# wwang2/CoarseGrainingVAE

Measured on AMD Instinct MI355X. Metric: train_step_frames_per_sec, higher is better.
Workload: dtype f32

## Files before the change

coarsegrainingvae_amd/_lib.py:

```python
from __future__ import annotations

import ctypes as C
import os
import re
import threading

import torch

from . import ktimer

_PKG = os.path.dirname(os.path.abspath(__file__))
LIB_PATH = os.environ.get("CGV_LIB") or os.path.join(_PKG, "libcgvae_hip.so")
HEADER_PATH = os.path.join(os.path.dirname(_PKG), "include", "cgvae_hip.h")

_lock = threading.Lock()
_lib = None

_p, _i, _f, _sz = C.c_void_p, C.c_int, C.c_float, C.c_size_t

PROTOTYPES = {
    "cgv_version": (_i, []),
    "cgv_last_error_string": (C.c_char_p, []),
    "cgv_timestamp": (_i, [_p, _p]),
    "cgv_timestamp_hz": (_i, []),
    "cgv_sustained_clock_probe": (_i, [_p, _p, _i, _i, _p]),
    "cgv_set_option": (_i, [_i, _i]),
    "cgv_get_option": (_i, [_i]),
    "cgv_reset_options": (_i, []),
    "cgv_rbf_supported": (_i, [_i]),
    "cgv_geom_stride": (_i, [_i]),
    "cgv_geom_unit_offset": (_i, [_i]),
    "cgv_radius_graph_count": (_i, [_p, _p, _i, _i, _f, _i, _p, _p, _p]),
    "cgv_radius_graph_emit": (_i, [_p, _p, _i, _i, _f, _i, _p, _p, _p]),
    "cgv_csr_workspace_bytes": (_sz, [_i]),
    "cgv_csr_build": (_i, [_p, _p, _i, _i, _i, _i, _p, _p, _p, _p, _p, _p, _p, _p, _p, _sz, _p]),
    "cgv_group_plan_workspace_bytes": (_sz, [_i]),
    "cgv_group_plan_build": (_i, [_p, _p, _p, _i, _i, _i, _i, _p, _p, _p, _p, _p, _sz, _p]),
    "cgv_group_plan_radix_workspace_bytes": (_sz, [_i]),
    "cgv_group_plan_build_radix": (_i, [_p, _p, _i, _i, _i, _i, _p, _p, _p, _p, _p, _sz, _p]),
    "cgv_geom_group_stride": (_i, [_i]),
    "cgv_geom_group_unit_offset": (_i, [_i]),
    "cgv_edge_geometry_grouped": (_i, [_p, _p, _p, _p, _p, _i, _i, _f, _p, _p, _p]),
    "cgv_edge_geometry": (_i, [_p, _p, _p, _p, _p, _p, _i, _i, _f, _p, _p, _p]),
    "cgv_plan_jobs_max": (_i, []),
    "cgv_plan_job_bytes": (_i, []),
    "cgv_plan_jobs_build": (_i, [_p, _i, _p]),
    "cgv_geom_jobs_max": (_i, []),
    "cgv_geom_job_bytes": (_i, []),
    "cgv_geom_jobs_build": (_i, [_p, _i, _p]),
    "cgv_segment_reduce": (_i, [_p, _p, _p, _i, _i, _i, _p, _p]),
    "cgv_embedding_rows": (_i, [_p, _p, _i, _i, _i, _i, _p, _p]),
    "cgv_embedding_rows2": (_i, [_p, _p, _i, _i, _i, _p, _p, _p, _i, _i, _i, _p, _i, _p]),
    "cgv_segment_reduce_pair": (_i, [_p, _p, _p, _i, _p, _p, _p, _p, _i, _p, _i, _p]),
    "cgv_segment_broadcast": (_i, [_p, _p, _p, _i, _i, _i, _p, _p]),
    "cgv_equi_msg_fwd": (_i, [_p, _p, _p, _p, _p, _p, _p, _p, _p, _i, _i, _i, _i, C.c_int64, C.c_int64, _p, _p, _p]),
    "cgv_equi_msg_grouped_supported": (_i, [_i, _i, _i]),
    "cgv_equi_msg_fwd_grouped": (_i, [_p] * 9 + [_i, _i, _i, _i, C.c_int64, C.c_int64, _p, _p, _p]),
    "cgv_equi_msg_bwd_workspace_bytes": (_sz, [_i, _i, _i]),
    "cgv_equi_msg_bwd": (_i, [_p] * 13 + [_i, _i, _i, C.c_int64, C.c_int64, _p, _sz, _p]),
    "cgv_pseudo_msg_fwd": (_i, [_p] * 14 + [_i, _i, _i, _i, _p]),
    "cgv_pseudo_msg_fwd_rows": (_i, [_p] * 15 + [_i, _i, _i, _i, C.c_int64, _p]),
    "cgv_pseudo_msg_bwd_workspace_bytes": (_sz, [_i, _i, _i]),
    "cgv_pseudo_msg_bwd": (_i, [_p] * 24 + [_i, _i, _i, _i, C.c_int64, _p, _sz, _p]),
    "cgv_pseudo_msg_bwd_deferred": (_i, [_p] * 22 + [_i, _i, _i, _i, C.c_int64, _p, _sz, _p, _p]),
    "cgv_update_rows_from_vec": (_i, [_p, _p, _i, _i, _p]),
    "cgv_tile_bwd_input_plan": (_i, [_i, _i, _i, _i, _p, _p]),
    "cgv_tile_linear_bwd_input_norm_stack": (_i, [_p, _p, _p, _i, _i, _i, _i, _p, _p, _p, _p, _p, _i, _i, _p]),
    "cgv_update_vec_from_rows": (_i, [_p, _p, _p, _i, _i, _p]),
    "cgv_update_norm_stack_fwd": (_i, [_p, _p, _p, _i, _i, _i, _p]),
    "cgv_update_norm_stack_bwd": (_i, [_p, _p, _p, _p, _p, _p, _i, _i, _i, _i, _p]),
    "cgv_update_gate_fwd": (_i, [_p, _p, _p, _p, _p, _p, _p, _i, _i, _i, _p]),
    "cgv_update_gate_bwd": (_i, [_p, _p, _p, _p, _p, _p, _p, _p, _i, _i, _i, _p]),
    "cgv_skinny_max_rows": (_i, []),
    "cgv_skinny_supported": (_i, [_i, _i, _i]),
    "cgv_skinny_fwd_supported": (_i, [_i, _i, _i]),
    "cgv_skinny_linear_fwd": (_i, [_p, _p, _p, _p, _p, _i, _i, _i, _i, _p]),
    "cgv_skinny_bwd_input_supported": (_i, [_i, _i, _i]),
    "cgv_skinny_bwd_input_workspace_bytes": (_sz, [_i, _i, _i]),
    "cgv_skinny_linear_bwd_input": (_i, [_p, _p, _p, _p, _i, _i, _i, _i, _p, _sz, _p]),
    "cgv_decoder_layer_supported": (_i, [_i, _i, _i]),
    "cgv_decoder_slice_floats": (C.c_int64, [_i, _i]),
    "cgv_batch_load_rows": (_i, [_p, _p, _p, _i, _p, _p, _p, _i, _p]),
    "cgv_reparam_sample": (_i, [_p, _p, _p, _p, C.c_int64, _p, _p]),
    "cgv_reparam_bwd": (_i, [_p, _p, _p, _p, _p, _p, C.c_int64, _p]),
    "cgv_pair_linear_fwd": (_i, [_p] * 10 + [_i] * 5 + [_p]),
    "cgv_equi_msg_bwd_deferred": (_i, [_p] * 11 + [_i, _i, _i, C.c_int64, C.c_int64, _p, C.c_size_t, _p, _p, _p]),
    "cgv_filter_reduce_jobs_max": (_i, []),
    "cgv_filter_reduce_job_bytes": (_i, []),
    "cgv_filter_reduce_jobs": (_i, [_p, _i, _p]),
    "cgv_pair_linear_bwd_input": (_i, [_p] * 6 + [_i, _i, _p, _p, _i, _i, _i, _p, C.c_size_t, _p]),
    "cgv_loss_tail_supported": (_i, [_i, _i, _i, _i]),
    "cgv_loss_tail_workspace_bytes": (_sz, [_i]),
    "cgv_loss_tail": (_i, [_p] * 12 + [_i, _i, _i, _i, _i, _f, _f] + [_p] * 9 + [_p, _sz, _p]),
    "cgv_multi_linear_max": (_i, []),
    "cgv_multi_linear_fwd": (_i, [_i] + [_p] * 6 + [_i, _i, _i, _p]),
    "cgv_multi_linear_bwd_input": (_i, [_i, _i] + [_p] * 5 + [_i, _i, _i, _p, C.c_size_t, _p]),
    "cgv_decoder_max_edges": (_i, []),
    "cgv_decoder_block_channels": (_i, [_i]),
    "cgv_decoder_debug_clock": (_i, [_p]),
    "cgv_decoder_msg_fwd": (_i, [_p] * 18 + [_i, _i, _i, _i, _p]),
    "cgv_decoder_dense_fwd": (_i, [_p, _p, _p, _p, _p, _i, _i, _i, _i, _p]),
    "cgv_prior_msg_fwd": (_i, [_p] * 13 + [_i, _i, _i, _i, _i, _p]),
    "cgv_prior_msg_bwd": (_i, [_p] * 8 + [_i, C.c_int64] + [_p] * 6 + [C.c_int64, _i, _i, _i, _i, _p]),
    "cgv_decoder_uv_fwd": (_i, [_p, _p, _p, _p, _i, _i, _p]),
    "cgv_decoder_gate_fwd": (_i, [_p] * 9 + [_i, _i, _p]),
    "cgv_decoder_gate_bwd": (_i, [_p, _p, _p, _p, _i, C.c_int64, _p, _p, _p, _p, _p, _p, C.c_int64, _i, _i, _p]),
    "cgv_decoder_dense_bwd": (_i, [_p, _i, C.c_int64, _p, _i, _p, _p, _p, C.c_int64, _i, _i, _i, _p]),
    "cgv_decoder_uv_bwd": (_i, [_p, _i, C.c_int64, _p, _p, _p, _p, _p, _p, _p, _p, C.c_int64, _i, _i, _p]),
    "cgv_decoder_msg_bwd": (_i, [_p] * 15 + [_p, _i, C.c_int64, _p, _p, _p] + [_p] * 8 + [C.c_int64, _i, _i, _i, _i, _p]),
    "cgv_decoder_slices_to_dense": (_i, [_p, _p, _i, C.c_int64, _p, _i, _i, _p]),
    "cgv_dense_grad_prepare": (_i, [_p, _p, _p, _p, _i, _i, _i, _i, _p]),
    "cgv_tile_supported": (_i, [_i, _i, _i]),
    "cgv_tile_linear_fwd": (_i, [_p, _p, _p, _p, _p, _i, _i, _i, _i, _p]),
    "cgv_tile_linear_bwd_input": (_i, [_p, _p, _p, _i, _i, _i, _p]),
    "cgv_tile_linear_bwd_input_act": (_i, [_p, _p, _p, _p, _i, _i, _i, _i, _p]),
    "cgv_tile_linear_bwd_input_act_add": (_i, [_p, _p, _p, _p, _p, _i, _i, _i, _i, _p]),
    "cgv_tile_linear_bwd_input_act_add_bcast": (_i, [_p] * 7 + [_i, _p, _i, _i, _i, _i, _p]),
    "cgv_tile_pair_supported": (_i, [_i, _i, _i]),
    "cgv_tile_pair_linear_fwd": (_i, [_p] * 10 + [_i, _i, _i, _i, _i, _p]),
    "cgv_tile_pair_linear_bwd_input": (_i, [_p] * 10 + [_i, _i, _i, _i, _i, _p]),
    "cgv_tile_linear_bwd_input_out": (_i, [_p] * 5 + [_i, _i, _i, _i, _p, _i, _p]),
    "cgv_tile_bwd_input_split": (_i, [_p, _sz, _p]),
    "cgv_tile_pair_linear_bwd_input_out": (_i, [_p] * 10 + [_i, _i, _i, _i, _i, _p, _i, _p, _i, _p]),
    "cgv_tile_linear_bwd_input_sum2": (_i, [_p] * 10 + [_i, _p, _i, _i, _i, _i, _i, _p]),
    "cgv_segment_reduce2": (_i, [_p, _i, _p, _p, _i, _p, _p, _p, _i, _i, _p]),
    "cgv_skinny_linear_bwd_input_add": (_i, [_p, _p, _p, _p, _p, _i, _i, _i, _i, _p, _sz, _p]),
    "cgv_skinny_linear_bwd_input_out": (_i, [_p] * 5 + [_i, _i, _i, _i, _p, _i, _p, _sz, _p]),
    "cgv_tile_linear_wgrad": (_i, [_p, _p, _p, _i, _i, _i, _i, _p]),
    "cgv_wgrad_record_bytes": (_i, []),
    "cgv_wgrad_plan": (_i, [_i, _i, _i, _p, _p, _p]),
    "cgv_wgrad_lds_floats": (_i, [_i, _i]),
    "cgv_grouped_wgrad": (_i, [_p, _i, _i, _i, _p]),
    "cgv_wgrad_gathered_plan": (_i, [_i, _i, _i, _i, _p, _p]),
    "cgv_grouped_wgrad_gathered": (_i, [_p, _i, _i, _p]),
    "cgv_wgrad_gathered_plan_tile": (_i, [_i, _i, _i, _i, _i, _p, _p]),
    "cgv_grouped_wgrad_gathered_tile": (_i, [_p, _i, _i, _i, _p]),
    "cgv_grouped_wgrad_split": (_i, [_p, _i, _i, _p]),
    "cgv_grouped_wgrad_gathered_sumsq": (_i, [_p, _i, _i, _p, _p, _p]),
    "cgv_grouped_wgrad_gathered_adam": (_i, [_p, _i, _i, _p, _p, _p, _p, _f, _f, _f, _f, _p, _p]),
    "cgv_wgrad_strip_max_rows": (_i, []),
    "cgv_wgrad_strip_plan": (_i, [_i, _i, _i, _i, _p]),
    "cgv_wgrad_strip_split_max_rows": (_i, []),
    "cgv_wgrad_strip_split_plane_bytes": (_sz, [_i, _i]),
    "cgv_grouped_wgrad_strip_split": (_i, [_p, _i, _i, _i, _i, _p, _sz, _p]),
    "cgv_grouped_wgrad_strip": (_i, [_p, _i, _i, _i, _p]),
    "cgv_grouped_wgrad_strip_sumsq": (_i, [_p, _i, _i, _i, _p, _p, _p]),
    "cgv_grouped_wgrad_strip_adam": (_i, [_p, _i, _i, _i, _p, _p, _p, _p, _f, _f, _f, _f, _p, _p]),
    "cgv_pack_record_bytes": (_i, []),
    "cgv_pack_plan": (_i, [_i, _i, _i, _p]),
    "cgv_pack_operands": (_i, [_p, _i, _i, _p]),
    "cgv_reconstruct_fwd": (_i, [_p, _p, _p, _p, _p, _i, _i, _i, _p, _p]),
    "cgv_reconstruct_bwd": (_i, [_p, _p, _p, _p, _i, _i, _i, _p, _p, _p]),
    "cgv_elbo_workspace_bytes": (_sz, [_i, _i]),
    "cgv_elbo_fwd": (_i, [_p] * 7 + [_i, _i, _i, _i, _f, _f] + [_p] * 7 + [_p, _sz, _p]),
    "cgv_elbo_scale": (_i, [_p, _p, _p, _p, _p, _i, _p, _i, _p]),
    "cgv_optim_state_floats": (_i, []),
    "cgv_optim_partial_floats": (_i, []),
    "cgv_adam_clip_step": (_i, [_p, _p, _p, _p, C.c_int64, _f, _f, _f, _f, _f, _f, _p, _f, _p, _p, _p]),
    "cgv_optim_prepare": (_i, [_p, C.c_int64, _f, _f, _f, _f, _p, _f, _p, _p, _p]),
    "cgv_adam_apply": (_i, [_p, _p, _p, _p, C.c_int64, _f, _f, _f, _f, _p, _p]),
    "cgv_sgd_apply": (_i, [_p, _p, C.c_int64, _f, _p, _p]),
    "cgv_wgrad_gram": (_i, [_p, _i, _i, _p, _p, C.c_size_t, _p]),
    "cgv_wgrad_gram_workspace_bytes": (C.c_size_t, [_i]),
    "cgv_wgrad_gram_mfma": (_i, [_p, _i, _i, _p, _p, C.c_size_t, _p]),
    "cgv_wgrad_gram_mfma_workspace_bytes": (C.c_size_t, [_i, _i]),
    "cgv_wgrad_gram_mfma_max_rows": (_i, []),
    "cgv_rank_update_supported": (_i, [_i, _i, _i]),
    "cgv_optim_prepare_extra": (_i, [_p, C.c_int64, _p, _i, _f, _f, _f, _f, _p, _f, _p, _p, _p]),
    "cgv_grouped_wgrad_adam": (_i, [_p, _i, _i, _i, _p, _p, _p, _p, _f, _f, _f, _f, _p, _p]),
    "cgv_rank_flat_quantum": (_i, []),
    "cgv_rank_flat_plan": (_i, [_i, _i, _i, _i, _p, _p]),
    "cgv_grouped_wgrad_adam_flat": (_i, [_p, _i, _i, _i, _i, _p, _p, _p, _p, _f, _f, _f, _f, _p, _p]),
    "cgv_grouped_wgrad_adam_mixed": (_i, [_p, _i, _i, _i, _i, _i, _i, _p, _p, _p, _p, _f, _f, _f, _f, _p, _p]),
    "cgv_sample_quality_max_classes": (_i, []),
    "cgv_sample_quality": (_i, [_p] * 6 + [_i] * 5 + [_p, _p, _p]),
    "cgv_ensemble_check_max_classes": (_i, []),
    "cgv_ensemble_check_max_samples": (_i, []),
    "cgv_ensemble_check": (_i, [_p] * 7 + [_i] * 6 + [_p, _p, _p]),
    "cgv_internal_hist_max_features": (_i, []),
    "cgv_internal_hist_max_pairs": (_i, []),
    "cgv_internal_hist_max_bins": (_i, []),
    "cgv_internal_hist_max_bins2": (_i, []),
    "cgv_internal_hist_max_atoms": (_i, []),
    "cgv_internal_hist_max_staged_atoms": (_i, []),
    "cgv_internal_hist_feature_tile": (_i, [_i]),
    "cgv_internal_hist_pair_tile": (_i, [_i]),
    "cgv_internal_hist": (_i, [_p] * 4 + [_i] * 6 + [C.c_double] * 2 + [_p] * 3),
    "cgv_internal_values": (_i, [_p] * 3 + [_i] * 3 + [_p] * 3),
    "cgv_kde_max_planes": (_i, []),
    "cgv_kde_max_samples": (_i, []),
    "cgv_kde_max_points": (_i, []),
    "cgv_kde_max_splits": (_i, []),
# ... 21 lines not shown
    "cgv_sasa_max_points": (_i, []),
    "cgv_sasa_max_classes": (_i, []),
    "cgv_sasa_max_structures": (_i, []),
    "cgv_sasa_workspace_bytes": (_sz, [_i, _i, _i]),
    "cgv_sasa_counts": (_i, [_p] * 5 + [_i] * 5 + [_p] * 5 + [_p, _sz, _p]),
    "cgv_cluster_max_structures": (_i, []),
    "cgv_cluster_workspace_bytes": (_sz, [_i, _i]),
    "cgv_cluster_pack": (_i, [_p, _i, _i, _i, _i, _i, C.c_double, _p, _p]),
    "cgv_cluster_gromos": (_i, [_p, _p, _i, _p, _p, _p, _p, _p]),
    "cgv_hbond_max_structures": (_i, []),
    "cgv_hbond_max_hydrogens": (_i, []),
    "cgv_hbond_max_acceptors": (_i, []),
    "cgv_hbond_row_tile": (_i, []),
    "cgv_hbond_chunk": (_i, []),
    "cgv_hbond_workspace_bytes": (_sz, [_i, _i, _i]),
    "cgv_hbond_counts": (_i, [_p] * 6 + [_i, _i, _i, _i, _f, _f] + [_p] * 5 + [_p, _sz, _p]),
    "cgv_lddt_max_atoms": (_i, []),
    "cgv_lddt_max_structures": (_i, []),
    "cgv_lddt_max_references": (_i, []),
    "cgv_lddt_row_tile": (_i, []),
    "cgv_lddt_col_tile": (_i, []),
    "cgv_lddt_chunk": (_i, []),
    "cgv_lddt_workspace_bytes": (_sz, [_i, _i, _i]),
    "cgv_lddt_counts": (_i, [_p] * 7 + [_i] * 4 + [_f] * 6 + [_p] * 3 + [_p, _sz, _p]),
    "cgv_dssp_max_residues": (_i, []),
    "cgv_dssp_max_structures": (_i, []),
    "cgv_dssp_wave_path_max": (_i, []),
    "cgv_dssp_bend_c2": (_f, []),
    "cgv_dssp_assign": (_i, [_p] * 4 + [_i, _i, _i] + [_p] * 5 + [_p]),
    "cgv_pca_max_features": (_i, []),
    "cgv_pca_max_atoms": (_i, []),
    "cgv_pca_max_structures": (_i, []),
    "cgv_pca_max_components": (_i, []),
    "cgv_pca_max_bins2": (_i, []),
    "cgv_pca_moments_splits": (_i, [_i, _i]),
    "cgv_pca_moments_workspace_bytes": (_sz, [_i, _i]),
    "cgv_pca_moments": (_i, [_p] * 4 + [_i] * 3 + [_p] * 3 + [_p, _sz, _p]),
    "cgv_pca_project": (_i, [_p] * 6 + [_i] * 4 + [_p, _i, _i, _i] + [C.c_double] * 4 + [_p] * 3),
    "cgv_pairdist_max_atoms": (_i, []),
    "cgv_pairdist_max_structures": (_i, []),
    "cgv_pairdist_max_classes": (_i, []),
    "cgv_pairdist_max_bins": (_i, []),
    "cgv_pairdist_row_tile": (_i, []),
    "cgv_pairdist_col_tile": (_i, []),
    "cgv_pairdist_chunk": (_i, []),
    "cgv_pairdist_workspace_bytes": (_sz, [_i, _i]),
    "cgv_pairdist_counts": (_i, [_p] * 4 + [_i] * 5 + [_f] * 2 + [_p] * 3 + [_p, _sz, _p]),
    "cgv_dist_moments_max_atoms": (_i, []),
    "cgv_dist_moments_max_structures": (_i, []),
    "cgv_dist_moments_max_total": (_i, []),
    "cgv_dist_moments_row_tile": (_i, []),
    "cgv_dist_moments_col_tile": (_i, []),
    "cgv_dist_moments_chunk": (_i, []),
    "cgv_dist_moments_workspace_bytes": (_sz, [_i, _i]),
    "cgv_dist_moments": (_i, [_p] * 4 + [_i] * 3 + [_p] * 4 + [_p, _sz, _p]),
    "cgv_align_max_atoms": (_i, []),
    "cgv_align_max_structures": (_i, []),
    "cgv_align_wave_fits": (_i, [_i]),
    "cgv_align_workspace_bytes": (_sz, [_i, _i, _i]),
    "cgv_align_accumulate": (_i, [_p] * 3 + [_i] * 4 + [_p] * 6 + [_p, _sz, _p]),
    "cgv_cgae_resident_fits": (_i, [_i, _i, _i]),
    "cgv_cgae_workspace_bytes": (_sz, [_i, _i, _i, _i]),
    "cgv_cgae_steps": (_i, [_i] + [_p] * 7 + [_i, _p, C.c_int64, _i, _i, _i, _i, C.c_int64, _i, _f] + [C.c_double] * 4 +
                       [C.c_uint64, _p, _p, _p, _p, _sz, _p]),
    "cgv_cgae_noise": (_i, [C.c_uint64, C.c_int64, _i, _i, _i, _p, _p]),
    "cgv_newman_resident_fits": (_i, [_i, _i]),
    "cgv_newman_groups": (_i, [_i, _i]),
    "cgv_newman_workspace_bytes": (_sz, [_i, _i, _i, _i]),
    "cgv_newman_betweenness": (_i, [_p] * 4 + [_i] * 4 + [_p, _p, _sz, _p]),
    "cgv_newman_components": (_i, [_p] * 5 + [_i] * 4 + [_p, _p, _p, _sz, _p]),
    "cgv_newman_partition": (_i, [_p] * 8 + [_i] * 6 + [_p, _sz, _p]),
    "cgv_baseline_resident_fits": (_i, [_i, _i, _i, _i]),
    "cgv_baseline_workspace_bytes": (_sz, [_i] * 7),
    "cgv_baseline_steps": (_i, [_i, _i, _i] + [_p] * 4 + [_i, _p, C.c_int64] + [_i] * 5 + [_p, _p, _p, _i, C.c_int64, _i, _f] +
                           [C.c_double] * 4 + [_p, _p, _p, _sz, _p]),
    "cgv_baseline_loss_workspace_bytes": (_sz, [_i, _i, _i]),
    "cgv_baseline_loss": (_i, [_p, _p, _p, _i, _i, _i, _f, _p, _p, _p, _sz, _p]),
}


OPTIONS = {"msg_fwd_split": 0, "msg_bwd_split": 1, "csr_build": 2, "pseudo_chunks": 3, "wgrad_tiling": 4, "tile_fwd_lds_min": 5,
           "bwd_input_waves": 6, "pseudo_fwd": 7, "decoder_fat": 8, "decoder_wlds": 9, "skinny_rows": 10, "tile_fwd_bal": 11,
           "optim_one_launch": 12, "decoder_colsplit": 13, "decoder_nodesplit": 14, "bwd_input_split": 15, "msg_bwd_mfma": 16,
           "streamk": 17}


def set_option(name: str, value: int) -> None:
    call("cgv_set_option", OPTIONS[name], int(value))


def get_option(name: str) -> int:
    return int(load().cgv_get_option(OPTIONS[name]))


def reset_options() -> None:
    call("cgv_reset_options")


def header_symbols():
    text = open(HEADER_PATH).read()
    text = re.sub(r"/\*.*?\*/", "", text, flags=re.S)
    return sorted(set(re.findall(r"\b(cgv_[a-z0-9_]+)\s*\(", text)))


def load():
    global _lib
    if _lib is not None:
        return _lib
    with _lock:
        if _lib is not None:
            return _lib
        if not os.path.exists(LIB_PATH):
            raise RuntimeError(
                f"{LIB_PATH} is missing: build it with `python -m coarsegrainingvae_amd.build` "
                "(hipcc --offload-arch=gfx950).  There is no fallback path.")
        lib = C.CDLL(LIB_PATH)
        for name, (res, args) in PROTOTYPES.items():
            fn = getattr(lib, name)
            fn.restype = res
            fn.argtypes = args
        if lib.cgv_version() < 101:
            raise RuntimeError("libcgvae_hip.so is older than this package")
        _lib = lib
    return _lib


def stream_ptr() -> int:
    return torch.cuda.current_stream().cuda_stream


def ptr(t):
    if t is None:
        return None
    if not t.is_cuda:
        raise RuntimeError("coarsegrainingvae_amd kernels need device (hip) tensors; there is no CPU path")
    if not t.is_contiguous():
        raise RuntimeError("tensor handed to the C ABI must be contiguous")
    return t.data_ptr()


_SPLIT_WS = {}
_SPLIT_TLS = threading.local()
_SPLIT_BYTES = 64 * 1024 + 64 * 1024 * 1024


def prepare_split_workspace(stream=None):
    st = torch.cuda.current_stream() if stream is None else stream
    key = (st.device.index if st.device.index is not None else torch.cuda.current_device(), int(st.cuda_stream))
    if key not in _SPLIT_WS:
        if torch.cuda.is_current_stream_capturing():
            return None
        _SPLIT_WS[key] = torch.zeros(_SPLIT_BYTES, dtype=torch.uint8, device=f"cuda:{key[0]}")
    return _SPLIT_WS[key]


def split_workspace_ready() -> bool:
    if load().cgv_get_option(OPTIONS["bwd_input_split"]) == 1:
        return False
    key = (torch.cuda.current_device(), int(torch.cuda.current_stream().cuda_stream))
    return key in _SPLIT_WS or not torch.cuda.is_current_stream_capturing()


def _register_split_workspace(lib):
    key = (torch.cuda.current_device(), int(torch.cuda.current_stream().cuda_stream))
    if getattr(_SPLIT_TLS, "cur", None) == key:
        return
    ws = prepare_split_workspace()
# ... 20 lines not shown
```

coarsegrainingvae_amd/csrc/api.cpp:

```cpp
#include <stdarg.h>
#include <string.h>
#include <atomic>
#include "cgv_common.h"

namespace cgv {
static thread_local char g_err[512] = "";
void set_error(const char* fmt, ...) {
  va_list ap;
  va_start(ap, fmt);
  vsnprintf(g_err, sizeof(g_err), fmt, ap);
  va_end(ap);
}

static const int g_opt_default[] = {
     -1,    -1,     0,
     0,     0,       448,
     0,   0,         1,
     1,      0,        1,
     0,  2,   1,
     -1,  -1,      0};
static_assert(sizeof(g_opt_default) == CGV_OPT_COUNT * sizeof(int), "one default per CGV_OPT_*");
static std::atomic<int> g_opt[CGV_OPT_COUNT];
static void reset_options() {
  for (int i = 0; i < CGV_OPT_COUNT; ++i) g_opt[i].store(g_opt_default[i], std::memory_order_relaxed);
}
static const bool g_opt_ready = (reset_options(), true);
int option(int id) { return g_opt[id].load(std::memory_order_relaxed); }
}

extern "C" {
int cgv_version(void) { return CGV_VERSION; }
int cgv_set_option(int option, int value) {
  CGV_REQUIRE(option >= 0 && option < CGV_OPT_COUNT, "unknown option");
  cgv::g_opt[option].store(value, std::memory_order_relaxed);
  return 0;
}
int cgv_get_option(int option) {
  if (option < 0 || option >= CGV_OPT_COUNT) return INT32_MIN;
  return cgv::g_opt[option].load(std::memory_order_relaxed);
}
int cgv_reset_options(void) {
  cgv::reset_options();
  return 0;
}
const char* cgv_last_error_string(void) { return cgv::g_err; }
int cgv_rbf_supported(int R) {
  switch (R) {
#define X(n) case n:
    CGV_RBF_LIST(X)
#undef X
    return 1;
    default:
      return 0;
  }
}
int cgv_geom_stride(int R) { return cgv::geom_stride(R); }
int cgv_geom_unit_offset(int R) { return cgv::geom_unit_offset(R); }
}
```

coarsegrainingvae_amd/csrc/decoder_layer.hip:

```cpp
#include "cgv_common.h"

namespace cgv {

typedef float f32x4 __attribute__((ext_vector_type(4)));

__constant__ unsigned long long* g_dl_clock = nullptr;
#ifndef CGV_DL_CLOCK
#define CGV_DL_CLOCK 0
#endif
#if CGV_DL_CLOCK
#define DL_SPAN(id, end)                                                                                    \
  do {                                                                                                      \
    if (g_dl_clock && threadIdx.x == 0) {                                                                   \
      if (blockIdx.x == 0) g_dl_clock[32 + 4 * (id) + (end)] = wall_clock64();                              \
      if (blockIdx.x == gridDim.x - 1) g_dl_clock[32 + 4 * (id) + 2 + (end)] = wall_clock64();              \
    }                                                                                                       \
  } while (0)

#define DL_PH(id, i) do { if (g_dl_clock && blockIdx.x == 0 && threadIdx.x == 0) g_dl_clock[80 + 10 * (id) + (i)] = wall_clock64(); } while (0)
#else
#define DL_SPAN(id, end) do { } while (0)
#define DL_PH(id, i) do { } while (0)
#endif

#if CGV_DL_CLOCK
#define DL_WV(i) do { if (g_dl_clock && blockIdx.x == 0 && (threadIdx.x & 63) == 0) g_dl_clock[192 + 8 * (threadIdx.x >> 6) + (i)] = wall_clock64(); } while (0)
#else
#define DL_WV(i) do { } while (0)
#endif
#ifndef CGV_DL_FILTER_PERM
#define CGV_DL_FILTER_PERM 1
#endif
constexpr int DL_CB = 4;
constexpr int DL_WAVES = 9;
constexpr int DL_THREADS = 64 * DL_WAVES;
constexpr int DL_MAX_NODES = 16;

struct dv3 { float x, y, z; };
__device__ __forceinline__ dv3 dldv(const float* p) { f3 t = ld3(p); return dv3{t.x, t.y, t.z}; }
__device__ __forceinline__ dv3 dcross(const dv3& a, const dv3& b) {
  return dv3{a.y * b.z - a.z * b.y, a.z * b.x - a.x * b.z, a.x * b.y - a.y * b.x};
}
__device__ __forceinline__ float ddot(const dv3& a, const dv3& b) { return a.x * b.x + a.y * b.y + a.z * b.z; }
__device__ __forceinline__ void daxpy(dv3& acc, float a, const dv3& x) {
  acc.x = fmaf(a, x.x, acc.x); acc.y = fmaf(a, x.y, acc.y); acc.z = fmaf(a, x.z, acc.z);
}
__device__ __forceinline__ float add_xor32(float x) {
  const auto r = __builtin_amdgcn_permlane32_swap(__float_as_uint(x), __float_as_uint(x), false, false);
  return __uint_as_float(r[0]) + __uint_as_float(r[1]);
}
__device__ __forceinline__ float add_xor16(float x) {
  const auto r = __builtin_amdgcn_permlane16_swap(__float_as_uint(x), __float_as_uint(x), false, false);
  return __uint_as_float(r[0]) + __uint_as_float(r[1]);
}
__device__ __forceinline__ float add_row_stride4(float x) {
  x += __uint_as_float(__builtin_amdgcn_update_dpp(0, __float_as_uint(x), 0x128 , 0xf, 0xf, false));
  x += __uint_as_float(__builtin_amdgcn_update_dpp(0, __float_as_uint(x), 0x124 , 0xf, 0xf, false));
  return x;
}
template <int R>
__device__ __forceinline__ float dfilt(const float (&W)[R + 1], const float* __restrict__ g) {
  float w = W[R] * g[R];
#pragma unroll
  for (int n = 0; n < R; ++n) w = fmaf(W[n], g[n], w);
  return w;
}

extern __shared__ __attribute__((aligned(16))) unsigned char dl_smem[];
struct Carve {
  size_t off = 0;
  __device__ __forceinline__ float* take(size_t floats) {
    float* p = reinterpret_cast<float*>(dl_smem + off);
    off += ((floats * 4 + 15) / 16) * 16;
    return p;
  }
};

#define CGV_GLOBAL_AS __attribute__((address_space(1)))
typedef const CGV_GLOBAL_AS float* gcf;
typedef const CGV_GLOBAL_AS int* gci;
__device__ __forceinline__ gcf launder(const float* p) {
  unsigned long long a = reinterpret_cast<unsigned long long>(p);
  asm volatile("" : "+s"(a));
  return reinterpret_cast<gcf>(a);
}
__device__ __forceinline__ gci launder(const int* p) {
  unsigned long long a = reinterpret_cast<unsigned long long>(p);
  asm volatile("" : "+s"(a));
  return reinterpret_cast<gci>(a);
}
__device__ __forceinline__ const float* generic(gcf p) { return (const float*)p; }
__device__ __forceinline__ void pin_loads() { asm volatile("" ::: "memory"); }
__device__ __forceinline__ float4 ldg4_pinned(gcf p) {
  const f32x4 t = *reinterpret_cast<const CGV_GLOBAL_AS f32x4*>(p);
  return make_float4(t.x, t.y, t.z, t.w);
}
#ifndef CGV_DL_NT_WEIGHTS
#define CGV_DL_NT_WEIGHTS 0
#endif
__device__ __forceinline__ float4 ldg4_stream(gcf p) {
#if CGV_DL_NT_WEIGHTS
  const f32x4 t = __builtin_nontemporal_load(reinterpret_cast<const CGV_GLOBAL_AS f32x4*>(p));
#else
  const f32x4 t = *reinterpret_cast<const CGV_GLOBAL_AS f32x4*>(p);
#endif
  return make_float4(t.x, t.y, t.z, t.w);
}
__device__ __forceinline__ float ldg_pinned(gcf p) { return *p; }
__device__ __forceinline__ int ldgi_pinned(gci p) { return *p; }
__device__ __forceinline__ f3 ld3_pinned(gcf p) { return f3{p[0], p[1], p[2]}; }

constexpr int DL_QS = 6;
template <int MB, int NQ, int QS = DL_QS>
struct QuadRegs { float4 v[QS][NQ][MB]; };

template <int MB, int NQ, int QS>
__device__ __forceinline__ void quad_issue(QuadRegs<MB, NQ, QS>& r, gcf slices, int n_slices, long long stride,
                                           int rows, const int (&kq)[NQ]) {
  const int lane = threadIdx.x & 63, wave = __builtin_amdgcn_readfirstlane(threadIdx.x >> 6);
  const int m = lane & 15, cls = wave * 4 + (lane >> 4);
#pragma unroll
  for (int u = 0; u < QS; ++u) {
    const int s = min(cls + 36 * u, n_slices - 1);
#pragma unroll
    for (int q = 0; q < NQ; ++q)
#pragma unroll
      for (int mb = 0; mb < MB; ++mb)
        r.v[u][q][mb] = ldg4_pinned(slices + (size_t)s * stride + ((size_t)kq[q] * rows + min(mb * 16 + m, rows - 1)) * 4);
  }
}

template <int MB, int NQ, int QS>
__device__ __forceinline__ void quad_finish(const QuadRegs<MB, NQ, QS>& r, float4* __restrict__ tile ,
                                            float4* __restrict__ scratch , int n_slices, int rows, int ph = -1) {
  constexpr int MP = 16 * MB;
  const int lane = threadIdx.x & 63, wave = __builtin_amdgcn_readfirstlane(threadIdx.x >> 6);
  const int m = lane & 15, cls = wave * 4 + (lane >> 4);
#pragma unroll
  for (int q = 0; q < NQ; ++q)
#pragma unroll
    for (int mb = 0; mb < MB; ++mb) {
      float4 acc = make_float4(0.f, 0.f, 0.f, 0.f);
#pragma unroll
      for (int u = 0; u < QS; ++u)
        if (cls + 36 * u < n_slices) { acc.x += r.v[u][q][mb].x; acc.y += r.v[u][q][mb].y; acc.z += r.v[u][q][mb].z; acc.w += r.v[u][q][mb].w; }
      acc.x = add_xor16(acc.x); acc.y = add_xor16(acc.y); acc.z = add_xor16(acc.z); acc.w = add_xor16(acc.w);
      acc.x = add_xor32(acc.x); acc.y = add_xor32(acc.y); acc.z = add_xor32(acc.z); acc.w = add_xor32(acc.w);
      if (lane < 16) scratch[((q * DL_WAVES + wave) * MB + mb) * 16 + m] = acc;
    }
  if (ph >= 0) DL_PH(ph, 2);
  if (ph == 8) DL_WV(3);
  __syncthreads();
  if (ph >= 0) DL_PH(ph, 3);
  if (threadIdx.x < NQ * MP) {
    const int q = threadIdx.x / MP, mm = threadIdx.x - q * MP;
    float4 t = make_float4(0.f, 0.f, 0.f, 0.f);
#pragma unroll
    for (int c = 0; c < DL_WAVES; ++c) {
      const float4 v = scratch[((q * DL_WAVES + c) * MB + mm / 16) * 16 + (mm & 15)];
      t.x += v.x; t.y += v.y; t.z += v.z; t.w += v.w;
    }
    if (mm >= rows) t = make_float4(0.f, 0.f, 0.f, 0.f);
    tile[q * MP + mm] = t;
  }
  __syncthreads();
}

template <int G, int NT>
struct BiRegs { float4 w[NT][G]; };

struct TileRange { int beg, end; };
__device__ __forceinline__ TileRange dl_tile_range(int K) {
  const int tiles = (K + 63) / 64, per = (tiles + (int)gridDim.y - 1) / (int)gridDim.y;
  const int beg = (int)blockIdx.y * per;
  return TileRange{beg, min(beg + per, tiles)};
}
__device__ __forceinline__ int dl_tile_of(const TileRange& tr, int wave, int t) {
  const int pos = t == 0 ? wave : (int)((0x854372106ull >> (4 * wave)) & 15);
  return tr.beg + DL_WAVES * t + pos;
}

template <int G, int NT>
__device__ __forceinline__ void bi_prefetch(BiRegs<G, NT>& r, gcf W, int K, const int (&row0)[G], const TileRange& tr) {
  const int lane = threadIdx.x & 63, wave = __builtin_amdgcn_readfirstlane(threadIdx.x >> 6);
  const int j = lane & 15, q = lane >> 4;
#pragma unroll
  for (int t = 0; t < NT; ++t) {
    const int tile = dl_tile_of(tr, wave, t);
    if (tile < tr.end) {
      const int col = tile * 64 + 4 * j;
      const int cc = col < K ? col : 0;
#pragma unroll
      for (int g = 0; g < G; ++g) r.w[t][g] = ldg4_stream(W + (size_t)(row0[g] + q) * K + cc);
    } else {
#pragma unroll
      for (int g = 0; g < G; ++g) r.w[t][g] = make_float4(0.f, 0.f, 0.f, 0.f);
    }
  }
}

template <int SLOT, int G, int NT>
__device__ __forceinline__ void bi_prefetch_slot(BiRegs<G, NT>& r, gcf W, int K, const int (&row0)[G], int tile) {
  const int lane = threadIdx.x & 63;
  const int j = lane & 15, q = lane >> 4;
  const int col = tile * 64 + 4 * j;
  const int cc = col < K ? col : 0;
#pragma unroll
  for (int g = 0; g < G; ++g) r.w[SLOT][g] = ldg4_stream(W + (size_t)(row0[g] + q) * K + cc);
}

#ifndef CGV_DL_SLICE_STORE
#define CGV_DL_SLICE_STORE 1
#endif
__device__ __forceinline__ void st4_slice(float4* p, const float4& v) {
#if CGV_DL_SLICE_STORE == 1
  const f32x4 t = {v.x, v.y, v.z, v.w};
  asm volatile("global_store_dwordx4 %0, %1, off sc1" : : "v"(p), "v"(t) : "memory");
#else
  *p = v;
#endif
}

template <int MB>
__host__ __device__ constexpr size_t bi_stage_floats() { return (size_t)DL_WAVES * 16 * 16 * MB * 4; }

template <int MB, int G, int NT, int NPRE = NT>
__device__ __forceinline__ void bi_core(const BiRegs<G, NPRE>& r, const float* __restrict__ g_tile ,
                                        float* __restrict__ stage ,
                                        float* __restrict__ slice , int K, int rows, const TileRange& tr,
                                        const float* __restrict__ W = nullptr, const int* row0 = nullptr, int ph = -1) {
  constexpr int MP = 16 * MB;
  const int lane = threadIdx.x & 63, wave = __builtin_amdgcn_readfirstlane(threadIdx.x >> 6);
  const int j = lane & 15, q = lane >> 4;
  float4* st = reinterpret_cast<float4*>(stage) + (size_t)wave * 16 * MP;
#pragma unroll
  for (int t = 0; t < NT; ++t) {
    const int tile = dl_tile_of(tr, wave, t);
    if (tile >= tr.end) continue;
    f32x4 acc[MB][4];
#pragma unroll
    for (int mb = 0; mb < MB; ++mb)
#pragma unroll
      for (int c = 0; c < 4; ++c) acc[mb][c] = f32x4{0.f, 0.f, 0.f, 0.f};
    float4 late[G];
    if (t >= NPRE) {
      const int col = tile * 64 + 4 * j;
      const int cc = col < K ? col : 0;
#pragma unroll
      for (int g = 0; g < G; ++g) late[g] = *reinterpret_cast<const float4*>(W + (size_t)(row0[g] + q) * K + cc);
    }
#pragma unroll
    for (int g = 0; g < G; ++g) {
      const float4 w = t < NPRE ? r.w[t < NPRE ? t : 0][g] : late[g];
#pragma unroll
      for (int mb = 0; mb < MB; ++mb) {
        const float a = g_tile[(mb * 16 + j) * (G * 4) + g * 4 + q];
        acc[mb][0] = __builtin_amdgcn_mfma_f32_16x16x4f32(a, w.x, acc[mb][0], 0, 0, 0);
        acc[mb][1] = __builtin_amdgcn_mfma_f32_16x16x4f32(a, w.y, acc[mb][1], 0, 0, 0);
        acc[mb][2] = __builtin_amdgcn_mfma_f32_16x16x4f32(a, w.z, acc[mb][2], 0, 0, 0);
        acc[mb][3] = __builtin_amdgcn_mfma_f32_16x16x4f32(a, w.w, acc[mb][3], 0, 0, 0);
      }
    }
#pragma unroll
    for (int mb = 0; mb < MB; ++mb)
#pragma unroll
      for (int rr = 0; rr < 4; ++rr)
        st[j * MP + mb * 16 + 4 * q + rr] = make_float4(acc[mb][0][rr], acc[mb][1][rr], acc[mb][2][rr], acc[mb][3][rr]);
    if (ph >= 0 && t == 0) DL_PH(ph, 7);
    const int quads = min(16, (K - tile * 64) / 4);
    float4* out = reinterpret_cast<float4*>(slice) + (size_t)tile * 16 * rows;
    for (int idx = lane; idx < quads * rows; idx += 64) {
      const int jj = idx / rows, m = idx - jj * rows;
      st4_slice(out + idx, st[jj * MP + m]);
    }
  }
}

template <int MB, int G>
__host__ __device__ constexpr size_t fwd_red_floats() { return (size_t)DL_WAVES * ((G + 3) / 4) * MB * 256; }

struct NoHook { __device__ __forceinline__ void operator()() const {} };
template <int MB, int G, int SB = (((G + 3) / 4) * MB >= 3 ? 5 : 9), typename Hook = NoHook>
__device__ __forceinline__ void fwd_core(float* __restrict__ out, float* __restrict__ red, const float* __restrict__ x,
                                         int M, int K, const float* __restrict__ W, const int (&row0)[G],
                                         Hook after_issue = Hook(), int ph = -1) {
  constexpr int T = (G + 3) / 4;
  const int lane = threadIdx.x & 63, wave = __builtin_amdgcn_readfirstlane(threadIdx.x >> 6);
  const int i = lane & 15, q = lane >> 4;
  const int steps = (K + 15) / 16, per = (steps + DL_WAVES - 1) / DL_WAVES;
  const int s_beg = wave * per, s_end = min(s_beg + per, steps);
  const float* wrow[T];
#pragma unroll
  for (int t = 0; t < T; ++t) {
    const int g = min(t * 4 + (i >> 2), G - 1);
    wrow[t] = W + (size_t)(row0[g] + (i & 3)) * K;
  }
  const float* xrow[MB];
#pragma unroll
  for (int mb = 0; mb < MB; ++mb) xrow[mb] = x + (size_t)min(mb * 16 + i, M - 1) * K;
  f32x4 acc[T][MB];
#pragma unroll
  for (int t = 0; t < T; ++t)
#pragma unroll
    for (int mb = 0; mb < MB; ++mb) acc[t][mb] = f32x4{0.f, 0.f, 0.f, 0.f};
  bool first = true;
  for (int s0 = s_beg; first || s0 < s_end; s0 += SB) {
    float4 a[SB][T], b[SB][MB];
#pragma unroll
    for (int u = 0; u < SB; ++u) {
      const int k = (s0 + u) * 16 + 4 * q;
      const int kc = (s0 + u < s_end && k < K) ? k : 0;
#pragma unroll
      for (int t = 0; t < T; ++t) a[u][t] = *reinterpret_cast<const float4*>(wrow[t] + kc);
#pragma unroll
      for (int mb = 0; mb < MB; ++mb) b[u][mb] = *reinterpret_cast<const float4*>(xrow[mb] + kc);
    }
    if (first) { after_issue(); first = false; if (ph >= 0) DL_PH(ph, 1); }
#pragma unroll
    for (int u = 0; u < SB; ++u) {
      if (s0 + u < s_end) {
        const bool kok = (s0 + u) * 16 + 4 * q < K;
#pragma unroll
        for (int t = 0; t < T; ++t) {
          const float4 w = make_float4(kok ? a[u][t].x : 0.f, kok ? a[u][t].y : 0.f, kok ? a[u][t].z : 0.f, kok ? a[u][t].w : 0.f);
#pragma unroll
          for (int mb = 0; mb < MB; ++mb) {
            acc[t][mb] = __builtin_amdgcn_mfma_f32_16x16x4f32(w.x, b[u][mb].x, acc[t][mb], 0, 0, 0);
            acc[t][mb] = __builtin_amdgcn_mfma_f32_16x16x4f32(w.y, b[u][mb].y, acc[t][mb], 0, 0, 0);
            acc[t][mb] = __builtin_amdgcn_mfma_f32_16x16x4f32(w.z, b[u][mb].z, acc[t][mb], 0, 0, 0);
            acc[t][mb] = __builtin_amdgcn_mfma_f32_16x16x4f32(w.w, b[u][mb].w, acc[t][mb], 0, 0, 0);
          }
        }
      }
    }
  }
#pragma unroll
  for (int t = 0; t < T; ++t)
#pragma unroll
    for (int mb = 0; mb < MB; ++mb)
#pragma unroll
      for (int r = 0; r < 4; ++r) red[(((wave * T + t) * MB + mb) * 4 + r) * 64 + lane] = acc[t][mb][r];
  if (ph >= 0) DL_PH(ph, 2);
  __syncthreads();
  if (ph >= 0) DL_PH(ph, 3);
  for (int o = threadIdx.x; o < T * MB * 256; o += DL_THREADS) {
    const int l = o & 63, r = (o >> 6) & 3, rest = o >> 8;
    const int mb = rest % MB, t = rest / MB;
    const int g = t * 4 + (l >> 4), m = mb * 16 + (l & 15);
    float v = 0.f;
#pragma unroll
    for (int w = 0; w < DL_WAVES; ++w) v += red[(((w * T + t) * MB + mb) * 4 + r) * 64 + l];
    if (g < G) out[(m * G + g) * 4 + r] = v;
  }
  __syncthreads();
  if (ph >= 0) DL_PH(ph, 4);
}

template <int G>
__device__ __forceinline__ void wlds_issue(float* __restrict__ w_l, const float* __restrict__ W, int K, const int (&row0)[G]) {
  const int lane = threadIdx.x & 63, wave = __builtin_amdgcn_readfirstlane(threadIdx.x >> 6);
#pragma unroll
  for (int g = 0; g < G; ++g) {
    if ((g % DL_WAVES) != wave) continue;
    const float* src = W + (size_t)row0[g] * K;
    for (int u = 0; u * 64 < K; ++u) {
      const int idx = u * 64 + lane;
      if (idx < K)
        __builtin_amdgcn_global_load_lds(reinterpret_cast<const CGV_GLOBAL_AS void*>(reinterpret_cast<unsigned long long>(src + 4 * (size_t)idx)),
                                         (__attribute__((address_space(3))) void*)(w_l + (size_t)g * 4 * K + u * 256), 16, 0, 0);
    }
  }
}

constexpr int WLDS_SB = 6;
__device__ __forceinline__ void wlds_x_issue(float4 (&b)[WLDS_SB], const float* __restrict__ x, int M, int K) {
  const int lane = threadIdx.x & 63, wave = __builtin_amdgcn_readfirstlane(threadIdx.x >> 6);
  const int i = lane & 15, q = lane >> 4;
  const int steps = (K + 15) / 16, per = (steps + DL_WAVES - 1) / DL_WAVES;
  const int s_beg = wave * per, s_end = min(s_beg + per, steps);
  const float* xrow = x + (size_t)min(i, M - 1) * K;
#pragma unroll
  for (int u = 0; u < WLDS_SB; ++u) {
    const int k = (s_beg + u) * 16 + 4 * q;
    b[u] = *reinterpret_cast<const float4*>(xrow + ((s_beg + u < s_end && k < K) ? k : 0));
  }
}
template <int G>
__device__ __forceinline__ void fwd_core_wlds_finish(float* __restrict__ out, float* __restrict__ red, const float4 (&b)[WLDS_SB],
                                                     int K, const float* __restrict__ w_l, int ph = -1) {
  constexpr int T = (G + 3) / 4, SB = WLDS_SB;
  const int lane = threadIdx.x & 63, wave = __builtin_amdgcn_readfirstlane(threadIdx.x >> 6);
  const int i = lane & 15, q = lane >> 4;
  const int steps = (K + 15) / 16, per = (steps + DL_WAVES - 1) / DL_WAVES;
  const int s_beg = wave * per, s_end = min(s_beg + per, steps);
  if (ph >= 0) DL_PH(ph, 1);
  asm volatile("s_waitcnt vmcnt(0)" ::: "memory");
  __syncthreads();
  if (ph >= 0) DL_PH(ph, 2);
  f32x4 acc[T];
#pragma unroll
  for (int t = 0; t < T; ++t) acc[t] = f32x4{0.f, 0.f, 0.f, 0.f};
  int wrow[T];
#pragma unroll
  for (int t = 0; t < T; ++t) wrow[t] = (min(t * 4 + (i >> 2), G - 1) * 4 + (i & 3)) * K;
#pragma unroll
  for (int u = 0; u < SB; ++u) {
    const int k = (s_beg + u) * 16 + 4 * q;
    const bool kok = s_beg + u < s_end && k < K;
    if (s_beg + u < s_end) {
#pragma unroll
      for (int t = 0; t < T; ++t) {
        float4 w = *reinterpret_cast<const float4*>(w_l + wrow[t] + (kok ? k : 0));
        if (!kok) w = make_float4(0.f, 0.f, 0.f, 0.f);
        acc[t] = __builtin_amdgcn_mfma_f32_16x16x4f32(w.x, b[u].x, acc[t], 0, 0, 0);
        acc[t] = __builtin_amdgcn_mfma_f32_16x16x4f32(w.y, b[u].y, acc[t], 0, 0, 0);
        acc[t] = __builtin_amdgcn_mfma_f32_16x16x4f32(w.z, b[u].z, acc[t], 0, 0, 0);
        acc[t] = __builtin_amdgcn_mfma_f32_16x16x4f32(w.w, b[u].w, acc[t], 0, 0, 0);
      }
    }
  }
#pragma unroll
  for (int t = 0; t < T; ++t)
#pragma unroll
    for (int r = 0; r < 4; ++r) red[((wave * T + t) * 4 + r) * 64 + lane] = acc[t][r];
  if (ph >= 0) DL_PH(ph, 3);
  __syncthreads();
  for (int o = threadIdx.x; o < T * 256; o += DL_THREADS) {
    const int l = o & 63, r = (o >> 6) & 3, t = o >> 8;
    const int g = t * 4 + (l >> 4), m = l & 15;
    float v = 0.f;
#pragma unroll
    for (int w = 0; w < DL_WAVES; ++w) v += red[((w * T + t) * 4 + r) * 64 + l];
    if (g < G) out[(m * G + g) * 4 + r] = v;
  }
  __syncthreads();
  if (ph >= 0) DL_PH(ph, 4);
}

constexpr int DL_MAX_EDGES = 240;
template <int SLOTS> struct Slots4 { float4 v[SLOTS]; };
template <int SLOTS>
__device__ __forceinline__ void copy4_issue(Slots4<SLOTS>& r, gcf src, int n4) {
#pragma unroll
  for (int u = 0; u < SLOTS; ++u) r.v[u] = ldg4_pinned(src + 4 * (size_t)min((int)threadIdx.x + u * DL_THREADS, n4 - 1));
}
template <int SLOTS>
__device__ __forceinline__ void copy4_commit(const Slots4<SLOTS>& r, float* __restrict__ dst, int n4) {
#pragma unroll
  for (int u = 0; u < SLOTS; ++u)
    if ((int)threadIdx.x + u * DL_THREADS < n4) reinterpret_cast<float4*>(dst)[threadIdx.x + u * DL_THREADS] = r.v[u];
}
__device__ __forceinline__ int int_issue(gci src, int n) { return ldgi_pinned(src + min((int)threadIdx.x, n - 1)); }
__device__ __forceinline__ void int_commit(int v, int* __restrict__ dst, int n) { if ((int)threadIdx.x < n) dst[threadIdx.x] = v; }
__device__ __forceinline__ float4 scalar_issue(gcf src, gcf valid, int n, int F, int f0) {
  return ldg4_pinned((src ? src : valid) + (size_t)min((int)threadIdx.x, n - 1) * F + f0);
}
__device__ __forceinline__ void scalar_commit(float4 v, bool have, float* __restrict__ dst, int n) {
  if ((int)threadIdx.x < n) reinterpret_cast<float4*>(dst)[threadIdx.x] = have ? v : make_float4(0.f, 0.f, 0.f, 0.f);
}
__device__ __forceinline__ float4 vector_issue(gcf src, gcf valid, int n, int F, int f0) {
  const int t = min((int)threadIdx.x, 3 * n - 1), m = t / 3, part = t - 3 * m;
  return ldg4_pinned((src ? src : valid) + ((size_t)m * F + f0) * 3 + 4 * part);
}
__device__ __forceinline__ void vector_commit(float4 v, bool have, float* __restrict__ dst, int n) {
  if ((int)threadIdx.x < 3 * n) reinterpret_cast<float4*>(dst)[threadIdx.x] = have ? v : make_float4(0.f, 0.f, 0.f, 0.f);
}
constexpr int geom_slots(int R) { return (DL_MAX_EDGES * geom_stride(R) / 4 + DL_THREADS - 1) / DL_THREADS; }
__device__ __forceinline__ void stage_copy4(float* __restrict__ dst, const float* __restrict__ src, int n4) {
  for (int i = threadIdx.x; i < n4; i += DL_THREADS) reinterpret_cast<float4*>(dst)[i] = reinterpret_cast<const float4*>(src)[i];
}
__device__ __forceinline__ void stage_ints(int* __restrict__ dst, const int* __restrict__ src, int n) {
  for (int i = threadIdx.x; i < n; i += DL_THREADS) dst[i] = src[i];
}
__device__ __forceinline__ void stage_scalar(float* __restrict__ dst, const float* __restrict__ src, int n, int F, int f0) {
  if (threadIdx.x < n)
    reinterpret_cast<float4*>(dst)[threadIdx.x] = src ? *reinterpret_cast<const float4*>(src + (size_t)threadIdx.x * F + f0)
                                                      : make_float4(0.f, 0.f, 0.f, 0.f);
}
__device__ __forceinline__ void stage_vector(float* __restrict__ dst, const float* __restrict__ src, int n, int F, int f0) {
  if (threadIdx.x < 3 * n) {
    const int m = threadIdx.x / 3, part = threadIdx.x - 3 * m;
    reinterpret_cast<float4*>(dst)[threadIdx.x] =
        src ? *reinterpret_cast<const float4*>(src + ((size_t)m * F + f0) * 3 + 4 * part) : make_float4(0.f, 0.f, 0.f, 0.f);
  }
}
__device__ __forceinline__ dv3 lds_v3(const float* p) { return dv3{p[0], p[1], p[2]}; }

template <int R, bool WLDS>
__global__ __launch_bounds__(DL_THREADS) void dec_msg_fwd_k(
    const float* __restrict__ a1, const float* __restrict__ W2, const float* __restrict__ b2, const float* __restrict__ s_,
    const float* __restrict__ sbar_, const float* __restrict__ v_, const float* __restrict__ vbar_,
    const float* __restrict__ geom_, const int* __restrict__ rowptr_, const int* __restrict__ src_,
    const float* __restrict__ Wd_, const float* __restrict__ bd_, float* __restrict__ phi_out, float* __restrict__ stack,
    float* __restrict__ sbar_out, float* __restrict__ v_out, float* __restrict__ vbar_out, float* __restrict__ rows_out,
    int n, int F, int E) {
  constexpr int GS = geom_stride(R), U = geom_unit_offset(R);
  Carve cv;
  float* red = cv.take(fwd_red_floats<1, 9>());
  float* phi_l = cv.take(16 * 9 * 4);
  float* red2 = cv.take(8 * 3 * 64);
  float* geom_l = cv.take((size_t)DL_MAX_EDGES * GS);
  int* rp_l = reinterpret_cast<int*>(cv.take(20));
  int* src_l = reinterpret_cast<int*>(cv.take(DL_MAX_EDGES));
  float* s_l = cv.take(64); float* sb_l = cv.take(64);
  float* v_l = cv.take(192); float* vb_l = cv.take(192);
  float* w_l = cv.take(WLDS ? (size_t)36 * F : 0);
  const int f0 = blockIdx.x * DL_CB;
  const int lane = threadIdx.x & 63;
  const int k = __builtin_amdgcn_readfirstlane(threadIdx.x >> 6);
  const int i = lane >> 2, c = lane & 3;
  const bool live = i < n;
  const int f = f0 + c;
  int row0[9];
#pragma unroll
  for (int g = 0; g < 9; ++g) row0[g] = g * F + f0;
  if (WLDS) wlds_issue<9>(w_l, W2, F, row0);
  DL_PH(1, 0);
  DL_SPAN(1, 0);
  const gcf geom = launder(geom_); const gci rowptr = launder(rowptr_); const gci src = launder(src_);
  const gcf s = launder(s_); const gcf sbar = launder(sbar_); const gcf v = launder(v_);
  const gcf vbar = launder(vbar_); const gcf Wd = launder(Wd_); const gcf bd = launder(bd_);
  const int n4 = E * GS / 4;
  Slots4<geom_slots(R)> r_geom;
  copy4_issue(r_geom, geom, n4);
  const int half = k == 0 ? lane >> 5 : 0;
  const gcf cand = k == 0 ? (half == 0 ? s : sbar) : k == 1 ? v : vbar;
  const int sm_D = k == 0 ? 1 : 3, sm_cnt = k == 0 ? n : 3 * n, sm_A = k == 0 ? F : 3 * F, sm_B = k == 0 ? 0 : 4;
  const int sm_C = k == 0 ? f0 : 3 * f0, sm_item = k == 0 ? (lane & 31) : lane;
  float4 r_small;
  {
    const int it = min(sm_item, sm_cnt - 1);
    const int m = (it * (sm_D == 1 ? 65536 : 21846)) >> 16, part = it - m * sm_D;
    r_small = ldg4_pinned(cand + ((size_t)m * sm_A + part * sm_B + sm_C));
  }
  const int id_item = k < 4 ? k * 64 + lane : lane, id_cnt = k < 4 ? E : n + 1;
  const int r_ids = ldgi_pinned((k < 4 ? src : rowptr) + min(id_item, id_cnt - 1));
  float W[R + 1];
#pragma unroll
  for (int nn = 0; nn < R; ++nn) W[nn] = ldg_pinned(Wd + ((size_t)k * F + f) * R + nn);
  W[R] = ldg_pinned(bd + (size_t)k * F + f);
  pin_loads();
  float4 xb[WLDS_SB];
  if (WLDS) wlds_x_issue(xb, a1, n, F);
  else fwd_core<1, 9, 5>(phi_l, red, a1, n, F, W2, row0, NoHook(), 1);
  {
    copy4_commit(r_geom, geom_l, n4);
    float* dst = k == 0 ? (half == 0 ? s_l : sb_l) : k == 1 ? v_l : vb_l;
    if (k <= 2 && sm_item < sm_cnt) reinterpret_cast<float4*>(dst)[sm_item] = r_small;
    if (k <= 4 && id_item < id_cnt) (k < 4 ? src_l : rp_l)[id_item] = r_ids;
  }
  if (WLDS) fwd_core_wlds_finish<9>(phi_l, red, xb, F, w_l, 1);
  for (int o = threadIdx.x; o < 16 * 9; o += DL_THREADS) {
    const int m = o / 9, g = o - m * 9;
    float4 p = *reinterpret_cast<float4*>(phi_l + (m * 9 + g) * 4);
    const float4 b = *reinterpret_cast<const float4*>(b2 + (size_t)g * F + f0);
    p.x += b.x; p.y += b.y; p.z += b.z; p.w += b.w;
    *reinterpret_cast<float4*>(phi_l + (m * 9 + g) * 4) = p;
    if (m < n) *reinterpret_cast<float4*>(phi_out + (size_t)m * 9 * F + (size_t)g * F + f0) = p;
  }
  __syncthreads();
  DL_PH(1, 5);
  const int ic = live ? i : 0;
  const float s_i = s_l[ic * 4 + c], sb_i = sb_l[ic * 4 + c];
  const dv3 v_i = lds_v3(v_l + (ic * 4 + c) * 3), vb_i = lds_v3(vb_l + (ic * 4 + c) * 3);
  float ah = 0.f, ahb = 0.f;
  dv3 acc{0.f, 0.f, 0.f};
  const float* __restrict__ vsrc = (k == 2 || k == 6 || k == 7) ? v_l : vb_l;
  const int e_beg = live ? rp_l[i] : 0, e_end = live ? min(rp_l[i + 1], E) : 0;
  int j_nx = e_beg < e_end ? src_l[e_beg] : 0;
  for (int e = e_beg; e < e_end; ++e) {
    const int j = j_nx;
    j_nx = src_l[min(e + 1, e_end - 1)];
    const float* __restrict__ g = geom_l + (size_t)e * GS;
    const dv3 vj = lds_v3(vsrc + (j * 4 + c) * 3);
    const float q = phi_l[(j * 9 + k) * 4 + c] * dfilt<R>(W, g);
    switch (k) {
      case 0: ah = fmaf(q, s_i, ah); ahb += ddot(v_i, vj); break;
      case 1: daxpy(acc, q, dv3{g[U], g[U + 1], g[U + 2]}); break;
      case 2: daxpy(acc, q, vj); break;
      case 3: daxpy(acc, q, dcross(v_i, vj)); break;
      case 4: daxpy(acc, q * sb_i, vj); break;
      case 5: daxpy(acc, q, vj); break;
      case 6: daxpy(acc, q * sb_i, vj); break;
      case 7: daxpy(acc, q, dcross(v_i, vj)); break;
      default: daxpy(acc, q, dcross(vb_i, vj)); break;
    }
  }
  DL_PH(1, 6);
  if (k > 0) { red2[((k - 1) * 3 + 0) * 64 + lane] = acc.x; red2[((k - 1) * 3 + 1) * 64 + lane] = acc.y; red2[((k - 1) * 3 + 2) * 64 + lane] = acc.z; }
  __syncthreads();
  if (k != 0 || !live) { DL_SPAN(1, 1); return; }
  dv3 av{0.f, 0.f, 0.f}, avb{0.f, 0.f, 0.f};
#pragma unroll
  for (int w = 0; w < 4; ++w) { av.x += red2[(w * 3 + 0) * 64 + lane]; av.y += red2[(w * 3 + 1) * 64 + lane]; av.z += red2[(w * 3 + 2) * 64 + lane]; }
#pragma unroll
  for (int w = 4; w < 8; ++w) { avb.x += red2[(w * 3 + 0) * 64 + lane]; avb.y += red2[(w * 3 + 1) * 64 + lane]; avb.z += red2[(w * 3 + 2) * 64 + lane]; }
  ah += s_i; ahb += sb_i;
  av.x += v_i.x; av.y += v_i.y; av.z += v_i.z;
  avb.x += vb_i.x; avb.y += vb_i.y; avb.z += vb_i.z;
  const size_t nf = (size_t)i * F + f;
  stack[(size_t)i * 2 * F + f] = ah;
  sbar_out[nf] = ahb;
  st3(v_out + nf * 3, av.x, av.y, av.z);
  st3(vbar_out + nf * 3, avb.x, avb.y, avb.z);
  rows_out[((size_t)3 * i + 0) * F + f] = av.x;
  rows_out[((size_t)3 * i + 1) * F + f] = av.y;
  rows_out[((size_t)3 * i + 2) * F + f] = av.z;
  DL_PH(1, 7);
  DL_SPAN(1, 1);
}

__global__ __launch_bounds__(DL_THREADS) void dec_dense_fwd_k(const float* __restrict__ x, const float* __restrict__ W,
                                                              const float* __restrict__ bias_, float* __restrict__ y,
                                                              float* __restrict__ zout, int n, int N, int K, int act) {
  Carve cv;
  float* red = cv.take(fwd_red_floats<1, 1>());
  float* o_l = cv.take(16 * 4);
  const int n0 = blockIdx.x * DL_CB;
  const int row0[1] = {n0};
  const bool mine = threadIdx.x < n * 4;
  const int i = threadIdx.x >> 2, c = threadIdx.x & 3;
  const gcf bias = launder(bias_);
  const float b = (mine && bias) ? ldg_pinned(bias + n0 + c) : 0.f;
  pin_loads();
  const int ph = K > N ? 3 : 0;
  DL_SPAN(ph, 0);
  DL_PH(ph, 0);
  if (K <= 16 * DL_WAVES * 5) fwd_core<1, 1, 5>(o_l, red, x, n, K, W, row0, NoHook(), ph);
  else fwd_core<1, 1, 9>(o_l, red, x, n, K, W, row0, NoHook(), ph);
  if (mine) {
    const float zv = o_l[i * 4 + c] + b;
    const size_t at = (size_t)i * N + n0 + c;
    if (act) { if (zout) zout[at] = zv; y[at] = act_fwd(zv, act); } else y[at] = zv;
  }
  DL_PH(ph, 5);
  DL_SPAN(ph, 1);
}

constexpr int DL_MULTI_MAX = 4;
struct DensePair {
  const float* x[DL_MULTI_MAX]; const float* W[DL_MULTI_MAX]; const float* bias[DL_MULTI_MAX];
  float* y[DL_MULTI_MAX]; float* z[DL_MULTI_MAX];
  int act[DL_MULTI_MAX];
};
template <int CQ>
__global__ __launch_bounds__(DL_THREADS) void dec_dense_fwd_pair_k(DensePair p, int n, int N, int K) {
  Carve cv;
  float* red = cv.take(fwd_red_floats<1, CQ>());
  float* o_l = cv.take(16 * CQ * 4);
  const int j = blockIdx.y;
  const float* __restrict__ x = p.x[j];
  const float* __restrict__ W = p.W[j];
  float* __restrict__ y = p.y[j];
  float* __restrict__ zout = p.z[j];
  const int act = p.act[j];
  const int n0 = blockIdx.x * DL_CB * CQ;
  int row0[CQ];
#pragma unroll
  for (int g = 0; g < CQ; ++g) row0[g] = n0 + 4 * g;
  const bool mine = threadIdx.x < n * 4 * CQ;
  const int i = threadIdx.x / (4 * CQ), c = threadIdx.x - i * 4 * CQ;
  const gcf bias = launder(p.bias[j]);
  const float b = (mine && bias) ? ldg_pinned(bias + n0 + c) : 0.f;
  pin_loads();
  if (K <= 16 * DL_WAVES * 5) fwd_core<1, CQ, 5>(o_l, red, x, n, K, W, row0);
  else fwd_core<1, CQ, 9>(o_l, red, x, n, K, W, row0);
  if (mine) {
    const float zv = o_l[(i * CQ + (c >> 2)) * 4 + (c & 3)] + b;
    const size_t at = (size_t)i * N + n0 + c;
    if (act) { if (zout) zout[at] = zv; y[at] = act_fwd(zv, act); } else y[at] = zv;
  }
}

__global__ __launch_bounds__(DL_THREADS) void dec_uv_fwd_k(const float* __restrict__ rows, const float* __restrict__ Wuv,
                                                           float* __restrict__ UV, float* __restrict__ stack, int n, int F) {
  Carve cv;
  float* red = cv.take(fwd_red_floats<3, 2>());
  float* uv_l = cv.take(48 * 2 * 4);
  const int f0 = blockIdx.x * DL_CB;
  const int row0[2] = {f0, F + f0};
  DL_SPAN(2, 0);
  DL_PH(2, 0);
  fwd_core<3, 2>(uv_l, red, rows, 3 * n, F, Wuv, row0, NoHook(), 2);
  for (int o = threadIdx.x; o < 3 * n * 2; o += DL_THREADS) {
    const int m = o >> 1, g = o & 1;
    *reinterpret_cast<float4*>(UV + (size_t)m * 2 * F + (size_t)g * F + f0) = *reinterpret_cast<const float4*>(uv_l + (m * 2 + g) * 4);
  }
// ... 184 lines not shown
      g = reinterpret_cast<const float*>(sum_l + q * 16)[i * 4 + c4];
      if (blockIdx.y == 0) g_dense[at] = g;
      if (act) g *= act_bwd(zz, act);
    }
    g_l[(i * CBQ + q) * 4 + c4] = g;
  }
  __syncthreads();
  DL_PH(ph, 6);
  bi_core<1, CBQ, NT>(wr, g_l, stage, slices_out + (size_t)blockIdx.x * out_stride, K, n, tr, nullptr, nullptr, ph);
  DL_PH(ph, 8);
  DL_SPAN(ph, 1);
}

template <int CBQ, int QS, int NT>
__global__ __launch_bounds__(DL_THREADS) void dec_uv_bwd_k(const float* __restrict__ gstack_slices_, int gs_n, long long gs_stride,
                                                           const float* __restrict__ UV_, const float* __restrict__ stack_,
                                                           const float* __restrict__ gs_res_, const float* __restrict__ Wuv_,
                                                           const float* gUV_in_, float* gUV_out, float* __restrict__ g_s2,
                                                           float* __restrict__ slices_out, long long out_stride, int n, int F) {
  constexpr int C = 4 * CBQ, G = 2 * CBQ;
  Carve cv;
  float* stage = cv.take(bi_stage_floats<3>());
  float4* scratch = reinterpret_cast<float4*>(cv.take(G * 36 * 16 * 4));
  float4* gsum_l = reinterpret_cast<float4*>(cv.take(G * 16 * 4));
  float* g_l = cv.take(48 * G * 4);
  const int f0 = blockIdx.x * C;
  DL_SPAN(7, 0);
  DL_PH(7, 0);
  const gcf gstack_slices = launder(gstack_slices_); const gcf UV = launder(UV_); const gcf stack = launder(stack_);
  const gcf gs_res = launder(gs_res_); const gcf Wuv = launder(Wuv_);
  const gcf gUV_in = launder(gUV_in_);
  int row0[G], kq[G];
#pragma unroll
  for (int q = 0; q < CBQ; ++q) {
    row0[q] = f0 + 4 * q; row0[CBQ + q] = F + f0 + 4 * q;
    kq[q] = (int)blockIdx.x * CBQ + q; kq[CBQ + q] = F / 4 + (int)blockIdx.x * CBQ + q;
  }
  QuadRegs<1, G, QS> qr;
  quad_issue<1, G>(qr, gstack_slices, gs_n, gs_stride, n, kq);
  const bool mine = threadIdx.x < n * C;
  const int i = threadIdx.x / C, c = threadIdx.x - i * C, f = f0 + c;
  const size_t nf = (size_t)i * F + f;
  const size_t b = (size_t)i * 3 * 2 * F + f;
  float gu[3] = {0.f, 0.f, 0.f}, gvv[3] = {0.f, 0.f, 0.f}, vv[3] = {0.f, 0.f, 0.f}, res = 0.f, nrm = 1.f;
  if (mine) {
#pragma unroll
    for (int xyz = 0; xyz < 3; ++xyz) {
      const size_t at = b + (size_t)xyz * 2 * F;
      gu[xyz] = ldg_pinned(gUV_in + at); gvv[xyz] = ldg_pinned(gUV_in + at + F); vv[xyz] = ldg_pinned(UV + at + F);
    }
    res = ldg_pinned(gs_res + nf);
    nrm = ldg_pinned(stack + (size_t)i * 2 * F + F + f);
  }
  const TileRange tr = dl_tile_range(F);
  BiRegs<G, NT> wr;
  bi_prefetch<G, NT>(wr, Wuv, F, row0, tr);
  pin_loads();
  DL_PH(7, 1);
  for (int o = threadIdx.x; o < 48 * G * 4; o += DL_THREADS) g_l[o] = 0.f;
  quad_finish<1, G>(qr, gsum_l, scratch, gs_n, n, 7);
  DL_PH(7, 4);
  if (mine) {
    const int q = c >> 2, c4 = c & 3;
    if (blockIdx.y == 0) g_s2[nf] = reinterpret_cast<const float*>(gsum_l + q * 16)[i * 4 + c4] + res;
    const float t = reinterpret_cast<const float*>(gsum_l + (CBQ + q) * 16)[i * 4 + c4] / nrm;
#pragma unroll
    for (int xyz = 0; xyz < 3; ++xyz) {
      const float tot = gvv[xyz] + t * vv[xyz];
      if (blockIdx.y == 0) {
        if (gUV_out != gUV_in_) gUV_out[b + (size_t)xyz * 2 * F] = gu[xyz];
        gUV_out[b + (size_t)xyz * 2 * F + F] = tot;
      }
      g_l[((3 * i + xyz) * G + q) * 4 + c4] = gu[xyz];
      g_l[((3 * i + xyz) * G + CBQ + q) * 4 + c4] = tot;
    }
  }
  __syncthreads();
  DL_PH(7, 6);
  bi_core<3, G, NT>(wr, g_l, stage, slices_out + (size_t)blockIdx.x * out_stride, F, 3 * n, tr, nullptr, nullptr, 7);
  DL_PH(7, 8);
  DL_SPAN(7, 1);
}

template <int R, int QS>
__global__ __launch_bounds__(DL_THREADS) void dec_msg_bwd_k(
    const float* __restrict__ phi_, const float* __restrict__ s_, const float* __restrict__ sbar_, const float* __restrict__ v_,
    const float* __restrict__ vbar_, const float* __restrict__ geom_d_, const int* __restrict__ rowptr_d_,
    const int* __restrict__ src_d_, const float* __restrict__ geom_s_, const int* __restrict__ rowptr_s_,
    const int* __restrict__ dst_s_, const float* __restrict__ Wd_, const float* __restrict__ bd_,
    const float* __restrict__ gh_, const float* __restrict__ ghb_, const float* __restrict__ gvrows_slices_, int gvr_n,
    long long gvr_stride, const float* __restrict__ gv_res_, const float* __restrict__ gvb_, const float* __restrict__ W2_,
    float* __restrict__ g_phi, float* __restrict__ g_s, float* __restrict__ g_sbar, float* __restrict__ g_v,
    float* __restrict__ g_vbar, float* __restrict__ gWd, float* __restrict__ gbd, float* __restrict__ slices_out,
    long long out_stride, int n, int F, int E) {
  constexpr int GS = geom_stride(R), U = geom_unit_offset(R);
  Carve cv;
  float* stage = cv.take(bi_stage_floats<1>());
  float4* scratch = reinterpret_cast<float4*>(stage);
  static_assert(bi_stage_floats<1>() >= 36 * 16 * 3 * 4, "scratch aliases the stage");
  float4* gvr_l = reinterpret_cast<float4*>(cv.take(48 * 4));
  float* gphi_l = cv.take(16 * 9 * 4);
  float* phi_l = cv.take(16 * 9 * 4);
  float* red_src = cv.take(9 * 6 * 64);
  float* red_rcv = cv.take(9 * 8 * 64);
  float* geomd_l = cv.take((size_t)DL_MAX_EDGES * GS);
  float* geoms_l = cv.take((size_t)DL_MAX_EDGES * GS);
  int* rpd_l = reinterpret_cast<int*>(cv.take(20)); int* rps_l = reinterpret_cast<int*>(cv.take(20));
  int* srcd_l = reinterpret_cast<int*>(cv.take(DL_MAX_EDGES)); int* dsts_l = reinterpret_cast<int*>(cv.take(DL_MAX_EDGES));
  float* s_l = cv.take(64); float* sb_l = cv.take(64); float* gh_l = cv.take(64); float* ghb_l = cv.take(64);
  float* v_l = cv.take(192); float* vb_l = cv.take(192); float* gv_l = cv.take(192); float* gvb_l = cv.take(192);
  float* gvres_l = cv.take(192);
  const int f0 = blockIdx.x * DL_CB;
  int row0[9];
#pragma unroll
  for (int g = 0; g < 9; ++g) row0[g] = g * F + f0;
  DL_PH(8, 0);
  DL_WV(0);
  DL_SPAN(8, 0);
  const gcf geom_d = launder(geom_d_); const gcf geom_s = launder(geom_s_); const gci rowptr_d = launder(rowptr_d_);
  const gci rowptr_s = launder(rowptr_s_); const gci src_d = launder(src_d_); const gci dst_s = launder(dst_s_);
  const gcf s = launder(s_); const gcf sbar = launder(sbar_); const gcf v = launder(v_);
  const gcf vbar = launder(vbar_); const gcf gh = launder(gh_); const gcf ghb = launder(ghb_);
  const gcf gvb = launder(gvb_); const gcf gv_res = launder(gv_res_); const gcf phi = launder(phi_);
  const gcf Wd = launder(Wd_); const gcf bd = launder(bd_); const gcf gvrows_slices = launder(gvrows_slices_);
  const gcf W2 = launder(W2_);
  const int lane = threadIdx.x & 63;
  const int wave = __builtin_amdgcn_readfirstlane(threadIdx.x >> 6);
#if CGV_DL_FILTER_PERM
  const int k = (int)((0x164058732ull >> (4 * wave)) & 15);
#else
  const int k = wave;
#endif
  const int node = lane >> 2, c = lane & 3, f = f0 + c;
  const bool live = node < n;
  const int nc = live ? node : 0;
  const int n4 = E * GS / 4;
  Slots4<geom_slots(R)> r_gd, r_gs;
#pragma unroll
  for (int u = 0; u < geom_slots(R); ++u) {
    if (wave * 64 + u * DL_THREADS < n4) {
      const int at = min((int)threadIdx.x + u * DL_THREADS, n4 - 1);
      r_gd.v[u] = ldg4_pinned(geom_d + 4 * (size_t)at);
      r_gs.v[u] = ldg4_pinned(geom_s + 4 * (size_t)at);
    }
  }
  const int quarter = wave == 0 ? lane >> 4 : 0;
  const gcf cand = wave == 0 ? (quarter == 0 ? s : quarter == 1 ? sbar : quarter == 2 ? gh : ghb)
                 : wave == 1 ? v : wave == 2 ? vbar : wave == 3 ? gvb : wave == 4 ? gv_res : phi;
  const bool small_have = cand != nullptr;
  const int sm_D = wave == 0 ? 1 : wave <= 4 ? 3 : 9;
  const int sm_cnt = wave == 0 ? n : wave <= 4 ? 3 * n : n * 9;
  const int sm_A = wave == 0 ? F : wave <= 4 ? 3 * F : 9 * F, sm_B = wave == 0 ? 0 : wave <= 4 ? 4 : F;
  const int sm_C = wave <= 4 && wave >= 1 ? 3 * f0 : f0;
  const int sm_item = wave == 0 ? (lane & 15) : wave <= 4 ? lane : (wave - 5) * 64 + lane;
  float4 r_small;
  {
    const int it = min(sm_item, sm_cnt - 1);
    const int m = (it * (sm_D == 1 ? 65536 : sm_D == 3 ? 21846 : 7282)) >> 16, part = it - m * sm_D;
    r_small = ldg4_pinned((small_have ? cand : (wave >= 1 && wave <= 4 ? v : s)) + ((size_t)m * sm_A + part * sm_B + sm_C));
  }
  const int id_item = wave < 8 ? (wave & 3) * 64 + lane : (lane & 31), id_cnt = wave < 8 ? E : n + 1;
  const gci id_src = wave < 4 ? src_d : wave < 8 ? dst_s : (lane < 32 ? rowptr_d : rowptr_s);
  const int r_ids = ldgi_pinned(id_src + min(id_item, id_cnt - 1));
  float W[R + 1], G[R + 1];
#pragma unroll
  for (int nn = 0; nn < R; ++nn) W[nn] = ldg_pinned(Wd + ((size_t)k * F + f) * R + nn);
  W[R] = ldg_pinned(bd + (size_t)k * F + f);
#pragma unroll
  for (int nn = 0; nn <= R; ++nn) G[nn] = 0.f;
  QuadRegs<3, 1, QS> qr;
  { const int kq[1] = {(int)blockIdx.x}; quad_issue<3, 1>(qr, gvrows_slices, gvr_n, gvr_stride, 3 * n, kq); }
  pin_loads();
  DL_WV(1);
#pragma unroll
  for (int u = 0; u < geom_slots(R); ++u)
    if ((int)threadIdx.x + u * DL_THREADS < n4) {
      reinterpret_cast<float4*>(geomd_l)[threadIdx.x + u * DL_THREADS] = r_gd.v[u];
      reinterpret_cast<float4*>(geoms_l)[threadIdx.x + u * DL_THREADS] = r_gs.v[u];
    }
  {
    float* dst = wave == 0 ? (quarter == 0 ? s_l : quarter == 1 ? sb_l : quarter == 2 ? gh_l : ghb_l)
               : wave == 1 ? v_l : wave == 2 ? vb_l : wave == 3 ? gvb_l : wave == 4 ? gvres_l : phi_l;
    if (sm_item < sm_cnt && wave <= 7) reinterpret_cast<float4*>(dst)[sm_item] = small_have ? r_small : make_float4(0.f, 0.f, 0.f, 0.f);
    int* idst = wave < 4 ? srcd_l : wave < 8 ? dsts_l : (lane < 32 ? rpd_l : rps_l);
    if (id_item < id_cnt) idst[id_item] = r_ids;
  }
  DL_PH(8, 1);
  DL_WV(2);
  BiRegs<9, 2> wr;
  const TileRange tr{0, (F + 63) / 64};
  bi_prefetch_slot<0>(wr, W2, F, row0, dl_tile_of(tr, wave, 0));
  pin_loads();
  quad_finish<3, 1>(qr, gvr_l, scratch, gvr_n, 3 * n, 8);
  if (threadIdx.x < 64) {
    const float* gr = reinterpret_cast<const float*>(gvr_l);
#pragma unroll
    for (int xyz = 0; xyz < 3; ++xyz)
      gv_l[(node * 4 + c) * 3 + xyz] = live ? gr[(3 * node + xyz) * 4 + c] + gvres_l[(node * 4 + c) * 3 + xyz] : 0.f;
  }
  __syncthreads();
  DL_PH(8, 4);
  if (dl_tile_of(tr, wave, 1) < tr.end) {
    bi_prefetch_slot<1>(wr, W2, F, row0, dl_tile_of(tr, wave, 1));
  } else {
#pragma unroll
    for (int g = 0; g < 9; ++g) wr.w[1][g] = make_float4(0.f, 0.f, 0.f, 0.f);
  }
  pin_loads();
  const float p_j = phi_l[(nc * 9 + k) * 4 + c];
  const float s_n = s_l[nc * 4 + c], sb_n = sb_l[nc * 4 + c];
  const dv3 v_n = lds_v3(v_l + (nc * 4 + c) * 3), vb_n = lds_v3(vb_l + (nc * 4 + c) * 3);
  const float gh_n = gh_l[nc * 4 + c], ghb_n = ghb_l[nc * 4 + c];
  const dv3 gvb_n = lds_v3(gvb_l + (nc * 4 + c) * 3), gv_n = lds_v3(gv_l + (nc * 4 + c) * 3);
  (void)s_n;
  float a = 0.f;
  dv3 av{0.f, 0.f, 0.f}, avb{0.f, 0.f, 0.f};
  {
    DL_WV(4);
    const float* __restrict__ pA = k >= 5 ? gvb_l : gv_l;
    const float* __restrict__ pB = k == 8 ? vb_l : v_l;
    const float* __restrict__ pS = k == 0 ? gh_l : sb_l;
    const int e_beg = live ? rps_l[node] : 0, e_end = live ? min(rps_l[node + 1], E) : 0;
    int i_nx = e_beg < e_end ? dsts_l[e_beg] : 0;
    for (int e = e_beg; e < e_end; ++e) {
      const float* __restrict__ g = geoms_l + (size_t)e * GS;
      const int ic = i_nx * 4 + c;
      i_nx = dsts_l[min(e + 1, e_end - 1)];
      const dv3 gA = lds_v3(pA + ic * 3), sB = lds_v3(pB + ic * 3);
      const float sc = pS[ic], s_i = s_l[ic], ghb_i = ghb_l[ic];
      float gr[R + 1];
#pragma unroll
      for (int nn = 0; nn <= R; ++nn) gr[nn] = g[nn];
      const dv3 unit{g[U], g[U + 1], g[U + 2]};
      const dv3 zero{0.f, 0.f, 0.f};
      float gq = 0.f;
      dv3 cav = zero, cavb = zero;
      switch (k) {
        case 0: gq = sc * s_i; break;
        case 1: gq = ddot(gA, unit); break;
        case 2: gq = ddot(gA, v_n); cav = gA; break;
        case 3: gq = ddot(gA, dcross(sB, vb_n)); cavb = dcross(gA, sB); break;
        case 4: gq = sc * ddot(gA, vb_n); cavb = dv3{sc * gA.x, sc * gA.y, sc * gA.z}; break;
        case 5: gq = ddot(gA, vb_n); cavb = gA; break;
        case 6: gq = sc * ddot(gA, v_n); cav = dv3{sc * gA.x, sc * gA.y, sc * gA.z}; break;
        case 7: gq = ddot(gA, dcross(sB, v_n)); cav = dcross(gA, sB); break;
        default: gq = ddot(gA, dcross(sB, vb_n)); cavb = dcross(gA, sB); break;
      }
      const float w = dfilt<R>(W, gr);
      a = fmaf(gq, w, a);
      const float t = gq * p_j;
#pragma unroll
      for (int nn = 0; nn <= R; ++nn) G[nn] = fmaf(t, gr[nn], G[nn]);
      const float q = p_j * w;
      daxpy(av, q, cav);
      daxpy(avb, q, cavb);
      if (k == 0) daxpy(avb, ghb_i, sB);
    }
  }
  DL_PH(8, 5);
  DL_WV(5);
  gphi_l[(node * 9 + k) * 4 + c] = live ? a : 0.f;
  {
    float* r = red_src + (size_t)k * 6 * 64 + lane;
    r[0] = av.x; r[64] = av.y; r[128] = av.z; r[192] = avb.x; r[256] = avb.y; r[320] = avb.z;
  }
#pragma unroll
  for (int nn = 0; nn <= R; ++nn) {
    float x = G[nn];
    x = add_xor32(add_xor16(add_row_stride4(x)));
    G[nn] = x;
  }
  if (lane < 4) {
#pragma unroll
    for (int nn = 0; nn < R; ++nn) gWd[((size_t)k * F + f) * R + nn] = G[nn];
    gbd[(size_t)k * F + f] = G[R];
  }
  float as = 0.f, asb = 0.f;
  dv3 rv{0.f, 0.f, 0.f}, rvb{0.f, 0.f, 0.f};
  if (k == 0 || k == 1 || k == 3 || k == 4 || k == 6 || k == 7 || k == 8) {
    const float* __restrict__ pV = (k == 6 || k == 7) ? v_l : vb_l;
    const int e_beg = live ? rpd_l[node] : 0, e_end = live ? min(rpd_l[node + 1], E) : 0;
    int j_nx = e_beg < e_end ? srcd_l[e_beg] : 0;
    for (int e = e_beg; e < e_end; ++e) {
      const int j = j_nx;
      j_nx = srcd_l[min(e + 1, e_end - 1)];
      const dv3 vj = lds_v3(pV + (j * 4 + c) * 3);
      if (k == 1) { daxpy(rv, ghb_n, vj); continue; }
      const float* __restrict__ g = geomd_l + (size_t)e * GS;
      const float q = phi_l[(j * 9 + k) * 4 + c] * dfilt<R>(W, g);
      switch (k) {
        case 0: as = fmaf(gh_n, q, as); break;
        case 3: daxpy(rv, q, dcross(vj, gv_n)); break;
        case 4: asb = fmaf(q, ddot(gv_n, vj), asb); break;
        case 6: asb = fmaf(q, ddot(gvb_n, vj), asb); break;
        case 7: daxpy(rv, q, dcross(vj, gvb_n)); break;
        default: daxpy(rvb, q, dcross(vj, gvb_n)); break;
      }
    }
  }
  {
    float* r = red_rcv + (size_t)k * 8 * 64 + lane;
    r[0] = as; r[64] = asb; r[128] = rv.x; r[192] = rv.y; r[256] = rv.z; r[320] = rvb.x; r[384] = rvb.y; r[448] = rvb.z;
  }
  DL_PH(8, 6);
  DL_WV(6);
  __syncthreads();
  DL_PH(8, 9);
  for (int o = threadIdx.x; o < n * 9; o += DL_THREADS) {
    const int m = o / 9, g = o - m * 9;
    *reinterpret_cast<float4*>(g_phi + (size_t)m * 9 * F + (size_t)g * F + f0) = *reinterpret_cast<const float4*>(gphi_l + (m * 9 + g) * 4);
  }
  if (k < 8 && live) {
    float t = k == 0 ? gh_n : k == 1 ? ghb_n : k == 2 ? gv_n.x : k == 3 ? gv_n.y : k == 4 ? gv_n.z
            : k == 5 ? gvb_n.x : k == 6 ? gvb_n.y : gvb_n.z;
#pragma unroll
    for (int w = 0; w < 9; ++w) t += red_rcv[((size_t)w * 8 + k) * 64 + lane];
    if (k >= 2) {
#pragma unroll
      for (int w = 0; w < 9; ++w) t += red_src[((size_t)w * 6 + (k - 2)) * 64 + lane];
    }
    const size_t jf = (size_t)node * F + f;
    if (k == 0) g_s[jf] = t;
    else if (k == 1) g_sbar[jf] = t;
    else if (k < 5) g_v[jf * 3 + (k - 2)] = t;
    else g_vbar[jf * 3 + (k - 5)] = t;
  }
  bi_core<1, 9, 2>(wr, gphi_l, stage, slices_out + (size_t)blockIdx.x * out_stride, F, n, tr, nullptr, nullptr, 8);
  DL_WV(7);
  DL_PH(8, 8);
  DL_SPAN(8, 1);
}

template <int QS>
__global__ __launch_bounds__(DL_THREADS) void dec_quad_to_dense_k(const float* __restrict__ base, const float* __restrict__ slices,
                                                                  int n_slices, long long stride, float* __restrict__ out, int n,
                                                                  int F) {
  Carve cv;
  float4* scratch = reinterpret_cast<float4*>(cv.take(36 * 16 * 4));
  float4* sum_l = reinterpret_cast<float4*>(cv.take(16 * 4));
  const int kq[1] = {(int)blockIdx.x};
  QuadRegs<1, 1, QS> qr;
  quad_issue<1, 1>(qr, launder(slices), n_slices, stride, n, kq);
  quad_finish<1, 1>(qr, sum_l, scratch, n_slices, n);
  if (threadIdx.x < n) {
    float4 t = sum_l[threadIdx.x];
    if (base) {
      const float4 b = *reinterpret_cast<const float4*>(base + (size_t)threadIdx.x * F + 4 * blockIdx.x);
      t.x += b.x; t.y += b.y; t.z += b.z; t.w += b.w;
    }
    *reinterpret_cast<float4*>(out + (size_t)threadIdx.x * F + 4 * blockIdx.x) = t;
  }
}

template <int R>
__global__ __launch_bounds__(DL_THREADS) void prior_msg_fwd_k(
    const float* __restrict__ a1, const float* __restrict__ W2, const float* __restrict__ b2, const float* __restrict__ s_,
    const float* __restrict__ v_, const float* __restrict__ geom_, const int* __restrict__ rowptr_, const int* __restrict__ src_,
    const float* __restrict__ Wd_, const float* __restrict__ bd_, float* __restrict__ phi_out, float* __restrict__ s_out,
    float* __restrict__ v_out, int n, int F, int E, int with_dv) {
  constexpr int GS = geom_stride(R), U = geom_unit_offset(R);
  Carve cv;
  float* red = cv.take(fwd_red_floats<1, 3>());
  float* phi_l = cv.take(16 * 3 * 4);
  float* red2 = cv.take(2 * 3 * 64);
  float* geom_l = cv.take((size_t)DL_MAX_EDGES * GS);
  int* rp_l = reinterpret_cast<int*>(cv.take(20));
  int* src_l = reinterpret_cast<int*>(cv.take(DL_MAX_EDGES));
  float* s_l = cv.take(64);
  float* v_l = cv.take(192);
  const int f0 = blockIdx.x * DL_CB;
  const int lane = threadIdx.x & 63;
  const int k = __builtin_amdgcn_readfirstlane(threadIdx.x >> 6);
  const int kf = k < 3 ? k : 0;
  const int i = lane >> 2, c = lane & 3;
  const bool live = i < n;
  const int f = f0 + c;
  const int row0[3] = {f0, F + f0, 2 * F + f0};
  const gcf geom = launder(geom_); const gci rowptr = launder(rowptr_); const gci src = launder(src_);
  const gcf s = launder(s_); const gcf v = launder(v_); const gcf Wd = launder(Wd_); const gcf bd = launder(bd_);
  Slots4<geom_slots(R)> r_geom;
  copy4_issue(r_geom, geom, E * GS / 4);
  const int r_rp = int_issue(rowptr, n + 1), r_src = int_issue(src, E);
  const float4 r_s = scalar_issue(s, s, n, F, f0);
  const float4 r_v = vector_issue(v, v, n, F, f0);
  float W[R + 1];
#pragma unroll
  for (int nn = 0; nn < R; ++nn) W[nn] = ldg_pinned(Wd + ((size_t)kf * F + f) * R + nn);
  W[R] = ldg_pinned(bd + (size_t)kf * F + f);
  pin_loads();
  auto commit = [&]() {
    copy4_commit(r_geom, geom_l, E * GS / 4);
    int_commit(r_rp, rp_l, n + 1); int_commit(r_src, src_l, E);
    scalar_commit(r_s, true, s_l, n);
    vector_commit(r_v, true, v_l, n);
  };
  fwd_core<1, 3, 5>(phi_l, red, a1, n, F, W2, row0, commit);
  for (int o = threadIdx.x; o < 16 * 3; o += DL_THREADS) {
    const int m = o / 3, g = o - m * 3;
    float4 p = *reinterpret_cast<float4*>(phi_l + (m * 3 + g) * 4);
    const float4 b = *reinterpret_cast<const float4*>(b2 + (size_t)g * F + f0);
    p.x += b.x; p.y += b.y; p.z += b.z; p.w += b.w;
    *reinterpret_cast<float4*>(phi_l + (m * 3 + g) * 4) = p;
    if (m < n) *reinterpret_cast<float4*>(phi_out + (size_t)m * 3 * F + (size_t)g * F + f0) = p;
  }
  __syncthreads();
  float as = 0.f;
  dv3 acc{0.f, 0.f, 0.f};
  if (k < 3 && (k == 1 || with_dv)) {
    const int e_beg = live ? rp_l[i] : 0, e_end = live ? min(rp_l[i + 1], E) : 0;
    for (int e = e_beg; e < e_end; ++e) {
// ... 78 lines not shown
    const float p_j = live ? p1_l[node * 4 + c] : 0.f;
    const int e_beg = live ? rps_l[node] : 0, e_end = live ? min(rps_l[node + 1], E) : 0;
    for (int e = e_beg; e < e_end; ++e) {
      const float* __restrict__ g = geoms_l + (size_t)e * GS;
      const float gq = gh_l[dsts_l[e] * 4 + c];
      a = fmaf(gq, dfilt<R>(W, g), a);
      const float t = gq * p_j;
#pragma unroll
      for (int nn = 0; nn <= R; ++nn) G[nn] = fmaf(t, g[nn], G[nn]);
    }
    gphi_l[node * 4 + c] = live ? a : 0.f;
#pragma unroll
    for (int nn = 0; nn <= R; ++nn) {
      float x = G[nn];
      x = add_xor32(add_xor16(add_row_stride4(x)));
      G[nn] = x;
    }
    if (lane < 4) {
#pragma unroll
      for (int nn = 0; nn < R; ++nn) gWd[((size_t)F + f) * R + nn] = G[nn];
      gbd[(size_t)F + f] = G[R];
    }
  } else if (k == 1 || k == 2) {
    const int kk = k == 1 ? 0 : 2;
    if (lane < 4) {
#pragma unroll
      for (int nn = 0; nn < R; ++nn) gWd[((size_t)kk * F + f) * R + nn] = 0.f;
      gbd[(size_t)kk * F + f] = 0.f;
    }
  }
  __syncthreads();
  for (int o = threadIdx.x; o < n * 3; o += DL_THREADS) {
    const int m = o / 3, g = o - m * 3;
    const float4 val = g == 1 ? *reinterpret_cast<const float4*>(gphi_l + m * 4) : make_float4(0.f, 0.f, 0.f, 0.f);
    *reinterpret_cast<float4*>(g_phi + (size_t)m * 3 * F + (size_t)g * F + f0) = val;
  }
  bi_core<1, 1, 2>(wr, gphi_l, stage, slices_out + (size_t)blockIdx.x * out_stride, F, n, tr);
}

}

namespace cgv {
static size_t lds_bytes(size_t floats) { return floats * 4 + 512; }
template <typename Kern>
static int allow_lds(Kern kern, size_t bytes) {
  if (bytes <= 64 * 1024) return 0;
  hipError_t e = hipFuncSetAttribute(reinterpret_cast<const void*>(kern), hipFuncAttributeMaxDynamicSharedMemorySize, (int)bytes);
  if (e != hipSuccess) { cgv::set_error("hipFuncSetAttribute(%zu bytes of LDS): %s", bytes, hipGetErrorString(e)); return (int)e; }
  return 0;
}
}

extern "C" {

int cgv_decoder_layer_supported(int n_nodes, int n_feat, int n_rbf) {
  return n_nodes >= 1 && n_nodes <= cgv::DL_MAX_NODES && n_feat >= 16 && (n_feat % 4) == 0 && n_feat <= 864 &&
         cgv_rbf_supported(n_rbf);
}
int cgv_decoder_max_edges(void) { return cgv::DL_MAX_EDGES; }
int cgv_decoder_block_channels(int width) { return (width % 8) == 0 && cgv::option(CGV_OPT_DECODER_FAT) != 0 ? 8 : 4; }
static int cgv_decoder_column_parts(int K, bool heavy = false) {
  const int o = cgv::option(CGV_OPT_DECODER_COLSPLIT), tiles = (K + 63) / 64;
  const int want = o <= 0 ? 1 : o == 1 ? 2 : o == 2 ? (heavy ? 3 : 2) : 3;
  return want < tiles ? want : tiles;
}
int cgv_decoder_debug_clock(uint64_t* buf) {
#if !CGV_DL_CLOCK
  if (buf) { cgv::set_error("this build has no phase clock: rebuild csrc/decoder_layer.hip with -DCGV_DL_CLOCK=1"); return CGV_E_UNSUPPORTED; }
#endif
  unsigned long long* p = reinterpret_cast<unsigned long long*>(buf);
  hipError_t e = hipMemcpyToSymbol(HIP_SYMBOL(cgv::g_dl_clock), &p, sizeof(p));
  return e == hipSuccess ? 0 : (int)e;
}

int64_t cgv_decoder_slice_floats(int K, int rows) { return (int64_t)K * rows; }


#define CGV_DL_QS(n_slices, ...)                                           \
  do {                                                                     \
    if ((n_slices) <= 108) { constexpr int QS = 3; __VA_ARGS__ }           \
    else { constexpr int QS = 6; __VA_ARGS__ }                             \
  } while (0)

#define CGV_DL_CHECK()                                                                                        \
  CGV_REQUIRE(cgv_decoder_layer_supported(n_nodes, n_feat, n_rbf), "unsupported shape (n <= 16 nodes, F % 4 == 0, 16 <= F <= 864)"); \
  hipStream_t st = (hipStream_t)stream;                                                                       \
  const int blocks = n_feat / cgv::DL_CB

int cgv_decoder_msg_fwd(const float* a1, const float* W2, const float* b2, const float* s, const float* sbar, const float* v,
                        const float* vbar, const float* geom_d, const int32_t* rowptr_d, const int32_t* src_d, const float* Wd,
                        const float* bd, float* phi, float* stack, float* sbar_out, float* v_out, float* vbar_out,
                        float* rows_out, int n_nodes, int n_feat, int n_rbf, int n_edges, void* stream) {
  CGV_REQUIRE(a1 && W2 && b2 && s && sbar && v && vbar && geom_d && rowptr_d && src_d && Wd && bd, "null input");
  CGV_REQUIRE(phi && stack && sbar_out && v_out && vbar_out && rows_out, "null output");
  CGV_REQUIRE(n_edges >= 1 && n_edges <= cgv::DL_MAX_EDGES, "the staged bead graph holds 1..cgv_decoder_max_edges() edges");
  CGV_DL_CHECK();
  const size_t base_floats = cgv::fwd_red_floats<1, 9>() + 576 + 1536 + (size_t)cgv::DL_MAX_EDGES * cgv::geom_stride(n_rbf) + 20 +
                             cgv::DL_MAX_EDGES + 128 + 384;
  const bool wlds = cgv::option(CGV_OPT_DECODER_WLDS) != 0 && cgv::lds_bytes(base_floats + (size_t)36 * n_feat) <= 160 * 1024;
  const size_t lds = cgv::lds_bytes(base_floats + (wlds ? (size_t)36 * n_feat : 0));
  CGV_DISPATCH_RBF(n_rbf, {
    if (wlds) {
      if (int rc = cgv::allow_lds(cgv::dec_msg_fwd_k<RBF, true>, lds)) return rc;
      hipLaunchKernelGGL((cgv::dec_msg_fwd_k<RBF, true>), dim3(blocks), dim3(cgv::DL_THREADS), lds, st, a1, W2, b2, s, sbar, v, vbar,
                         geom_d, rowptr_d, src_d, Wd, bd, phi, stack, sbar_out, v_out, vbar_out, rows_out, n_nodes, n_feat, n_edges);
    } else {
      if (int rc = cgv::allow_lds(cgv::dec_msg_fwd_k<RBF, false>, lds)) return rc;
      hipLaunchKernelGGL((cgv::dec_msg_fwd_k<RBF, false>), dim3(blocks), dim3(cgv::DL_THREADS), lds, st, a1, W2, b2, s, sbar, v, vbar,
                         geom_d, rowptr_d, src_d, Wd, bd, phi, stack, sbar_out, v_out, vbar_out, rows_out, n_nodes, n_feat, n_edges);
    }
  });
  return cgv::check_launch("cgv_decoder_msg_fwd");
}

int cgv_prior_msg_fwd(const float* a1, const float* W2, const float* b2, const float* s, const float* v, const float* geom_d,
                      const int32_t* rowptr_d, const int32_t* src_d, const float* Wd, const float* bd, float* phi, float* s_out,
                      float* v_out, int n_nodes, int n_feat, int n_rbf, int n_edges, int with_dv, void* stream) {
  CGV_REQUIRE(a1 && W2 && b2 && s && v && geom_d && rowptr_d && src_d && Wd && bd && phi && s_out && v_out, "null pointer");
  CGV_REQUIRE(n_edges >= 1 && n_edges <= cgv::DL_MAX_EDGES, "the staged bead graph holds 1..cgv_decoder_max_edges() edges");
  CGV_DL_CHECK();
  const size_t lds = cgv::lds_bytes(cgv::fwd_red_floats<1, 3>() + 192 + 384 + (size_t)cgv::DL_MAX_EDGES * cgv::geom_stride(n_rbf) + 20 +
                                    cgv::DL_MAX_EDGES + 64 + 192);
  CGV_DISPATCH_RBF(n_rbf, {
    if (int rc = cgv::allow_lds(cgv::prior_msg_fwd_k<RBF>, lds)) return rc;
    hipLaunchKernelGGL((cgv::prior_msg_fwd_k<RBF>), dim3(blocks), dim3(cgv::DL_THREADS), lds, st, a1, W2, b2, s, v, geom_d, rowptr_d,
                       src_d, Wd, bd, phi, s_out, v_out, n_nodes, n_feat, n_edges, with_dv);
  });
  return cgv::check_launch("cgv_prior_msg_fwd");
}

int cgv_prior_msg_bwd(const float* phi, const float* geom_s, const int32_t* rowptr_s, const int32_t* dst_s, const float* Wd,
                      const float* bd, const float* gh_base, const float* gh_slices, int gh_n_slices, int64_t gh_slice_floats,
                      const float* W2, float* g_phi, float* g_h, float* gWd, float* gbd, float* slices_out,
                      int64_t out_slice_floats, int n_nodes, int n_feat, int n_rbf, int n_edges, void* stream) {
  CGV_REQUIRE(phi && geom_s && rowptr_s && dst_s && Wd && bd && W2 && g_phi && g_h && gWd && gbd && slices_out, "null pointer");
  CGV_REQUIRE((gh_base || gh_slices) && (gh_slices ? gh_n_slices >= 1 && gh_n_slices <= 216 : true), "the upstream gradient: base and / or 1 .. 216 slices");
  CGV_REQUIRE(n_edges >= 1 && n_edges <= cgv::DL_MAX_EDGES, "the staged bead graph holds 1..cgv_decoder_max_edges() edges");
  CGV_DL_CHECK();
  const size_t lds = cgv::lds_bytes(cgv::bi_stage_floats<1>() + 64 + 64 + 64 + 64 + (size_t)cgv::DL_MAX_EDGES * cgv::geom_stride(n_rbf) +
                                    20 + cgv::DL_MAX_EDGES);
  CGV_DISPATCH_RBF(n_rbf, {
    CGV_DL_QS(gh_slices ? gh_n_slices : 1, {
      if (int rc = cgv::allow_lds(cgv::prior_msg_bwd_k<RBF, QS>, lds)) return rc;
      hipLaunchKernelGGL((cgv::prior_msg_bwd_k<RBF, QS>), dim3(blocks), dim3(cgv::DL_THREADS), lds, st, phi, geom_s, rowptr_s, dst_s,
                         Wd, bd, gh_base, gh_slices, gh_n_slices, (long long)gh_slice_floats, W2, g_phi, g_h, gWd, gbd, slices_out,
                         (long long)out_slice_floats, n_nodes, n_feat, n_edges);
    });
  });
  return cgv::check_launch("cgv_prior_msg_bwd");
}

int cgv_decoder_dense_fwd(const float* x, const float* W, const float* bias, float* y, float* z, int n_nodes, int N, int K,
                          int act, void* stream) {
  CGV_REQUIRE(x && W && y, "null pointer");
  CGV_REQUIRE(act >= 0 && act <= cgv::CGV_ACT_MAX, "unknown activation");
  CGV_REQUIRE(n_nodes >= 1 && n_nodes <= cgv::DL_MAX_NODES && (N % 4) == 0 && (K % 4) == 0 && N >= 4 && K >= 4, "unsupported shape");
  hipLaunchKernelGGL(cgv::dec_dense_fwd_k, dim3(N / cgv::DL_CB), dim3(cgv::DL_THREADS), cgv::lds_bytes(cgv::fwd_red_floats<1, 1>() + 64),
                     (hipStream_t)stream, x, W, bias, y, z, n_nodes, N, K, act);
  return cgv::check_launch("cgv_decoder_dense_fwd");
}

int cgv_pair_linear_fwd(const float* x0, const float* x1, const float* W0, const float* W1, const float* bias0,
                        const float* bias1, float* y0, float* y1, float* z0, float* z1, int act0, int act1, int n_rows, int N,
                        int K, void* stream) {
  CGV_REQUIRE(x0 && x1 && W0 && W1 && y0 && y1, "null pointer");
  CGV_REQUIRE(act0 >= 0 && act0 <= cgv::CGV_ACT_MAX && act1 >= 0 && act1 <= cgv::CGV_ACT_MAX, "unknown activation");
  CGV_REQUIRE(n_rows >= 1 && n_rows <= cgv::DL_MAX_NODES && (N % 4) == 0 && (K % 4) == 0 && N >= 4 && K >= 4, "unsupported shape");
  cgv::DensePair p{{x0, x1}, {W0, W1}, {bias0, bias1}, {y0, y1}, {z0, z1}, {act0, act1}};
  hipLaunchKernelGGL(cgv::dec_dense_fwd_pair_k<1>, dim3(N / cgv::DL_CB, 2), dim3(cgv::DL_THREADS),
                     cgv::lds_bytes(cgv::fwd_red_floats<1, 1>() + 64), (hipStream_t)stream, p, n_rows, N, K);
  return cgv::check_launch("cgv_pair_linear_fwd");
}

int cgv_multi_linear_max(void) { return cgv::DL_MULTI_MAX; }

int cgv_multi_linear_fwd(int n, const float* const* x, const float* const* W, const float* const* bias, float* const* y,
                         float* const* z, const int* act, int n_rows, int N, int K, void* stream) {
  CGV_REQUIRE(n >= 1 && n <= cgv::DL_MULTI_MAX && x && W && y && act, "1 .. 4 problems, non-null tables");
  CGV_REQUIRE(n_rows >= 1 && n_rows <= cgv::DL_MAX_NODES && (N % 4) == 0 && (K % 4) == 0 && N >= 4 && K >= 4, "unsupported shape");
  cgv::DensePair p{};
  for (int j = 0; j < n; ++j) {
    CGV_REQUIRE(x[j] && W[j] && y[j], "null pointer");
    CGV_REQUIRE(act[j] >= 0 && act[j] <= cgv::CGV_ACT_MAX && (act[j] == 0 || (z && z[j])), "activation needs its pre-activation buffer");
    p.x[j] = x[j]; p.W[j] = W[j]; p.bias[j] = bias ? bias[j] : nullptr; p.y[j] = y[j]; p.z[j] = z ? z[j] : nullptr; p.act[j] = act[j];
  }
  if ((N % 8) == 0 && (N / cgv::DL_CB) * n > 256)
    hipLaunchKernelGGL(cgv::dec_dense_fwd_pair_k<2>, dim3(N / (2 * cgv::DL_CB), n), dim3(cgv::DL_THREADS),
                       cgv::lds_bytes(cgv::fwd_red_floats<1, 2>() + 128), (hipStream_t)stream, p, n_rows, N, K);
  else
    hipLaunchKernelGGL(cgv::dec_dense_fwd_pair_k<1>, dim3(N / cgv::DL_CB, n), dim3(cgv::DL_THREADS),
                       cgv::lds_bytes(cgv::fwd_red_floats<1, 1>() + 64), (hipStream_t)stream, p, n_rows, N, K);
  return cgv::check_launch("cgv_multi_linear_fwd");
}
// ... 37 lines not shown
  CGV_DL_QS(gs_n_slices, {                                                                                                      \
    if (cgv_decoder_block_channels(n_feat) == 8)                                                                                \
      hipLaunchKernelGGL((cgv::dec_gate_bwd_k<2, QS, NTV>), dim3(n_feat / 8, parts), dim3(cgv::DL_THREADS),                     \
                         cgv::lds_bytes(cgv::bi_stage_floats<1>() + 2 * 2304 + 2 * 64 + 384), st, UV, a, gs_base, gs_slices,   \
                         gs_n_slices, (long long)gs_slice_stride, gv, W1p, ga, gUV, gs_sum, slices_out,                        \
                         (long long)out_slice_stride, n_nodes, n_feat);                                                        \
    else                                                                                                                        \
      hipLaunchKernelGGL((cgv::dec_gate_bwd_k<1, QS, NTV>), dim3(n_feat / 4, parts), dim3(cgv::DL_THREADS),                     \
                         cgv::lds_bytes(cgv::bi_stage_floats<1>() + 2304 + 64 + 192), st, UV, a, gs_base, gs_slices, gs_n_slices, \
                         (long long)gs_slice_stride, gv, W1p, ga, gUV, gs_sum, slices_out, (long long)out_slice_stride, n_nodes, \
                         n_feat);                                                                                               \
  })
  if (one_round) { CGV_DL_GATE(1); } else { CGV_DL_GATE(2); }
#undef CGV_DL_GATE
  return cgv::check_launch("cgv_decoder_gate_bwd");
}
int cgv_decoder_dense_bwd(const float* g_slices, int g_n_slices, int64_t g_slice_stride, const float* z, int act, const float* W,
                          float* g_dense, float* slices_out, int64_t out_slice_stride, int n_nodes, int N, int K, void* stream) {
  CGV_REQUIRE(g_slices && W && g_dense && slices_out && g_n_slices >= 1 && g_n_slices <= 216, "null pointer / slice count");
  CGV_REQUIRE(act == 0 || (act >= 1 && act <= cgv::CGV_ACT_MAX && z), "act != 0 needs the saved pre-activation z");
  CGV_REQUIRE(n_nodes >= 1 && n_nodes <= cgv::DL_MAX_NODES && (N % 4) == 0 && (K % 4) == 0 && K <= 64 * 27 && N >= 4, "unsupported shape");
  CGV_REQUIRE(out_slice_stride >= cgv_decoder_slice_floats(K, n_nodes), "bad slices");
  hipStream_t st = (hipStream_t)stream;
  const int parts = cgv_decoder_column_parts(K);
  const int tiles = ((K + 63) / 64 + parts - 1) / parts;
  const bool fat = cgv_decoder_block_channels(N) == 8;
  const dim3 blocks(fat ? N / 8 : N / 4, parts);
  const size_t lds = cgv::lds_bytes(cgv::bi_stage_floats<1>() + 2 * 2304 + 2 * 64 + 2 * 64);
#define CGV_DL_DENSE(NTV)                                                                                                  \
  CGV_DL_QS(g_n_slices, {                                                                                                  \
    if (fat)                                                                                                               \
      hipLaunchKernelGGL((cgv::dec_dense_bwd_k<NTV, 2, QS>), blocks, dim3(cgv::DL_THREADS), lds, st, g_slices,             \
                         g_n_slices, (long long)g_slice_stride, z, act, W, g_dense, slices_out, (long long)out_slice_stride, \
                         n_nodes, N, K);                                                                                   \
    else                                                                                                                   \
      hipLaunchKernelGGL((cgv::dec_dense_bwd_k<NTV, 1, QS>), blocks, dim3(cgv::DL_THREADS), lds, st, g_slices,             \
                         g_n_slices, (long long)g_slice_stride, z, act, W, g_dense, slices_out, (long long)out_slice_stride, \
                         n_nodes, N, K);                                                                                   \
  })
  if (tiles <= 9) { CGV_DL_DENSE(1); } else if (tiles <= 18) { CGV_DL_DENSE(2); } else { CGV_DL_DENSE(3); }
#undef CGV_DL_DENSE
  return cgv::check_launch("cgv_decoder_dense_bwd");
}

int cgv_decoder_uv_bwd(const float* gstack_slices, int n_slices, int64_t slice_stride, const float* UV, const float* stack,
                       const float* gs_res, const float* Wuv, const float* gUV, float* gUV_out, float* g_s2, float* slices_out,
                       int64_t out_slice_stride, int n_nodes, int n_feat, void* stream) {
  CGV_REQUIRE(gstack_slices && UV && stack && gs_res && Wuv && gUV && gUV_out && g_s2 && slices_out && n_slices >= 1 && n_slices <= 216,
              "null pointer / slice count");
  const int parts = cgv_decoder_column_parts(n_feat, true);
  CGV_REQUIRE(parts == 1 || gUV_out != gUV, "gUV_out may alias gUV only with one block per channel group (CGV_OPT_DECODER_COLSPLIT = 0)");
  CGV_REQUIRE(out_slice_stride >= cgv_decoder_slice_floats(n_feat, 3 * n_nodes), "bad slices");
  const int n_rbf = 8;
  CGV_DL_CHECK();
  (void)blocks;
  const bool one_round = (((n_feat + 63) / 64 + parts - 1) / parts) <= cgv::DL_WAVES;
#define CGV_DL_UV(NTV)                                                                                                          \
  CGV_DL_QS(n_slices, {                                                                                                         \
    if (cgv_decoder_block_channels(n_feat) == 8) {                                                                              \
      const size_t lds = cgv::lds_bytes(cgv::bi_stage_floats<3>() + 2 * 4608 + 2 * 128 + 2 * 384);                              \
      if (int rc = cgv::allow_lds(cgv::dec_uv_bwd_k<2, QS, NTV>, lds)) return rc;                                               \
      hipLaunchKernelGGL((cgv::dec_uv_bwd_k<2, QS, NTV>), dim3(n_feat / 8, parts), dim3(cgv::DL_THREADS), lds, st, gstack_slices, \
                         n_slices, (long long)slice_stride, UV, stack, gs_res, Wuv, gUV, gUV_out, g_s2, slices_out,             \
                         (long long)out_slice_stride, n_nodes, n_feat);                                                        \
    } else {                                                                                                                    \
      const size_t lds = cgv::lds_bytes(cgv::bi_stage_floats<3>() + 4608 + 128 + 384);                                          \
      if (int rc = cgv::allow_lds(cgv::dec_uv_bwd_k<1, QS, NTV>, lds)) return rc;                                               \
      hipLaunchKernelGGL((cgv::dec_uv_bwd_k<1, QS, NTV>), dim3(n_feat / 4, parts), dim3(cgv::DL_THREADS), lds, st, gstack_slices, \
                         n_slices, (long long)slice_stride, UV, stack, gs_res, Wuv, gUV, gUV_out, g_s2, slices_out,             \
                         (long long)out_slice_stride, n_nodes, n_feat);                                                        \
    }                                                                                                                           \
  })
  if (one_round) { CGV_DL_UV(1); } else { CGV_DL_UV(2); }
#undef CGV_DL_UV
  return cgv::check_launch("cgv_decoder_uv_bwd");
}

int cgv_decoder_msg_bwd(const float* phi, const float* s, const float* sbar, const float* v, const float* vbar,
                        const float* geom_d, const int32_t* rowptr_d, const int32_t* src_d, const float* geom_s,
                        const int32_t* rowptr_s, const int32_t* dst_s, const float* Wd, const float* bd, const float* gh,
                        const float* ghb, const float* gvrows_slices, int n_slices, int64_t slice_stride, const float* gv_res,
                        const float* gvb, const float* W2, float* g_phi, float* g_s, float* g_sbar, float* g_v, float* g_vbar,
                        float* gWd, float* gbd, float* slices_out, int64_t out_slice_stride, int n_nodes, int n_feat, int n_rbf,
                        int n_edges, void* stream) {
  CGV_REQUIRE(phi && s && sbar && v && vbar && geom_d && rowptr_d && src_d && geom_s && rowptr_s && dst_s && Wd && bd && W2,
              "null input");
  CGV_REQUIRE(gvrows_slices && n_slices >= 1 && n_slices <= 216 && g_phi && g_s && g_sbar && g_v && g_vbar && gWd && gbd && slices_out,
              "null pointer / slice count");
  CGV_REQUIRE(out_slice_stride >= cgv_decoder_slice_floats(n_feat, n_nodes), "bad slices");
  CGV_REQUIRE(n_edges >= 1 && n_edges <= cgv::DL_MAX_EDGES, "the staged bead graph holds 1..cgv_decoder_max_edges() edges");
  CGV_DL_CHECK();
  const size_t lds = cgv::lds_bytes(cgv::bi_stage_floats<1>() + 192 + 576 + 576 + 3456 + 4608 +
                               2 * (size_t)cgv::DL_MAX_EDGES * cgv::geom_stride(n_rbf) + 40 + 2 * cgv::DL_MAX_EDGES + 256 + 960);
  CGV_DISPATCH_RBF(n_rbf, {
    CGV_DL_QS(n_slices, {
      if (int rc = cgv::allow_lds(cgv::dec_msg_bwd_k<RBF, QS>, lds)) return rc;
      hipLaunchKernelGGL((cgv::dec_msg_bwd_k<RBF, QS>), dim3(blocks), dim3(cgv::DL_THREADS), lds, st, phi, s, sbar, v, vbar, geom_d,
                         rowptr_d, src_d, geom_s, rowptr_s, dst_s, Wd, bd, gh, ghb, gvrows_slices, n_slices,
                         (long long)slice_stride, gv_res, gvb, W2, g_phi, g_s, g_sbar, g_v, g_vbar, gWd, gbd, slices_out,
                         (long long)out_slice_stride, n_nodes, n_feat, n_edges);
    });
  });
  return cgv::check_launch("cgv_decoder_msg_bwd");
}

int cgv_decoder_slices_to_dense(const float* base, const float* slices, int n_slices, int64_t slice_stride, float* out,
                                int n_nodes, int n_feat, void* stream) {
  CGV_REQUIRE(slices && out && n_slices >= 1 && n_slices <= 216 && n_nodes >= 1 && n_nodes <= 16 && (n_feat % 4) == 0, "bad argument");
  CGV_DL_QS(n_slices, {
    hipLaunchKernelGGL((cgv::dec_quad_to_dense_k<QS>), dim3(n_feat / 4), dim3(cgv::DL_THREADS), cgv::lds_bytes(2304 + 64),
                       (hipStream_t)stream, base, slices, n_slices, (long long)slice_stride, out, n_nodes, n_feat);
  });
  return cgv::check_launch("cgv_decoder_slices_to_dense");
}

}
```

coarsegrainingvae_amd/decoder_fused.py:

```python
from __future__ import annotations

from typing import Optional

import torch

from . import _lib
from .ktimer import mark
from .primitives import ACT_NONE, ACT_SWISH, Swish, _grad_target, _is_direct, wgrad_queue, wgrad_sink

_F32 = torch.float32
PER_LAYER = 12
calls = 0


class Slices:
    __slots__ = ("base", "part", "n", "stride")

    def __init__(self, base: Optional[torch.Tensor] = None, part: Optional[torch.Tensor] = None, n: int = 0, stride: int = 0):
        self.base, self.part, self.n, self.stride = base, part, (n if part is not None else 0), stride


def layer_params(decoder):
    flat = []
    for mb, ub in zip(decoder.message_blocks, decoder.update_blocks):
        im = mb.inv_message
        Wd, bd = im.dist_embed.filter_params()
        d0, d1 = ub.s_dense[0], ub.s_dense[1]
        flat += [im.inv_dense[0].weight, im.inv_dense[0].bias, im.inv_dense[1].weight, im.inv_dense[1].bias, Wd, bd,
                 ub.u_mat.weight, ub.v_mat.weight, d0.weight, d0.bias, d1.weight, d1.bias]
    return flat


def staged_edges(plan) -> int:
    return max(1, min(int(plan.capacity), int(_lib.load().cgv_decoder_max_edges())))


def usable(decoder, S: torch.Tensor, plan, geom) -> bool:
    from .ops import _adjacent
    if not (S.is_cuda and S.dtype == _F32 and len(decoder.message_blocks) > 0 and geom is not None):
        return False
    n, F = S.shape
    lib = _lib.load()
    if not lib.cgv_decoder_layer_supported(n, F, geom.n_rbf):
        return False
    ok = lambda M, N, K: bool(lib.cgv_skinny_supported(M, N, K))
    if not (ok(n, F, F) and ok(n, F, 2 * F)):
        return False
    if plan.n_dst != n or plan.n_src != n or not 1 <= plan.n_edges <= lib.cgv_decoder_max_edges():
        return False
    for mb, ub in zip(decoder.message_blocks, decoder.update_blocks):
        im = mb.inv_message
        d = (im.inv_dense[0], im.inv_dense[1], ub.s_dense[0], ub.s_dense[1])
        if not (isinstance(d[0].activation, Swish) and d[1].activation is None and isinstance(d[2].activation, Swish)
                and d[3].activation is None and all(x.dropout_rate == 0.0 for x in d)):
            return False
        if im.n_rbf != geom.n_rbf or any(x.bias is None for x in d) or ub.u_mat.bias is not None or ub.v_mat.bias is not None:
            return False
    params = layer_params(decoder)
    if not all(_is_direct(p) and p.grad.is_contiguous() and p.is_contiguous() and p.data_ptr() % 16 == 0 for p in params):
        return False
    for l in range(len(decoder.message_blocks)):
        Wu, Wv = params[PER_LAYER * l + 6], params[PER_LAYER * l + 7]
        if not (_adjacent(Wu, Wv) and _adjacent(Wu.grad, Wv.grad)):
            return False
    return True


class _PseudoDecoderFn(torch.autograd.Function):

    @staticmethod
    def forward(ctx, S, Sbar0, V0, plan, geom, hooks, n_layers, *flat):
        from .ops import _dense_fwd
        S = S.contiguous()
        n, F = S.shape
        R = geom.n_rbf
        dev, st = S.device, _lib.stream_ptr()
        new = lambda *shape: torch.empty(*shape, dtype=_F32, device=dev)
        Sbar, V, Vbar = Sbar0, V0, V0
        saved = []
        n_stage = staged_edges(plan)
        from .options import HOST
        if HOST["decoder_dense"] == 1:
            dense = _dense_fwd
        else:
            dense = lambda x, W, b, y, z, M, N, K, act, st_: _lib.call("cgv_decoder_dense_fwd", _lib.ptr(x), _lib.ptr(W), _lib.ptr(b),
                                                                      _lib.ptr(y), _lib.ptr(z), M, N, K, act, st_)
        for l in range(n_layers):
            W1, b1, W2, b2, Wd, bd, Wu, Wv, W0, b0, W1p, b1p = (t.detach() for t in flat[PER_LAYER * l: PER_LAYER * (l + 1)])
            Wuv = torch.as_strided(Wu, (2 * F, F), (F, 1))
            a1, z1, phi, stack = new(n, F), new(n, F), new(n, 9 * F), new(n, 2 * F)
            dense(S, W1, b1, a1, z1, n, F, F, ACT_SWISH, st)
            Sbar2, V2, Vbar2, rows = new(n, F), new(n, F, 3), new(n, F, 3), new(3 * n, F)
            _lib.call("cgv_decoder_msg_fwd", _lib.ptr(a1), _lib.ptr(W2), _lib.ptr(b2), _lib.ptr(S), _lib.ptr(Sbar), _lib.ptr(V),
                      _lib.ptr(Vbar), _lib.ptr(geom.geom_d), _lib.ptr(plan.rowptr_d), _lib.ptr(plan.src_d), _lib.ptr(Wd),
                      _lib.ptr(bd), _lib.ptr(phi), _lib.ptr(stack), _lib.ptr(Sbar2), _lib.ptr(V2), _lib.ptr(Vbar2), _lib.ptr(rows),
                      n, F, R, n_stage, st, tag=f"pseudo_msg_fwd:Nd{n}:E{plan.n_edges}:dv1")
            UV = new(3 * n, 2 * F)
            _lib.call("cgv_decoder_uv_fwd", _lib.ptr(rows), _lib.ptr(Wuv), _lib.ptr(UV), _lib.ptr(stack), n, F, st)
            z0, a0, a = new(n, F), new(n, F), new(n, 3 * F)
            dense(stack, W0, b0, a0, z0, n, F, 2 * F, ACT_SWISH, st)
            S3, V3 = new(n, F), new(n, F, 3)
            _lib.call("cgv_decoder_gate_fwd", _lib.ptr(a0), _lib.ptr(W1p), _lib.ptr(b1p), _lib.ptr(UV), _lib.ptr(stack),
                      _lib.ptr(V2), _lib.ptr(a), _lib.ptr(S3), _lib.ptr(V3), n, F, st)
            saved.append((S, Sbar, V, Vbar, z1, a1, phi, rows, UV, stack, z0, a0, a))
            S, Sbar, V, Vbar = S3, Sbar2, V3, Vbar2
            mark(f"decoder:fwd{l}")
        ctx.saved, ctx.flat, ctx.plan, ctx.geom, ctx.hooks, ctx.n_layers = saved, flat, plan, geom, hooks, n_layers
        ctx.set_materialize_grads(False)
        return S, V

    @staticmethod
    def backward(ctx, gS_out, gV_out):
        n_layers, flat, plan, geom = ctx.n_layers, ctx.flat, ctx.plan, ctx.geom
        if gS_out is None and gV_out is None:
            return (None,) * (7 + len(flat))
        saved, ctx.saved = ctx.saved, None
        n, F = saved[0][0].shape
        R = geom.n_rbf
        dev, st = saved[0][0].device, _lib.stream_ptr()
        new = lambda *shape: torch.empty(*shape, dtype=_F32, device=dev)
        lib = _lib.load()
        nb = F // 4
        fl16 = lambda K: int(lib.cgv_decoder_slice_floats(K, n))
        fl48 = int(lib.cgv_decoder_slice_floats(F, 3 * n))
        gS = Slices(gS_out.contiguous() if gS_out is not None else None)
        gV = gV_out.contiguous() if gV_out is not None else None
        gSbar = gVbar = None
        n_stage = staged_edges(plan)
        mark("backward:loss+tail")
        for l in range(n_layers - 1, -1, -1):
            pW1, pb1, pW2, pb2, pWd, pbd, pWu, pWv, pW0, pb0, pW1p, pb1p = flat[PER_LAYER * l: PER_LAYER * (l + 1)]
            S_in, Sbar_in, V_in, Vbar_in, z1, a1, phi, rows, UV, stack, z0, a0, a = saved[l]
            saved[l] = None
            Wuv = torch.as_strided(pWu.detach(), (2 * F, F), (F, 1))
            ga, gUV1, gs_sum = new(n, 3 * F), new(3 * n, 2 * F), new(n, F)
            nF = F // int(lib.cgv_decoder_block_channels(F))
            p1 = new(nF * fl16(F))
            _lib.call("cgv_decoder_gate_bwd", _lib.ptr(UV), _lib.ptr(a), _lib.ptr(gS.base), _lib.ptr(gS.part), gS.n, gS.stride,
                      _lib.ptr(gV), _lib.ptr(pW1p.detach()), _lib.ptr(ga), _lib.ptr(gUV1), _lib.ptr(gs_sum), _lib.ptr(p1), fl16(F),
                      n, F, st)
            g_a0 = new(n, F)
            p2 = new(nF * fl16(2 * F))
            _lib.call("cgv_decoder_dense_bwd", _lib.ptr(p1), nF, fl16(F), _lib.ptr(z0), ACT_SWISH, _lib.ptr(pW0.detach()),
                      _lib.ptr(g_a0), _lib.ptr(p2), fl16(2 * F), n, F, 2 * F, st)
            g_s2, gUV = new(n, F), new(3 * n, 2 * F)
            p3 = new(nF * fl48)
            _lib.call("cgv_decoder_uv_bwd", _lib.ptr(p2), nF, fl16(2 * F), _lib.ptr(UV), _lib.ptr(stack), _lib.ptr(gs_sum),
                      _lib.ptr(Wuv), _lib.ptr(gUV1), _lib.ptr(gUV), _lib.ptr(g_s2), _lib.ptr(p3), fl48, n, F, st)
            g_phi = new(n, 9 * F)
            g_s, g_sbar, g_v, g_vbar = new(n, F), new(n, F), new(n, F, 3), new(n, F, 3)
            tWd, accWd, _ = _grad_target(pWd, pWd)
            tbd, accbd, _ = _grad_target(pbd, pbd)
            if accWd or accbd:
                raise RuntimeError("a decoder layer's filter parameters received a second gradient in one step")
            p4 = new(nb * fl16(F))
            _lib.call("cgv_decoder_msg_bwd", _lib.ptr(phi), _lib.ptr(S_in), _lib.ptr(Sbar_in), _lib.ptr(V_in), _lib.ptr(Vbar_in),
                      _lib.ptr(geom.geom_d), _lib.ptr(plan.rowptr_d), _lib.ptr(plan.src_d), _lib.ptr(geom.geom_s),
                      _lib.ptr(plan.rowptr_s), _lib.ptr(plan.dst_s), _lib.ptr(pWd.detach()), _lib.ptr(pbd.detach()),
                      _lib.ptr(g_s2), _lib.ptr(gSbar), _lib.ptr(p3), nF, fl48, _lib.ptr(gV), _lib.ptr(gVbar), _lib.ptr(pW2.detach()),
                      _lib.ptr(g_phi), _lib.ptr(g_s), _lib.ptr(g_sbar), _lib.ptr(g_v), _lib.ptr(g_vbar), _lib.ptr(tWd), _lib.ptr(tbd),
                      _lib.ptr(p4), fl16(F), n, F, R, n_stage, st, tag=f"pseudo_msg_bwd:Nd{n}:E{plan.n_edges}:gv1")
            g_a1 = new(n, F)
            p5 = new(nF * fl16(F))
            _lib.call("cgv_decoder_dense_bwd", _lib.ptr(p4), nb, fl16(F), _lib.ptr(z1), ACT_SWISH, _lib.ptr(pW1.detach()),
                      _lib.ptr(g_a1), _lib.ptr(p5), fl16(F), n, F, F, st)

            wgrad_sink(pW1p, pb1p, ga, a0, None, ACT_NONE, (n, 3 * F, F), exch=False, flush=False)
            wgrad_sink(pW0, pb0, g_a0, stack, z0, ACT_SWISH, (n, F, 2 * F), exch=False, flush=False)
            wgrad_sink(pWu, None, gUV, rows, None, ACT_NONE, (3 * n, 2 * F, F), exch=False, stacked=pWv, flush=False)
            wgrad_sink(pW2, pb2, g_phi, a1, None, ACT_NONE, (n, 9 * F, F), flush=False)
            wgrad_sink(pW1, pb1, g_a1, S_in, z1, ACT_SWISH, (n, F, F), flush=False)
            gS = Slices(g_s, p5, nF, fl16(F))
            gV, gSbar, gVbar = g_v, g_sbar, g_vbar
            mark(f"decoder:bwd{l}")
            if ctx.hooks and l in ctx.hooks:
                ctx.hooks[l]()
        gS_in = new(n, F)
        _lib.call("cgv_decoder_slices_to_dense", _lib.ptr(gS.base), _lib.ptr(gS.part), gS.n, gS.stride, _lib.ptr(gS_in), n, F, st)
        if not wgrad_queue.active:
            wgrad_queue.flush()
        return (gS_in, None, None, None, None, None, None) + (None,) * len(flat)


def pseudo_decoder(decoder, S, Sbar0, V0, plan, geom, layer_hooks=None):
    global calls
    calls += 1
    flat = layer_params(decoder)
    return _PseudoDecoderFn.apply(S, Sbar0, V0, plan, geom, layer_hooks or None, len(decoder.message_blocks), *flat)
```

coarsegrainingvae_amd/model.py:

```python
from __future__ import annotations

from typing import Optional

import torch
from torch import nn

from . import ops
from .ktimer import mark
from .options import HOST
from .blocks import (ContractiveMessageBlock, contractive_pair, EquiMessageBlock, EquiMessageCross, EquiMessagePsuedo, PseudoUpdateBlock,
                     UpdateBlock)
from .graph import BatchGraph, EdgePlan, make_directed
from .primitives import (ACT_STD_ENC, ACT_STD_PRIOR, Dense, DistanceEmbed, Linear, MLPHead, dual_heads, mark_direct_grad, quad_heads,
                         to_module)


def _call_then_pass(fn):
    def hook(grad):
        fn()
        return grad
    return hook


_CONSTANTS = {}


def _constant(shape, value: float, device) -> torch.Tensor:
    key = (tuple(shape), float(value), str(device))
    t = _CONSTANTS.get(key)
    if t is None:
        t = _CONSTANTS[key] = torch.full(tuple(shape), float(value), dtype=torch.float32, device=device)
    return t


class EquivariantDecoder(nn.Module):

    def __init__(self, n_atom_basis, n_rbf, cutoff, num_conv, activation, cross_flag=True):
        super().__init__()
        block = EquiMessageCross if cross_flag else EquiMessageBlock
        self.message_blocks = nn.ModuleList(
            [block(feat_dim=n_atom_basis, activation=activation, n_rbf=n_rbf, cutoff=cutoff, dropout=0.0)
             for _ in range(num_conv)])
        self.update_blocks = nn.ModuleList(
            [UpdateBlock(feat_dim=n_atom_basis, activation=activation, dropout=0.0) for _ in range(num_conv)])
        self.n_atom_basis = n_atom_basis
        self.n_rbf, self.cutoff = n_rbf, cutoff

    def forward(self, cg_xyz, CG_nbr_list, mapping, H, graph: Optional[BatchGraph] = None, layer_hooks=None):
        if graph is not None:
            nbrs, plan = graph.cg_nbrs, graph.cg
            geom = graph.geometry("cg", self.n_rbf, self.cutoff)
            r_ij = None
        else:
            nbrs, _ = make_directed(CG_nbr_list)
            plan = EdgePlan.from_nbrs(nbrs, H.shape[0])
            r_ij = cg_xyz[nbrs[:, 1]] - cg_xyz[nbrs[:, 0]]
            from .graph import EdgeGeometry
            geom = EdgeGeometry(plan, self.n_rbf, self.cutoff, r_edges=r_ij)
        n, F = H.shape
        V = _constant((n, F, 3), 0.0, H.device)
        for layer, (message_block, update_block) in enumerate(zip(self.message_blocks, self.update_blocks)):
            if layer_hooks and layer in layer_hooks and H.requires_grad:
                H = H.view_as(H)
                H.register_hook(_call_then_pass(layer_hooks[layer]))
            H, V = message_block(H, V, r_ij, nbrs, plan=plan, geom=geom, residual=True)
            H, V = update_block(H, V, residual=True)
        return H, V


class EquivariantPsuedoDecoder(nn.Module):

    def __init__(self, n_atom_basis, n_rbf, cutoff, num_conv, activation, breaksym=False):
        super().__init__()
        self.message_blocks = nn.ModuleList(
            [EquiMessagePsuedo(feat_dim=n_atom_basis, activation=activation, n_rbf=n_rbf, cutoff=cutoff, dropout=0.0)
             for _ in range(num_conv)])
        self.update_blocks = nn.ModuleList(
            [UpdateBlock(feat_dim=n_atom_basis, activation=activation, dropout=0.0) for _ in range(num_conv)])
        self.pseudo_update_blocks = nn.ModuleList(
            [PseudoUpdateBlock(feat_dim=n_atom_basis, activation=activation, dropout=0.0) for _ in range(num_conv)])
        self.breaksym = breaksym
        self.n_atom_basis = n_atom_basis
        self.n_rbf, self.cutoff = n_rbf, cutoff
        self.fused_loop = True

    def forward(self, cg_xyz, CG_nbr_list, mapping, S, graph: Optional[BatchGraph] = None, layer_hooks=None):
        if graph is not None:
            nbrs, plan = graph.cg_nbrs, graph.cg
            geom = graph.geometry("cg", self.n_rbf, self.cutoff)
            r_ij = None
        else:
            nbrs, _ = make_directed(CG_nbr_list)
            plan = EdgePlan.from_nbrs(nbrs, S.shape[0])
            r_ij = cg_xyz[nbrs[:, 1]] - cg_xyz[nbrs[:, 0]]
            geom = None
        n, F = S.shape
        V = _constant((n, F, 3), 0.0, S.device)
        Sbar = _constant((n, F), 1.0 if self.breaksym else 0.0, S.device)
        Vbar = V
        if self.fused_loop and geom is not None and S.requires_grad:
            from . import decoder_fused
            if decoder_fused.usable(self, S, plan, geom):
                return decoder_fused.pseudo_decoder(self, S, Sbar, V, plan, geom, layer_hooks)
        for layer, (message_block, update_block) in enumerate(zip(self.message_blocks, self.update_blocks)):
            if layer_hooks and layer in layer_hooks and S.requires_grad:
                S = S.view_as(S)
                S.register_hook(_call_then_pass(layer_hooks[layer]))
            if geom is None:
                from .graph import EdgeGeometry
                geom = EdgeGeometry(plan, self.n_rbf, self.cutoff, r_edges=r_ij)
            S, Sbar, V, Vbar = message_block(S, Sbar, V, Vbar, r_ij, nbrs, plan=plan, geom=geom, residual=True)
            S, V = update_block(S, V, residual=True)
        return S, V


class EquiEncoder(nn.Module):

    def __init__(self, n_conv, n_atom_basis, n_rbf, activation, cutoff, dir_mp=False, cg_mp=False):
        super().__init__()
        F = n_atom_basis
        self.atom_embed = nn.Embedding(100, F, padding_idx=0)
        mark_direct_grad(self.atom_embed.weight)
        mk_msg = lambda: EquiMessageBlock(feat_dim=F, activation=activation, n_rbf=n_rbf, cutoff=cutoff, dropout=0.0)
        mk_upd = lambda: UpdateBlock(feat_dim=F, activation=activation, dropout=0.0)
        self.dist_embed = DistanceEmbed(n_rbf=n_rbf, cutoff=cutoff, feat_dim=F, dropout=0.0)
        self.message_blocks = nn.ModuleList([mk_msg() for _ in range(n_conv)])
        self.update_blocks = nn.ModuleList([mk_upd() for _ in range(n_conv)])
        self.cg_message_blocks = nn.ModuleList([mk_msg() for _ in range(n_conv)])
        self.cg_update_blocks = nn.ModuleList([mk_upd() for _ in range(n_conv)])
        self.cgmessage_layers = nn.ModuleList(
            [ContractiveMessageBlock(feat_dim=F, activation=activation, n_rbf=n_rbf, cutoff=20.0, dropout=0.0)
             for _ in range(n_conv)])
        self.atom2CGcouplings = nn.ModuleList(
            [nn.Sequential(Dense(in_features=F, out_features=F, bias=True, activation=to_module(activation)),
                           Dense(in_features=F, out_features=F, bias=True)) for _ in range(n_conv)])
        self.n_conv, self.dir_mp, self.cg_mp, self.n_atom_basis = n_conv, dir_mp, cg_mp, F
        self.n_rbf, self.cutoff = n_rbf, cutoff
        self.skip_dead_vector_channel = False

    def set_skip_dead_vector_channel(self, flag: bool):
        self.skip_dead_vector_channel = bool(flag)
        for blk in list(self.message_blocks) + list(self.cgmessage_layers):
            blk.with_dv = not flag

    def forward(self, z, xyz, cg_xyz, mapping, nbr_list, cg_nbr_list, graph: Optional[BatchGraph] = None, layer_hooks=None, h0=None):
        if graph is None:
            graph = BatchGraph(xyz, cg_xyz, mapping, nbr_list, cg_nbr_list, dir_mp=self.dir_mp)
        elif bool(self.dir_mp) != bool(getattr(graph, "dir_mp", False)):
            raise RuntimeError(f"this encoder has dir_mp={self.dir_mp}: prepare the batch with prepare_batch(..., dir_mp={self.dir_mp})")
        geom = graph.geometry("atom", self.n_rbf, self.cutoff)
        geom_c = graph.geometry("a2b", self.n_rbf, 20.0)
        h = h0 if h0 is not None else ops.embedding(self.atom_embed, z, graph.embed_plan("atom", z, self.atom_embed) if graph is not None else None)
        v = _constant((h.shape[0], h.shape[1], 3), 0.0, h.device)
        H = V = None
        phi_next = None
        hooked = False
        for i in range(self.n_conv):
            h_in = h
            if layer_hooks and i in layer_hooks and h.requires_grad and not hooked:
                h_in = h.view_as(h)
                h_in.register_hook(_call_then_pass(layer_hooks[i]))
            hooked = False
            h, v = self.message_blocks[i](h_in, v, None, graph.atom_nbrs, plan=graph.atom, geom=geom, residual=True, phi=phi_next)
            phi_next = None
            if HOST["encoder_pairs"] and i + 1 < self.n_conv and (i > 0 or HOST["fused_bead_mean"]):
                h_pair = h
                if layer_hooks and (i + 1) in layer_hooks and h.requires_grad:
                    h_pair = h.view_as(h)
                    h_pair.register_hook(_call_then_pass(layer_hooks[i + 1]))
                out = contractive_pair(self.cgmessage_layers[i], self.message_blocks[i + 1], h_pair, v, graph.mapping, graph.a2b, geom_c,
                                       (H, V) if H is not None else None, mean_init=H is None)
                if out is not None:
                    H, V, h, phi_next = out
                    hooked = h_pair is not h_in and layer_hooks is not None and (i + 1) in layer_hooks
                    continue
                if h_pair is not h:
                    h, hooked = h_pair, True
            if i == 0 and not HOST["fused_bead_mean"]:
                H = ops.scatter_mean(h, graph.mapping, plan=graph.a2b)
                V = ops.scatter_mean(v, graph.mapping, plan=graph.a2b)
            H, V, h = self.cgmessage_layers[i](h, v, None, graph.mapping, plan=graph.a2b, geom=geom_c,
                                               residual=(H, V) if H is not None else None, chain=True, mean_init=H is None)
        return H, h


class CGprior(nn.Module):
# ... 216 lines not shown
```

include/cgvae_hip.h:

```cpp
#ifndef CGVAE_HIP_H
#define CGVAE_HIP_H

#include <stddef.h>
#include <stdint.h>

#ifdef __cplusplus
extern "C" {
#endif

#define CGV_VERSION 101

#define CGV_E_BADARG (-1)
#define CGV_E_UNSUPPORTED (-2)
#define CGV_E_WORKSPACE (-3)

int cgv_version(void);
const char* cgv_last_error_string(void);

enum {
  CGV_OPT_MSG_FWD_SPLIT = 0,
  CGV_OPT_MSG_BWD_SPLIT = 1,
  CGV_OPT_CSR_BUILD = 2,
  CGV_OPT_PSEUDO_CHUNKS = 3,
  CGV_OPT_WGRAD_TILING = 4,
  CGV_OPT_TILE_FWD_LDS_MIN = 5,
  CGV_OPT_BWD_INPUT_WAVES = 6,
  CGV_OPT_PSEUDO_FWD = 7,
  CGV_OPT_DECODER_FAT = 8,
  CGV_OPT_DECODER_WLDS = 9,
  CGV_OPT_SKINNY_ROWS = 10,
  CGV_OPT_TILE_FWD_BAL = 11,
  CGV_OPT_OPTIM_ONE_LAUNCH = 12,
  CGV_OPT_DECODER_COLSPLIT = 13,
  CGV_OPT_DECODER_NODESPLIT = 14,
  CGV_OPT_BWD_INPUT_SPLIT = 15,
  CGV_OPT_MSG_BWD_MFMA = 16,
  CGV_OPT_STREAMK = 17,
  CGV_OPT_COUNT = 18
};
int cgv_timestamp(uint64_t* slot , void* stream);
int cgv_timestamp_hz(void);
int cgv_sustained_clock_probe(uint64_t* out , float* sink , int blocks, int iters, void* stream);
int cgv_set_option(int option, int value);
int cgv_get_option(int option);
int cgv_reset_options(void);

int cgv_rbf_supported(int n_rbf);
int cgv_geom_stride(int n_rbf);
int cgv_geom_unit_offset(int n_rbf);

int cgv_radius_graph_count(const float* xyz , const int32_t* frame_ptr ,
                           int n_frames, int n_nodes, float s_star, int undirected,
                           int32_t* counts , int32_t* offsets , void* stream);
int cgv_radius_graph_emit(const float* xyz, const int32_t* frame_ptr, int n_frames, int n_nodes, float s_star,
                          int undirected, const int32_t* offsets , int64_t* nbr_out ,
                          void* stream);

size_t cgv_csr_workspace_bytes(int n_edges);
int cgv_csr_build(const int64_t* dst, const int64_t* src, int stride, int n_edges, int n_dst, int n_src,
                  int32_t* rowptr_d, int32_t* eid_d, int32_t* dst_d, int32_t* src_d,
                  int32_t* rowptr_s, int32_t* eid_s, int32_t* dst_s, int32_t* src_s,
                  void* workspace, size_t workspace_bytes, void* stream);
size_t cgv_group_plan_workspace_bytes(int n_edges);
int cgv_group_plan_build(const int32_t* rowptr_d , const int32_t* dst_d, const int32_t* src_d, int n_edges,
                         int n_dst, int n_src, int rb, int32_t* dst_g, int32_t* src_g, int32_t* pos_g,
                         int32_t* meta_g , void* workspace, size_t workspace_bytes, void* stream);
size_t cgv_group_plan_radix_workspace_bytes(int n_edges);
int cgv_group_plan_build_radix(const int32_t* dst_d, const int32_t* src_d, int n_edges, int n_dst, int n_src, int rb,
                               int32_t* dst_g, int32_t* src_g, int32_t* pos_g , int32_t* meta_g ,
                               void* workspace, size_t workspace_bytes, void* stream);

int cgv_edge_geometry(const float* r_edges , const int32_t* eid ,
                      const float* pos_dst , const float* pos_src ,
                      const int32_t* dst , const int32_t* src , int n_edges, int n_rbf,
                      float cutoff, const float* coef , float* geom , void* stream);
int cgv_geom_group_stride(int n_rbf);
int cgv_geom_group_unit_offset(int n_rbf);
int cgv_edge_geometry_grouped(const float* pos_dst , const float* pos_src , const int32_t* dst_g,
                              const int32_t* src_g, const int32_t* meta_g , int n_edges, int n_rbf,
                              float cutoff, const float* coef , float* geom_g , void* stream);

int cgv_segment_reduce(const float* src, const int32_t* rowptr, const int32_t* perm, int n_seg, int channels,
                       int mean, float* out , void* stream);
int cgv_segment_reduce2(const float* src_a, int channels_a, float* out_a, const float* src_b, int channels_b, float* out_b,
                        const int32_t* rowptr, const int32_t* perm, int n_seg, int mean, void* stream);
int cgv_segment_broadcast(const float* gout, const int32_t* rowptr, const int32_t* perm, int n_seg, int channels,
                          int mean, float* gsrc , void* stream);
int cgv_pair_linear_fwd(const float* x0, const float* x1, const float* W0, const float* W1, const float* bias0,
                        const float* bias1, float* y0, float* y1, float* z0, float* z1, int act0, int act1, int n_rows, int N,
                        int K, void* stream);
int cgv_pair_linear_bwd_input(const float* gy0, const float* gy1, const float* z0, const float* z1, const float* W0,
                              const float* W1, int act0, int act1, float* gx0, float* gx1, int M, int N, int K, void* ws,
                              size_t ws_bytes, void* stream);
int cgv_multi_linear_max(void);
int cgv_multi_linear_fwd(int n, const float* const* x, const float* const* W, const float* const* bias, float* const* y,
                         float* const* z, const int* act, int n_rows, int N, int K, void* stream);
int cgv_multi_linear_bwd_input(int n, int group, const float* const* gy, const float* const* z, const float* const* W,
                               const int* act, float* const* gx, int M, int N, int K, void* ws, size_t ws_bytes, void* stream);
int cgv_reparam_sample(const float* mu, const float* sigma, float* eps, float* z, int64_t n, uint64_t* rng, void* stream);
int cgv_reparam_bwd(const float* g, const float* eps, const float* k_mu, const float* k_sigma, float* g_mu, float* g_sigma,
                    int64_t n, void* stream);
int cgv_embedding_rows(const float* weight , const float* ids_f32, int id_stride, int n_rows, int n_types,
                       int channels, float* out , void* stream);
int cgv_embedding_rows2(const float* weight_a, const float* ids_a, int id_stride_a, int n_rows_a, int n_types_a, float* out_a,
                        const float* weight_b, const float* ids_b, int id_stride_b, int n_rows_b, int n_types_b, float* out_b,
                        int channels, void* stream);
int cgv_segment_reduce_pair(const float* src_a, const int32_t* rowptr_a, const int32_t* perm_a, int n_seg_a, float* out_a,
                            const float* src_b, const int32_t* rowptr_b, const int32_t* perm_b, int n_seg_b, float* out_b,
                            int channels, void* stream);

int cgv_equi_msg_fwd(const float* phi , const float* v , const float* geom_d,
                     const int32_t* rowptr_d, const int32_t* src_d, const float* Wd ,
                     const float* bd , float* ds , float* dv , int n_dst,
                     int n_feat, int n_rbf, int with_dv, int64_t n_edges_hint, int64_t n_rows_hint,
                     const float* s_res , const float* v_res , void* stream);
int cgv_equi_msg_grouped_supported(int n_feat, int n_rbf, int rb);
int cgv_equi_msg_fwd_grouped(const float* phi , const float* v , const float* geom_g,
                             const int32_t* rowptr_d, const int32_t* src_g,
                             const float* Wd , const float* bd , float* ds ,
                             float* dv , int n_dst, int n_feat, int n_rbf, int rb, int64_t n_rows,
                             int64_t n_edges , const float* s_res , const float* v_res ,
                             void* stream);
size_t cgv_equi_msg_bwd_workspace_bytes(int n_src, int n_feat, int n_rbf);
int cgv_equi_msg_bwd(const float* phi, const float* v, const float* geom_s, const int32_t* rowptr_s,
                     const int32_t* dst_s, const float* Wd, const float* bd, const float* gs ,
                     const float* gv , float* g_phi, float* g_v, float* gWd, float* gbd,
                     int n_src, int n_feat, int n_rbf, int64_t n_edges_hint, int64_t n_rows_hint, void* workspace,
                     size_t workspace_bytes, void* stream);
int cgv_equi_msg_bwd_deferred(const float* phi, const float* v, const float* geom_s, const int32_t* rowptr_s,
                              const int32_t* dst_s, const float* Wd, const float* bd, const float* gs, const float* gv,
                              float* g_phi, float* g_v, int n_src, int n_feat, int n_rbf, int64_t n_edges_hint,
                              int64_t n_rows_hint, void* workspace, size_t workspace_bytes, int* n_chunks, int* k_live,
                              void* stream);
int cgv_filter_reduce_jobs_max(void);
int cgv_filter_reduce_job_bytes(void);
int cgv_filter_reduce_jobs(const void* jobs_host, int n_jobs, void* stream);

int cgv_batch_load_rows(const float* src_atoms, float* dst_atoms, float* xyz_atoms, int n_atoms, const float* src_beads,
                        float* dst_beads, float* xyz_beads, int n_beads, void* stream);
int cgv_plan_jobs_max(void);
int cgv_plan_job_bytes(void);
int cgv_plan_jobs_build(const void* jobs_host, int n_jobs, void* stream);
int cgv_geom_jobs_max(void);
int cgv_geom_job_bytes(void);
int cgv_geom_jobs_build(const void* jobs_host, int n_jobs, void* stream);

int cgv_pseudo_msg_fwd(const float* phi , const float* s, const float* sbar, const float* v,
                       const float* vbar, const float* geom_d, const int32_t* rowptr_d, const int32_t* src_d,
                       const float* Wd , const float* bd , float* dh, float* dhbar, float* dv,
                       float* dvbar, int n_nodes, int n_feat, int n_rbf, int residual, void* stream);
int cgv_pseudo_msg_fwd_rows(const float* phi, const float* s, const float* sbar, const float* v, const float* vbar,
                            const float* geom_d, const int32_t* rowptr_d, const int32_t* src_d, const float* Wd,
                            const float* bd, float* dh, float* dhbar, float* dv, float* dvbar, float* dv_rows,
                            int n_nodes, int n_feat, int n_rbf, int residual, int64_t n_edges_hint ,
                            void* stream);
size_t cgv_pseudo_msg_bwd_workspace_bytes(int n_nodes, int n_feat, int n_rbf);
int cgv_pseudo_msg_bwd(const float* phi, const float* s, const float* sbar, const float* v, const float* vbar,
                       const float* geom_d, const int32_t* rowptr_d, const int32_t* src_d,
                       const float* geom_s, const int32_t* rowptr_s, const int32_t* dst_s,
                       const float* Wd, const float* bd,
                       const float* gh, const float* ghbar, const float* gv, const float* gvbar,
                       float* g_phi , float* g_s, float* g_sbar, float* g_v, float* g_vbar,
                       float* gWd , float* gbd , int n_nodes, int n_feat, int n_rbf,
                       int residual, int64_t n_edges_hint , void* workspace,
                       size_t workspace_bytes, void* stream);
int cgv_pseudo_msg_bwd_deferred(const float* phi, const float* s, const float* sbar, const float* v, const float* vbar,
                                const float* geom_d, const int32_t* rowptr_d, const int32_t* src_d, const float* geom_s,
                                const int32_t* rowptr_s, const int32_t* dst_s, const float* Wd, const float* bd, const float* gh,
                                const float* ghbar, const float* gv, const float* gvbar, float* g_phi, float* g_s, float* g_sbar,
                                float* g_v, float* g_vbar, int n_nodes, int n_feat, int n_rbf, int residual,
                                int64_t n_edges_hint, void* workspace, size_t workspace_bytes, int* n_chunks , void* stream);

int cgv_decoder_layer_supported(int n_nodes, int n_feat, int n_rbf);
int64_t cgv_decoder_slice_floats(int K, int rows);
int cgv_decoder_max_edges(void);
int cgv_decoder_block_channels(int width);
int cgv_decoder_debug_clock(uint64_t* buf );
int cgv_decoder_msg_fwd(const float* a1, const float* W2, const float* b2, const float* s, const float* sbar, const float* v,
                        const float* vbar, const float* geom_d, const int32_t* rowptr_d, const int32_t* src_d, const float* Wd,
                        const float* bd, float* phi, float* stack, float* sbar_out, float* v_out, float* vbar_out,
                        float* rows_out, int n_nodes, int n_feat, int n_rbf, int n_edges, void* stream);
int cgv_prior_msg_fwd(const float* a1, const float* W2, const float* b2, const float* s, const float* v, const float* geom_d,
                      const int32_t* rowptr_d, const int32_t* src_d, const float* Wd, const float* bd, float* phi, float* s_out,
                      float* v_out, int n_nodes, int n_feat, int n_rbf, int n_edges, int with_dv, void* stream);
int cgv_prior_msg_bwd(const float* phi, const float* geom_s, const int32_t* rowptr_s, const int32_t* dst_s, const float* Wd,
                      const float* bd, const float* gh_base, const float* gh_slices, int gh_n_slices, int64_t gh_slice_floats,
                      const float* W2, float* g_phi, float* g_h, float* gWd, float* gbd, float* slices_out,
                      int64_t out_slice_floats, int n_nodes, int n_feat, int n_rbf, int n_edges, void* stream);
int cgv_decoder_dense_fwd(const float* x, const float* W , const float* bias, float* y, float* z, int n_nodes, int N,
                          int K, int act, void* stream);
int cgv_decoder_uv_fwd(const float* rows, const float* Wuv, float* UV, float* stack, int n_nodes, int n_feat, void* stream);
int cgv_decoder_gate_fwd(const float* a0, const float* W1p, const float* b1p, const float* UV, const float* stack,
                         const float* v2, float* a, float* s3, float* v3, int n_nodes, int n_feat, void* stream);
int cgv_decoder_gate_bwd(const float* UV, const float* a, const float* gs_base , const float* gs_slices ,
                         int gs_n_slices, int64_t gs_slice_stride, const float* gv , const float* W1p, float* ga,
                         float* gUV, float* gs_sum, float* slices_out, int64_t out_slice_stride, int n_nodes, int n_feat,
                         void* stream);
int cgv_decoder_dense_bwd(const float* g_slices, int g_n_slices, int64_t g_slice_stride, const float* z , int act,
                          const float* W, float* g_dense, float* slices_out, int64_t out_slice_stride, int n_nodes, int N, int K,
                          void* stream);
int cgv_decoder_uv_bwd(const float* gstack_slices, int n_slices, int64_t slice_stride, const float* UV, const float* stack,
                       const float* gs_res, const float* Wuv, const float* gUV, float* gUV_out, float* g_s2, float* slices_out,
                       int64_t out_slice_stride, int n_nodes, int n_feat, void* stream);
int cgv_decoder_msg_bwd(const float* phi, const float* s, const float* sbar, const float* v, const float* vbar,
                        const float* geom_d, const int32_t* rowptr_d, const int32_t* src_d, const float* geom_s,
                        const int32_t* rowptr_s, const int32_t* dst_s, const float* Wd, const float* bd, const float* gh,
                        const float* ghb , const float* gvrows_slices, int n_slices, int64_t slice_stride,
                        const float* gv_res , const float* gvb , const float* W2, float* g_phi, float* g_s,
                        float* g_sbar, float* g_v, float* g_vbar, float* gWd, float* gbd, float* slices_out,
                        int64_t out_slice_stride, int n_nodes, int n_feat, int n_rbf, int n_edges, void* stream);
int cgv_decoder_slices_to_dense(const float* base , const float* slices, int n_slices, int64_t slice_stride,
                                float* out, int n_nodes, int n_feat, void* stream);

int cgv_update_rows_from_vec(const float* v , float* rows , int n_nodes, int n_feat, void* stream);
int cgv_update_vec_from_rows(const float* rows, const float* res , float* vec, int n_nodes, int n_feat,
                             void* stream);
int cgv_update_norm_stack_fwd(const float* s , const float* Vv, float* stack , int n_nodes, int n_feat,
                              int ld, void* stream);
int cgv_update_norm_stack_bwd(const float* gstack, const float* Vv, const float* stack, const float* g_res ,
                              float* g_s, float* gVv, int n_nodes, int n_feat, int ld, int accumulate, void* stream);
int cgv_update_gate_fwd(const float* U, const float* Vv, const float* a, const float* s_res ,
                        const float* v_res , float* ds , float* dv ,
                        int n_nodes, int n_feat, int ld, void* stream);
int cgv_update_gate_bwd(const float* U, const float* Vv, const float* a, const float* g_ds, const float* g_dv,
                        float* gU, float* gVv, float* ga, int n_nodes, int n_feat, int ld, void* stream);

int cgv_skinny_max_rows(void);
int cgv_skinny_supported(int M, int N, int K);
int cgv_skinny_fwd_supported(int M, int N, int K);
int cgv_skinny_linear_fwd(const float* x, const float* W, const float* bias, float* y, float* z , int M, int N,
                          int K, int act, void* stream);
int cgv_skinny_bwd_input_supported(int M, int N, int K);
size_t cgv_skinny_bwd_input_workspace_bytes(int M, int N, int K);
int cgv_skinny_linear_bwd_input(const float* gy, const float* z , const float* W, float* gx, int M, int N, int K,
                                int act, void* ws , size_t ws_bytes, void* stream);
int cgv_skinny_linear_bwd_input_add(const float* gy, const float* z , const float* W, const float* add, float* gx,
                                    int M, int N, int K, int act, void* workspace, size_t workspace_bytes, void* stream);
int cgv_skinny_linear_bwd_input_out(const float* gy, const float* z , const float* W, const float* add ,
                                    float* gx, int M, int N, int K, int act, const float* z_out, int act_out, void* workspace,
                                    size_t workspace_bytes, void* stream);
int cgv_dense_grad_prepare(const float* gy, const float* z , float* g_out , float* gb ,
                           int M, int N, int act, int accumulate, void* stream);
int cgv_tile_supported(int M, int N, int K);
int cgv_tile_linear_fwd(const float* x, const float* W, const float* bias , float* y, float* z , int M,
                        int N, int K, int act, void* stream);
int cgv_tile_linear_bwd_input(const float* g, const float* W, float* gx, int M, int N, int K, void* stream);
int cgv_tile_linear_bwd_input_act(const float* gy, const float* z , const float* W, float* gx, int M, int N, int K,
                                  int act, void* stream);
int cgv_tile_linear_bwd_input_act_add(const float* gy, const float* z , const float* W, const float* add, float* gx,
                                      int M, int N, int K, int act, void* stream);
int cgv_tile_linear_bwd_input_act_add_bcast(const float* gy, const float* z, const float* W, const float* add, const float* seg_grad,
                                            const int64_t* row2seg, const int32_t* seg_rowptr, int mean, float* gx, int M, int N,
                                            int K, int act, void* stream);

int cgv_tile_pair_supported(int M, int N, int K);
int cgv_tile_pair_linear_fwd(const float* x_a, const float* W_a, const float* bias_a, float* y_a, float* z_a, const float* x_b,
                             const float* W_b, const float* bias_b, float* y_b, float* z_b, int M, int N, int K, int act_a,
                             int act_b, void* stream);
int cgv_tile_pair_linear_bwd_input(const float* gy_a, const float* z_a, const float* W_a, const float* add_a, float* gx_a,
                                   const float* gy_b, const float* z_b, const float* W_b, const float* add_b, float* gx_b, int M,
                                   int N, int K, int act_a, int act_b, void* stream);
int cgv_tile_linear_bwd_input_norm_stack(const float* gy, const float* z, const float* W, int M, int N, int K, int act,
                                         const float* stack, const float* Vv, const float* g_res, float* g_s, float* gVv, int ld,
                                         int accumulate, void* stream);
int cgv_tile_bwd_input_plan(int M, int N, int K, int np, int* shares , int* streamk );
int cgv_tile_bwd_input_split(void* workspace, size_t workspace_bytes, void* stream);
int cgv_tile_linear_bwd_input_out(const float* gy, const float* z, const float* W, const float* add, float* gx, int M, int N,
                                  int K, int act, const float* z_out, int act_out, void* stream);
int cgv_tile_pair_linear_bwd_input_out(const float* gy_a, const float* z_a, const float* W_a, const float* add_a, float* gx_a,
                                       const float* gy_b, const float* z_b, const float* W_b, const float* add_b, float* gx_b,
                                       int M, int N, int K, int act_a, int act_b, const float* z_out_a, int act_out_a,
                                       const float* z_out_b, int act_out_b, void* stream);
int cgv_tile_linear_bwd_input_sum2(const float* gy_a, const float* z_a, const float* W_a, const float* gy_b, const float* z_b,
                                   const float* W_b, const float* add, const float* seg_grad, const int64_t* row2seg,
                                   const int32_t* seg_rowptr, int mean, float* gx, int M, int N, int K, int act_a, int act_b,
                                   void* stream);
int cgv_tile_linear_wgrad(const float* g, const float* x, float* gW, int M, int N, int K, int accumulate, void* stream);
int cgv_wgrad_record_bytes(void);
int cgv_wgrad_plan(int M, int N, int K, int* tiles_k , int* tile_w , int* n_blocks );
int cgv_wgrad_lds_floats(int M, int tile_w);
int cgv_grouped_wgrad(const void* table_dev, int n_problems, int total_blocks, int max_lds_floats, void* stream);
int cgv_wgrad_gathered_plan(int M, int N, int K, int seg_rows, int* tiles_k , int* n_blocks );
int cgv_grouped_wgrad_gathered(const void* table_dev, int n_problems, int total_blocks, void* stream);
int cgv_wgrad_gathered_plan_tile(int M, int N, int K, int seg_rows, int tile, int* tiles_k , int* n_blocks );
int cgv_grouped_wgrad_gathered_tile(const void* table_dev, int n_problems, int total_blocks, int tile, void* stream);
int cgv_grouped_wgrad_split(const void* table_dev, int n_problems, int total_blocks, void* stream);
int cgv_grouped_wgrad_gathered_sumsq(const void* table_dev, int n_problems, int total_blocks, double* partial, double* sumsq,
                                     void* stream);
int cgv_grouped_wgrad_gathered_adam(const void* table_dev, int n_problems, int total_blocks, const float* arena_g,
                                    float* arena_p, float* arena_m, float* arena_v, float lr, float beta1, float beta2,
                                    float eps, const float* state, void* stream);
int cgv_wgrad_strip_max_rows(void);
int cgv_wgrad_strip_plan(int M, int N, int K, int seg_rows, int* n_blocks );
// ... 292 lines not shown
```

Baseline: 1283.

## Specialize decoder message kernels per layer to skip structurally-zero channel blocks

Adds compile-time layer variants (first/last) to the decoder message forward and backward kernels. Channel blocks whose inputs are known to be zero in the first layers (product-state input) or whose outputs are unused in the last layer are masked out: their weight loads, GEMM columns, edge loops and sbar/vbar stores are skipped, and phi is zero-filled for them. The goal is to cut redundant GEMM and edge work in the fused decoder. It adds more template instantiations, and correctness relies on the product-state assumption, which is now enabled by default in model.py. It also pins cross/dot products to explicit fma ordering.

```diff
diff --git a/coarsegrainingvae_amd/_lib.py b/coarsegrainingvae_amd/_lib.py
--- a/coarsegrainingvae_amd/_lib.py
+++ b/coarsegrainingvae_amd/_lib.py
@@ -98,7 +98,7 @@
     "cgv_decoder_max_edges": (_i, []),
     "cgv_decoder_block_channels": (_i, [_i]),
     "cgv_decoder_debug_clock": (_i, [_p]),
-    "cgv_decoder_msg_fwd": (_i, [_p] * 18 + [_i, _i, _i, _i, _p]),
+    "cgv_decoder_msg_fwd": (_i, [_p] * 18 + [_i, _i, _i, _i, _p, _i]),
     "cgv_decoder_dense_fwd": (_i, [_p, _p, _p, _p, _p, _i, _i, _i, _i, _p]),
     "cgv_prior_msg_fwd": (_i, [_p] * 13 + [_i, _i, _i, _i, _i, _p]),
     "cgv_prior_msg_bwd": (_i, [_p] * 8 + [_i, C.c_int64] + [_p] * 6 + [C.c_int64, _i, _i, _i, _i, _p]),
@@ -107,7 +107,7 @@
     "cgv_decoder_gate_bwd": (_i, [_p, _p, _p, _p, _i, C.c_int64, _p, _p, _p, _p, _p, _p, C.c_int64, _i, _i, _p]),
     "cgv_decoder_dense_bwd": (_i, [_p, _i, C.c_int64, _p, _i, _p, _p, _p, C.c_int64, _i, _i, _i, _p]),
     "cgv_decoder_uv_bwd": (_i, [_p, _i, C.c_int64, _p, _p, _p, _p, _p, _p, _p, _p, C.c_int64, _i, _i, _p]),
-    "cgv_decoder_msg_bwd": (_i, [_p] * 15 + [_p, _i, C.c_int64, _p, _p, _p] + [_p] * 8 + [C.c_int64, _i, _i, _i, _i, _p]),
+    "cgv_decoder_msg_bwd": (_i, [_p] * 15 + [_p, _i, C.c_int64, _p, _p, _p] + [_p] * 8 + [C.c_int64, _i, _i, _i, _i, _p, _i]),
     "cgv_decoder_slices_to_dense": (_i, [_p, _p, _i, C.c_int64, _p, _i, _i, _p]),
     "cgv_dense_grad_prepare": (_i, [_p, _p, _p, _p, _i, _i, _i, _i, _p]),
     "cgv_tile_supported": (_i, [_i, _i, _i]),
@@ -295,7 +295,7 @@
 OPTIONS = {"msg_fwd_split": 0, "msg_bwd_split": 1, "csr_build": 2, "pseudo_chunks": 3, "wgrad_tiling": 4, "tile_fwd_lds_min": 5,
            "bwd_input_waves": 6, "pseudo_fwd": 7, "decoder_fat": 8, "decoder_wlds": 9, "skinny_rows": 10, "tile_fwd_bal": 11,
            "optim_one_launch": 12, "decoder_colsplit": 13, "decoder_nodesplit": 14, "bwd_input_split": 15, "msg_bwd_mfma": 16,
-           "streamk": 17}
+           "streamk": 17, "decoder_all_live": 18}
 
 
 def set_option(name: str, value: int) -> None:
diff --git a/coarsegrainingvae_amd/csrc/api.cpp b/coarsegrainingvae_amd/csrc/api.cpp
--- a/coarsegrainingvae_amd/csrc/api.cpp
+++ b/coarsegrainingvae_amd/csrc/api.cpp
@@ -18,7 +18,8 @@
      0,   0,         1,
      1,      0,        1,
      0,  2,   1,
-     -1,  -1,      0};
+     -1,  -1,      0,
+     0};
 static_assert(sizeof(g_opt_default) == CGV_OPT_COUNT * sizeof(int), "one default per CGV_OPT_*");
 static std::atomic<int> g_opt[CGV_OPT_COUNT];
 static void reset_options() {
diff --git a/coarsegrainingvae_amd/csrc/decoder_layer.hip b/coarsegrainingvae_amd/csrc/decoder_layer.hip
--- a/coarsegrainingvae_amd/csrc/decoder_layer.hip
+++ b/coarsegrainingvae_amd/csrc/decoder_layer.hip
@@ -36,12 +36,32 @@
 constexpr int DL_THREADS = 64 * DL_WAVES;
 constexpr int DL_MAX_NODES = 16;
 
+constexpr unsigned DL_LIVE_ALL = 0x1ffu;
+constexpr unsigned DL_DEAD_FIRST = (1u << 3) | (1u << 4) | (1u << 5) | (1u << 8);
+constexpr unsigned DL_DEAD_LAST = (1u << 5) | (1u << 6) | (1u << 7) | (1u << 8);
+constexpr unsigned dl_live_mask(int variant) {
+  return DL_LIVE_ALL & ~(((variant & CGV_DECODER_FIRST) ? DL_DEAD_FIRST : 0u) | ((variant & CGV_DECODER_LAST) ? DL_DEAD_LAST : 0u));
+}
+constexpr int dl_count(unsigned mask) { int c = 0; for (int b = 0; b < 9; ++b) c += (mask >> b) & 1; return c; }
+template <unsigned MASK>
+__host__ __device__ __forceinline__ constexpr int dl_nth_block(int idx) {
+  int res = -1, seen = 0;
+#pragma unroll
+  for (int b = 0; b < 9; ++b)
+    if ((MASK >> b) & 1) { if (res < 0 || seen == idx) res = b; ++seen; }
+  return res;
+}
+
 struct dv3 { float x, y, z; };
 __device__ __forceinline__ dv3 dldv(const float* p) { f3 t = ld3(p); return dv3{t.x, t.y, t.z}; }
 __device__ __forceinline__ dv3 dcross(const dv3& a, const dv3& b) {
-  return dv3{a.y * b.z - a.z * b.y, a.z * b.x - a.x * b.z, a.x * b.y - a.y * b.x};
-}
-__device__ __forceinline__ float ddot(const dv3& a, const dv3& b) { return a.x * b.x + a.y * b.y + a.z * b.z; }
+#pragma clang fp contract(off)
+  return dv3{fmaf(a.y, b.z, -(a.z * b.y)), fmaf(a.z, b.x, -(a.x * b.z)), fmaf(a.x, b.y, -(a.y * b.x))};
+}
+__device__ __forceinline__ float ddot(const dv3& a, const dv3& b) {
+#pragma clang fp contract(off)
+  return fmaf(a.z, b.z, fmaf(a.y, b.y, a.x * b.x));
+}
 __device__ __forceinline__ void daxpy(dv3& acc, float a, const dv3& x) {
   acc.x = fmaf(a, x.x, acc.x); acc.y = fmaf(a, x.y, acc.y); acc.z = fmaf(a, x.z, acc.z);
 }
@@ -199,14 +219,15 @@
   }
 }
 
-template <int SLOT, int G, int NT>
+template <int SLOT, int G, int NT, unsigned MASK = ~0u>
 __device__ __forceinline__ void bi_prefetch_slot(BiRegs<G, NT>& r, gcf W, int K, const int (&row0)[G], int tile) {
   const int lane = threadIdx.x & 63;
   const int j = lane & 15, q = lane >> 4;
   const int col = tile * 64 + 4 * j;
   const int cc = col < K ? col : 0;
 #pragma unroll
-  for (int g = 0; g < G; ++g) r.w[SLOT][g] = ldg4_stream(W + (size_t)(row0[g] + q) * K + cc);
+  for (int g = 0; g < G; ++g)
+    if ((MASK >> g) & 1) r.w[SLOT][g] = ldg4_stream(W + (size_t)(row0[g] + q) * K + cc);
 }
 
 #ifndef CGV_DL_SLICE_STORE
@@ -224,7 +245,7 @@
 template <int MB>
 __host__ __device__ constexpr size_t bi_stage_floats() { return (size_t)DL_WAVES * 16 * 16 * MB * 4; }
 
-template <int MB, int G, int NT, int NPRE = NT>
+template <int MB, int G, int NT, int NPRE = NT, unsigned MASK = ~0u>
 __device__ __forceinline__ void bi_core(const BiRegs<G, NPRE>& r, const float* __restrict__ g_tile ,
                                         float* __restrict__ stage ,
                                         float* __restrict__ slice , int K, int rows, const TileRange& tr,
@@ -247,10 +268,12 @@
       const int col = tile * 64 + 4 * j;
       const int cc = col < K ? col : 0;
 #pragma unroll
-      for (int g = 0; g < G; ++g) late[g] = *reinterpret_cast<const float4*>(W + (size_t)(row0[g] + q) * K + cc);
+      for (int g = 0; g < G; ++g)
+        if ((MASK >> g) & 1) late[g] = *reinterpret_cast<const float4*>(W + (size_t)(row0[g] + q) * K + cc);
     }
 #pragma unroll
     for (int g = 0; g < G; ++g) {
+      if (!((MASK >> g) & 1)) continue;
       const float4 w = t < NPRE ? r.w[t < NPRE ? t : 0][g] : late[g];
 #pragma unroll
       for (int mb = 0; mb < MB; ++mb) {
@@ -356,11 +379,12 @@
   if (ph >= 0) DL_PH(ph, 4);
 }
 
-template <int G>
+template <int G, unsigned MASK = ~0u>
 __device__ __forceinline__ void wlds_issue(float* __restrict__ w_l, const float* __restrict__ W, int K, const int (&row0)[G]) {
   const int lane = threadIdx.x & 63, wave = __builtin_amdgcn_readfirstlane(threadIdx.x >> 6);
 #pragma unroll
   for (int g = 0; g < G; ++g) {
+    if (!((MASK >> g) & 1)) continue;
     if ((g % DL_WAVES) != wave) continue;
     const float* src = W + (size_t)row0[g] * K;
     for (int u = 0; u * 64 < K; ++u) {
@@ -385,10 +409,11 @@
     b[u] = *reinterpret_cast<const float4*>(xrow + ((s_beg + u < s_end && k < K) ? k : 0));
   }
 }
-template <int G>
+template <int G, unsigned MASK = (1u << G) - 1>
 __device__ __forceinline__ void fwd_core_wlds_finish(float* __restrict__ out, float* __restrict__ red, const float4 (&b)[WLDS_SB],
                                                      int K, const float* __restrict__ w_l, int ph = -1) {
-  constexpr int T = (G + 3) / 4, SB = WLDS_SB;
+  constexpr int GL = dl_count(MASK), T = (GL + 3) / 4, SB = WLDS_SB;
+  constexpr bool ALL = MASK == (1u << G) - 1;
   const int lane = threadIdx.x & 63, wave = __builtin_amdgcn_readfirstlane(threadIdx.x >> 6);
   const int i = lane & 15, q = lane >> 4;
   const int steps = (K + 15) / 16, per = (steps + DL_WAVES - 1) / DL_WAVES;
@@ -402,7 +427,8 @@
   for (int t = 0; t < T; ++t) acc[t] = f32x4{0.f, 0.f, 0.f, 0.f};
   int wrow[T];
 #pragma unroll
-  for (int t = 0; t < T; ++t) wrow[t] = (min(t * 4 + (i >> 2), G - 1) * 4 + (i & 3)) * K;
+  for (int t = 0; t < T; ++t)
+    wrow[t] = ((ALL ? min(t * 4 + (i >> 2), G - 1) : dl_nth_block<MASK>(t * 4 + (i >> 2))) * 4 + (i & 3)) * K;
 #pragma unroll
   for (int u = 0; u < SB; ++u) {
     const int k = (s_beg + u) * 16 + 4 * q;
@@ -431,7 +457,7 @@
     float v = 0.f;
 #pragma unroll
     for (int w = 0; w < DL_WAVES; ++w) v += red[((w * T + t) * 4 + r) * 64 + l];
-    if (g < G) out[(m * G + g) * 4 + r] = v;
+    if (g < GL) out[(m * GL + g) * 4 + r] = v;
   }
   __syncthreads();
   if (ph >= 0) DL_PH(ph, 4);
@@ -486,7 +512,7 @@
 }
 __device__ __forceinline__ dv3 lds_v3(const float* p) { return dv3{p[0], p[1], p[2]}; }
 
-template <int R, bool WLDS>
+template <int R, bool WLDS, int VAR>
 __global__ __launch_bounds__(DL_THREADS) void dec_msg_fwd_k(
     const float* __restrict__ a1, const float* __restrict__ W2, const float* __restrict__ b2, const float* __restrict__ s_,
     const float* __restrict__ sbar_, const float* __restrict__ v_, const float* __restrict__ vbar_,
@@ -495,6 +521,9 @@
     float* __restrict__ sbar_out, float* __restrict__ v_out, float* __restrict__ vbar_out, float* __restrict__ rows_out,
     int n, int F, int E) {
   constexpr int GS = geom_stride(R), U = geom_unit_offset(R);
+  constexpr unsigned MASK = dl_live_mask(VAR);
+  constexpr int GL = dl_count(MASK);
+  constexpr bool BAR = !(VAR & CGV_DECODER_LAST);
   Carve cv;
   float* red = cv.take(fwd_red_floats<1, 9>());
   float* phi_l = cv.take(16 * 9 * 4);
@@ -511,10 +540,13 @@
   const int i = lane >> 2, c = lane & 3;
   const bool live = i < n;
   const int f = f0 + c;
+  const bool alive = (MASK >> k) & 1;
+  const int kr = __builtin_popcount(MASK & ((1u << k) - 1));
+  const int kw = alive ? k : 0;
   int row0[9];
 #pragma unroll
   for (int g = 0; g < 9; ++g) row0[g] = g * F + f0;
-  if (WLDS) wlds_issue<9>(w_l, W2, F, row0);
+  if (WLDS) wlds_issue<9, MASK>(w_l, W2, F, row0);
   DL_PH(1, 0);
   DL_SPAN(1, 0);
   const gcf geom = launder(geom_); const gci rowptr = launder(rowptr_); const gci src = launder(src_);
@@ -537,26 +569,38 @@
   const int r_ids = ldgi_pinned((k < 4 ? src : rowptr) + min(id_item, id_cnt - 1));
   float W[R + 1];
 #pragma unroll
-  for (int nn = 0; nn < R; ++nn) W[nn] = ldg_pinned(Wd + ((size_t)k * F + f) * R + nn);
-  W[R] = ldg_pinned(bd + (size_t)k * F + f);
+  for (int nn = 0; nn < R; ++nn) W[nn] = ldg_pinned(Wd + ((size_t)kw * F + f) * R + nn);
+  W[R] = ldg_pinned(bd + (size_t)kw * F + f);
   pin_loads();
   float4 xb[WLDS_SB];
   if (WLDS) wlds_x_issue(xb, a1, n, F);
-  else fwd_core<1, 9, 5>(phi_l, red, a1, n, F, W2, row0, NoHook(), 1);
+  else {
+    int rowL[GL];
+#pragma unroll
+    for (int gl = 0; gl < GL; ++gl) rowL[gl] = dl_nth_block<MASK>(gl) * F + f0;
+    fwd_core<1, GL, 5>(phi_l, red, a1, n, F, W2, rowL, NoHook(), 1);
+  }
   {
     copy4_commit(r_geom, geom_l, n4);
     float* dst = k == 0 ? (half == 0 ? s_l : sb_l) : k == 1 ? v_l : vb_l;
     if (k <= 2 && sm_item < sm_cnt) reinterpret_cast<float4*>(dst)[sm_item] = r_small;
     if (k <= 4 && id_item < id_cnt) (k < 4 ? src_l : rp_l)[id_item] = r_ids;
   }
-  if (WLDS) fwd_core_wlds_finish<9>(phi_l, red, xb, F, w_l, 1);
-  for (int o = threadIdx.x; o < 16 * 9; o += DL_THREADS) {
-    const int m = o / 9, g = o - m * 9;
-    float4 p = *reinterpret_cast<float4*>(phi_l + (m * 9 + g) * 4);
+  if (WLDS) fwd_core_wlds_finish<9, MASK>(phi_l, red, xb, F, w_l, 1);
+  for (int o = threadIdx.x; o < 16 * GL; o += DL_THREADS) {
+    const int m = o / GL, gl = o - m * GL;
+    const int g = MASK == DL_LIVE_ALL ? gl : dl_nth_block<MASK>(gl);
+    float4 p = *reinterpret_cast<float4*>(phi_l + (m * GL + gl) * 4);
     const float4 b = *reinterpret_cast<const float4*>(b2 + (size_t)g * F + f0);
     p.x += b.x; p.y += b.y; p.z += b.z; p.w += b.w;
-    *reinterpret_cast<float4*>(phi_l + (m * 9 + g) * 4) = p;
+    *reinterpret_cast<float4*>(phi_l + (m * GL + gl) * 4) = p;
     if (m < n) *reinterpret_cast<float4*>(phi_out + (size_t)m * 9 * F + (size_t)g * F + f0) = p;
+  }
+  if constexpr (GL < 9) {
+    for (int o = threadIdx.x; o < n * (9 - GL); o += DL_THREADS) {
+      const int m = o / (9 - GL), g = dl_nth_block<DL_LIVE_ALL & ~MASK>(o - m * (9 - GL));
+      *reinterpret_cast<float4*>(phi_out + (size_t)m * 9 * F + (size_t)g * F + f0) = make_float4(0.f, 0.f, 0.f, 0.f);
+    }
   }
   __syncthreads();
   DL_PH(1, 5);
@@ -568,14 +612,14 @@
   const float* __restrict__ vsrc = (k == 2 || k == 6 || k == 7) ? v_l : vb_l;
   const int e_beg = live ? rp_l[i] : 0, e_end = live ? min(rp_l[i + 1], E) : 0;
   int j_nx = e_beg < e_end ? src_l[e_beg] : 0;
-  for (int e = e_beg; e < e_end; ++e) {
+  for (int e = e_beg; alive && e < e_end; ++e) {
     const int j = j_nx;
     j_nx = src_l[min(e + 1, e_end - 1)];
     const float* __restrict__ g = geom_l + (size_t)e * GS;
     const dv3 vj = lds_v3(vsrc + (j * 4 + c) * 3);
-    const float q = phi_l[(j * 9 + k) * 4 + c] * dfilt<R>(W, g);
+    const float q = phi_l[(j * GL + kr) * 4 + c] * dfilt<R>(W, g);
     switch (k) {
-      case 0: ah = fmaf(q, s_i, ah); ahb += ddot(v_i, vj); break;
+      case 0: ah = fmaf(q, s_i, ah); if (BAR) ahb += ddot(v_i, vj); break;
       case 1: daxpy(acc, q, dv3{g[U], g[U + 1], g[U + 2]}); break;
       case 2: daxpy(acc, q, vj); break;
       case 3: daxpy(acc, q, dcross(v_i, vj)); break;
@@ -600,9 +644,11 @@
   avb.x += vb_i.x; avb.y += vb_i.y; avb.z += vb_i.z;
   const size_t nf = (size_t)i * F + f;
   stack[(size_t)i * 2 * F + f] = ah;
-  sbar_out[nf] = ahb;
   st3(v_out + nf * 3, av.x, av.y, av.z);
-  st3(vbar_out + nf * 3, avb.x, avb.y, avb.z);
+  if (BAR) {
+    sbar_out[nf] = ahb;
+    st3(vbar_out + nf * 3, avb.x, avb.y, avb.z);
+  }
   rows_out[((size_t)3 * i + 0) * F + f] = av.x;
   rows_out[((size_t)3 * i + 1) * F + f] = av.y;
   rows_out[((size_t)3 * i + 2) * F + f] = av.z;
@@ -953,7 +999,7 @@
   DL_SPAN(7, 1);
 }
 
-template <int R, int QS>
+template <int R, int QS, int VAR>
 __global__ __launch_bounds__(DL_THREADS) void dec_msg_bwd_k(
     const float* __restrict__ phi_, const float* __restrict__ s_, const float* __restrict__ sbar_, const float* __restrict__ v_,
     const float* __restrict__ vbar_, const float* __restrict__ geom_d_, const int* __restrict__ rowptr_d_,
@@ -965,6 +1011,7 @@
     float* __restrict__ g_vbar, float* __restrict__ gWd, float* __restrict__ gbd, float* __restrict__ slices_out,
     long long out_stride, int n, int F, int E) {
   constexpr int GS = geom_stride(R), U = geom_unit_offset(R);
+  constexpr unsigned MASK = dl_live_mask(VAR);
   Carve cv;
   float* stage = cv.take(bi_stage_floats<1>());
   float4* scratch = reinterpret_cast<float4*>(stage);
@@ -1005,6 +1052,8 @@
   const int node = lane >> 2, c = lane & 3, f = f0 + c;
   const bool live = node < n;
   const int nc = live ? node : 0;
+  const bool alive = (MASK >> k) & 1;
+  const int kw = alive ? k : 0;
   const int n4 = E * GS / 4;
   Slots4<geom_slots(R)> r_gd, r_gs;
 #pragma unroll
@@ -1035,8 +1084,8 @@
   const int r_ids = ldgi_pinned(id_src + min(id_item, id_cnt - 1));
   float W[R + 1], G[R + 1];
 #pragma unroll
-  for (int nn = 0; nn < R; ++nn) W[nn] = ldg_pinned(Wd + ((size_t)k * F + f) * R + nn);
-  W[R] = ldg_pinned(bd + (size_t)k * F + f);
+  for (int nn = 0; nn < R; ++nn) W[nn] = ldg_pinned(Wd + ((size_t)kw * F + f) * R + nn);
+  W[R] = ldg_pinned(bd + (size_t)kw * F + f);
 #pragma unroll
   for (int nn = 0; nn <= R; ++nn) G[nn] = 0.f;
   QuadRegs<3, 1, QS> qr;
@@ -1060,7 +1109,7 @@
   DL_WV(2);
   BiRegs<9, 2> wr;
   const TileRange tr{0, (F + 63) / 64};
-  bi_prefetch_slot<0>(wr, W2, F, row0, dl_tile_of(tr, wave, 0));
+  bi_prefetch_slot<0, 9, 2, MASK>(wr, W2, F, row0, dl_tile_of(tr, wave, 0));
   pin_loads();
   quad_finish<3, 1>(qr, gvr_l, scratch, gvr_n, 3 * n, 8);
   if (threadIdx.x < 64) {
@@ -1072,7 +1121,7 @@
   __syncthreads();
   DL_PH(8, 4);
   if (dl_tile_of(tr, wave, 1) < tr.end) {
-    bi_prefetch_slot<1>(wr, W2, F, row0, dl_tile_of(tr, wave, 1));
+    bi_prefetch_slot<1, 9, 2, MASK>(wr, W2, F, row0, dl_tile_of(tr, wave, 1));
   } else {
 #pragma unroll
     for (int g = 0; g < 9; ++g) wr.w[1][g] = make_float4(0.f, 0.f, 0.f, 0.f);
@@ -1093,7 +1142,7 @@
     const float* __restrict__ pS = k == 0 ? gh_l : sb_l;
     const int e_beg = live ? rps_l[node] : 0, e_end = live ? min(rps_l[node + 1], E) : 0;
     int i_nx = e_beg < e_end ? dsts_l[e_beg] : 0;
-    for (int e = e_beg; e < e_end; ++e) {
+    for (int e = e_beg; alive && e < e_end; ++e) {
       const float* __restrict__ g = geoms_l + (size_t)e * GS;
       const int ic = i_nx * 4 + c;
       i_nx = dsts_l[min(e + 1, e_end - 1)];
@@ -1148,7 +1197,7 @@
   }
   float as = 0.f, asb = 0.f;
   dv3 rv{0.f, 0.f, 0.f}, rvb{0.f, 0.f, 0.f};
-  if (k == 0 || k == 1 || k == 3 || k == 4 || k == 6 || k == 7 || k == 8) {
+  if (alive && (k == 0 || k == 1 || k == 3 || k == 4 || k == 6 || k == 7 || k == 8)) {
     const float* __restrict__ pV = (k == 6 || k == 7) ? v_l : vb_l;
     const int e_beg = live ? rpd_l[node] : 0, e_end = live ? min(rpd_l[node + 1], E) : 0;
     int j_nx = e_beg < e_end ? srcd_l[e_beg] : 0;
@@ -1196,7 +1245,7 @@
     else if (k < 5) g_v[jf * 3 + (k - 2)] = t;
     else g_vbar[jf * 3 + (k - 5)] = t;
   }
-  bi_core<1, 9, 2>(wr, gphi_l, stage, slices_out + (size_t)blockIdx.x * out_stride, F, n, tr, nullptr, nullptr, 8);
+  bi_core<1, 9, 2, 2, MASK>(wr, gphi_l, stage, slices_out + (size_t)blockIdx.x * out_stride, F, n, tr, nullptr, nullptr, 8);
   DL_WV(7);
   DL_PH(8, 8);
   DL_SPAN(8, 1);
@@ -1441,6 +1490,16 @@
     else { constexpr int QS = 6; __VA_ARGS__ }                             \
   } while (0)
 
+#define CGV_DL_VARIANT(variant, ...)                                       \
+  do {                                                                     \
+    switch (variant) {                                                     \
+      case 0: { constexpr int VAR = 0; __VA_ARGS__ } break;                \
+      case 1: { constexpr int VAR = 1; __VA_ARGS__ } break;                \
+      case 2: { constexpr int VAR = 2; __VA_ARGS__ } break;                \
+      default: { constexpr int VAR = 3; __VA_ARGS__ } break;               \
+    }                                                                      \
+  } while (0)
+
 #define CGV_DL_CHECK()                                                                                        \
   CGV_REQUIRE(cgv_decoder_layer_supported(n_nodes, n_feat, n_rbf), "unsupported shape (n <= 16 nodes, F % 4 == 0, 16 <= F <= 864)"); \
   hipStream_t st = (hipStream_t)stream;                                                                       \
@@ -1449,9 +1508,11 @@
 int cgv_decoder_msg_fwd(const float* a1, const float* W2, const float* b2, const float* s, const float* sbar, const float* v,
                         const float* vbar, const float* geom_d, const int32_t* rowptr_d, const int32_t* src_d, const float* Wd,
                         const float* bd, float* phi, float* stack, float* sbar_out, float* v_out, float* vbar_out,
-                        float* rows_out, int n_nodes, int n_feat, int n_rbf, int n_edges, void* stream) {
+                        float* rows_out, int n_nodes, int n_feat, int n_rbf, int n_edges, void* stream, int variant) {
   CGV_REQUIRE(a1 && W2 && b2 && s && sbar && v && vbar && geom_d && rowptr_d && src_d && Wd && bd, "null input");
   CGV_REQUIRE(phi && stack && sbar_out && v_out && vbar_out && rows_out, "null output");
+  CGV_REQUIRE(variant >= 0 && variant <= (CGV_DECODER_FIRST | CGV_DECODER_LAST), "variant: 0 or CGV_DECODER_FIRST | CGV_DECODER_LAST");
+  if (cgv::option(CGV_OPT_DECODER_ALL_LIVE) != 0) variant = 0;
   CGV_REQUIRE(n_edges >= 1 && n_edges <= cgv::DL_MAX_EDGES, "the staged bead graph holds 1..cgv_decoder_max_edges() edges");
   CGV_DL_CHECK();
   const size_t base_floats = cgv::fwd_red_floats<1, 9>() + 576 + 1536 + (size_t)cgv::DL_MAX_EDGES * cgv::geom_stride(n_rbf) + 20 +
@@ -1459,15 +1520,19 @@
   const bool wlds = cgv::option(CGV_OPT_DECODER_WLDS) != 0 && cgv::lds_bytes(base_floats + (size_t)36 * n_feat) <= 160 * 1024;
   const size_t lds = cgv::lds_bytes(base_floats + (wlds ? (size_t)36 * n_feat : 0));
   CGV_DISPATCH_RBF(n_rbf, {
-    if (wlds) {
-      if (int rc = cgv::allow_lds(cgv::dec_msg_fwd_k<RBF, true>, lds)) return rc;
-      hipLaunchKernelGGL((cgv::dec_msg_fwd_k<RBF, true>), dim3(blocks), dim3(cgv::DL_THREADS), lds, st, a1, W2, b2, s, sbar, v, vbar,
-                         geom_d, rowptr_d, src_d, Wd, bd, phi, stack, sbar_out, v_out, vbar_out, rows_out, n_nodes, n_feat, n_edges);
-    } else {
-      if (int rc = cgv::allow_lds(cgv::dec_msg_fwd_k<RBF, false>, lds)) return rc;
-      hipLaunchKernelGGL((cgv::dec_msg_fwd_k<RBF, false>), dim3(blocks), dim3(cgv::DL_THREADS), lds, st, a1, W2, b2, s, sbar, v, vbar,
-                         geom_d, rowptr_d, src_d, Wd, bd, phi, stack, sbar_out, v_out, vbar_out, rows_out, n_nodes, n_feat, n_edges);
-    }
+    CGV_DL_VARIANT(variant, {
+      if (wlds) {
+        if (int rc = cgv::allow_lds(cgv::dec_msg_fwd_k<RBF, true, VAR>, lds)) return rc;
+        hipLaunchKernelGGL((cgv::dec_msg_fwd_k<RBF, true, VAR>), dim3(blocks), dim3(cgv::DL_THREADS), lds, st, a1, W2, b2, s, sbar, v,
+                           vbar, geom_d, rowptr_d, src_d, Wd, bd, phi, stack, sbar_out, v_out, vbar_out, rows_out, n_nodes, n_feat,
+                           n_edges);
+      } else {
+        if (int rc = cgv::allow_lds(cgv::dec_msg_fwd_k<RBF, false, VAR>, lds)) return rc;
+        hipLaunchKernelGGL((cgv::dec_msg_fwd_k<RBF, false, VAR>), dim3(blocks), dim3(cgv::DL_THREADS), lds, st, a1, W2, b2, s, sbar, v,
+                           vbar, geom_d, rowptr_d, src_d, Wd, bd, phi, stack, sbar_out, v_out, vbar_out, rows_out, n_nodes, n_feat,
+                           n_edges);
+      }
+    });
   });
   return cgv::check_launch("cgv_decoder_msg_fwd");
 }
@@ -1671,23 +1736,28 @@
                         const float* ghb, const float* gvrows_slices, int n_slices, int64_t slice_stride, const float* gv_res,
                         const float* gvb, const float* W2, float* g_phi, float* g_s, float* g_sbar, float* g_v, float* g_vbar,
                         float* gWd, float* gbd, float* slices_out, int64_t out_slice_stride, int n_nodes, int n_feat, int n_rbf,
-                        int n_edges, void* stream) {
+                        int n_edges, void* stream, int variant) {
   CGV_REQUIRE(phi && s && sbar && v && vbar && geom_d && rowptr_d && src_d && geom_s && rowptr_s && dst_s && Wd && bd && W2,
               "null input");
   CGV_REQUIRE(gvrows_slices && n_slices >= 1 && n_slices <= 216 && g_phi && g_s && g_sbar && g_v && g_vbar && gWd && gbd && slices_out,
               "null pointer / slice count");
   CGV_REQUIRE(out_slice_stride >= cgv_decoder_slice_floats(n_feat, n_nodes), "bad slices");
   CGV_REQUIRE(n_edges >= 1 && n_edges <= cgv::DL_MAX_EDGES, "the staged bead graph holds 1..cgv_decoder_max_edges() edges");
+  CGV_REQUIRE(variant >= 0 && variant <= (CGV_DECODER_FIRST | CGV_DECODER_LAST), "variant: 0 or CGV_DECODER_FIRST | CGV_DECODER_LAST");
+  CGV_REQUIRE(!(variant & CGV_DECODER_LAST) || (!ghb && !gvb), "CGV_DECODER_LAST: no gradient may arrive for Sbar' / Vbar'");
+  if (cgv::option(CGV_OPT_DECODER_ALL_LIVE) != 0) variant = 0;
   CGV_DL_CHECK();
   const size_t lds = cgv::lds_bytes(cgv::bi_stage_floats<1>() + 192 + 576 + 576 + 3456 + 4608 +
                                2 * (size_t)cgv::DL_MAX_EDGES * cgv::geom_stride(n_rbf) + 40 + 2 * cgv::DL_MAX_EDGES + 256 + 960);
   CGV_DISPATCH_RBF(n_rbf, {
     CGV_DL_QS(n_slices, {
-      if (int rc = cgv::allow_lds(cgv::dec_msg_bwd_k<RBF, QS>, lds)) return rc;
-      hipLaunchKernelGGL((cgv::dec_msg_bwd_k<RBF, QS>), dim3(blocks), dim3(cgv::DL_THREADS), lds, st, phi, s, sbar, v, vbar, geom_d,
-                         rowptr_d, src_d, geom_s, rowptr_s, dst_s, Wd, bd, gh, ghb, gvrows_slices, n_slices,
-                         (long long)slice_stride, gv_res, gvb, W2, g_phi, g_s, g_sbar, g_v, g_vbar, gWd, gbd, slices_out,
-                         (long long)out_slice_stride, n_nodes, n_feat, n_edges);
+      CGV_DL_VARIANT(variant, {
+        if (int rc = cgv::allow_lds(cgv::dec_msg_bwd_k<RBF, QS, VAR>, lds)) return rc;
+        hipLaunchKernelGGL((cgv::dec_msg_bwd_k<RBF, QS, VAR>), dim3(blocks), dim3(cgv::DL_THREADS), lds, st, phi, s, sbar, v, vbar,
+                           geom_d, rowptr_d, src_d, geom_s, rowptr_s, dst_s, Wd, bd, gh, ghb, gvrows_slices, n_slices,
+                           (long long)slice_stride, gv_res, gvb, W2, g_phi, g_s, g_sbar, g_v, g_vbar, gWd, gbd, slices_out,
+                           (long long)out_slice_stride, n_nodes, n_feat, n_edges);
+      });
     });
   });
   return cgv::check_launch("cgv_decoder_msg_bwd");
diff --git a/coarsegrainingvae_amd/decoder_fused.py b/coarsegrainingvae_amd/decoder_fused.py
--- a/coarsegrainingvae_amd/decoder_fused.py
+++ b/coarsegrainingvae_amd/decoder_fused.py
@@ -33,6 +33,15 @@
 
 def staged_edges(plan) -> int:
     return max(1, min(int(plan.capacity), int(_lib.load().cgv_decoder_max_edges())))
+
+
+MSG_ALL_LIVE, MSG_FIRST, MSG_LAST = 0, 1, 2
+
+
+def layer_variant(layer: int, n_layers: int, product_state: bool) -> int:
+    if not product_state:
+        return MSG_ALL_LIVE
+    return (MSG_FIRST if layer < 2 else 0) | (MSG_LAST if layer == n_layers - 1 else 0)
 
 
 def usable(decoder, S: torch.Tensor, plan, geom) -> bool:
@@ -69,7 +78,7 @@
 class _PseudoDecoderFn(torch.autograd.Function):
 
     @staticmethod
-    def forward(ctx, S, Sbar0, V0, plan, geom, hooks, n_layers, *flat):
+    def forward(ctx, S, Sbar0, V0, plan, geom, hooks, n_layers, product_state, *flat):
         from .ops import _dense_fwd
         S = S.contiguous()
         n, F = S.shape
@@ -94,7 +103,8 @@
             _lib.call("cgv_decoder_msg_fwd", _lib.ptr(a1), _lib.ptr(W2), _lib.ptr(b2), _lib.ptr(S), _lib.ptr(Sbar), _lib.ptr(V),
                       _lib.ptr(Vbar), _lib.ptr(geom.geom_d), _lib.ptr(plan.rowptr_d), _lib.ptr(plan.src_d), _lib.ptr(Wd),
                       _lib.ptr(bd), _lib.ptr(phi), _lib.ptr(stack), _lib.ptr(Sbar2), _lib.ptr(V2), _lib.ptr(Vbar2), _lib.ptr(rows),
-                      n, F, R, n_stage, st, tag=f"pseudo_msg_fwd:Nd{n}:E{plan.n_edges}:dv1")
+                      n, F, R, n_stage, st, layer_variant(l, n_layers, product_state),
+                      tag=f"pseudo_msg_fwd:Nd{n}:E{plan.n_edges}:dv1")
             UV = new(3 * n, 2 * F)
             _lib.call("cgv_decoder_uv_fwd", _lib.ptr(rows), _lib.ptr(Wuv), _lib.ptr(UV), _lib.ptr(stack), n, F, st)
             z0, a0, a = new(n, F), new(n, F), new(n, 3 * F)
@@ -106,6 +116,7 @@
             S, Sbar, V, Vbar = S3, Sbar2, V3, Vbar2
             mark(f"decoder:fwd{l}")
         ctx.saved, ctx.flat, ctx.plan, ctx.geom, ctx.hooks, ctx.n_layers = saved, flat, plan, geom, hooks, n_layers
+        ctx.product_state = product_state
         ctx.set_materialize_grads(False)
         return S, V
 
@@ -113,7 +124,7 @@
     def backward(ctx, gS_out, gV_out):
         n_layers, flat, plan, geom = ctx.n_layers, ctx.flat, ctx.plan, ctx.geom
         if gS_out is None and gV_out is None:
-            return (None,) * (7 + len(flat))
+            return (None,) * (8 + len(flat))
         saved, ctx.saved = ctx.saved, None
         n, F = saved[0][0].shape
         R = geom.n_rbf
@@ -159,7 +170,8 @@
                       _lib.ptr(plan.rowptr_s), _lib.ptr(plan.dst_s), _lib.ptr(pWd.detach()), _lib.ptr(pbd.detach()),
                       _lib.ptr(g_s2), _lib.ptr(gSbar), _lib.ptr(p3), nF, fl48, _lib.ptr(gV), _lib.ptr(gVbar), _lib.ptr(pW2.detach()),
                       _lib.ptr(g_phi), _lib.ptr(g_s), _lib.ptr(g_sbar), _lib.ptr(g_v), _lib.ptr(g_vbar), _lib.ptr(tWd), _lib.ptr(tbd),
-                      _lib.ptr(p4), fl16(F), n, F, R, n_stage, st, tag=f"pseudo_msg_bwd:Nd{n}:E{plan.n_edges}:gv1")
+                      _lib.ptr(p4), fl16(F), n, F, R, n_stage, st, layer_variant(l, n_layers, ctx.product_state),
+                      tag=f"pseudo_msg_bwd:Nd{n}:E{plan.n_edges}:gv1")
             g_a1 = new(n, F)
             p5 = new(nF * fl16(F))
             _lib.call("cgv_decoder_dense_bwd", _lib.ptr(p4), nb, fl16(F), _lib.ptr(z1), ACT_SWISH, _lib.ptr(pW1.detach()),
@@ -179,11 +191,12 @@
         _lib.call("cgv_decoder_slices_to_dense", _lib.ptr(gS.base), _lib.ptr(gS.part), gS.n, gS.stride, _lib.ptr(gS_in), n, F, st)
         if not wgrad_queue.active:
             wgrad_queue.flush()
-        return (gS_in, None, None, None, None, None, None) + (None,) * len(flat)
-
-
-def pseudo_decoder(decoder, S, Sbar0, V0, plan, geom, layer_hooks=None):
+        return (gS_in, None, None, None, None, None, None, None) + (None,) * len(flat)
+
+
+def pseudo_decoder(decoder, S, Sbar0, V0, plan, geom, layer_hooks=None, product_state=False):
     global calls
     calls += 1
     flat = layer_params(decoder)
-    return _PseudoDecoderFn.apply(S, Sbar0, V0, plan, geom, layer_hooks or None, len(decoder.message_blocks), *flat)
+    return _PseudoDecoderFn.apply(S, Sbar0, V0, plan, geom, layer_hooks or None, len(decoder.message_blocks), bool(product_state),
+                                  *flat)
diff --git a/coarsegrainingvae_amd/model.py b/coarsegrainingvae_amd/model.py
--- a/coarsegrainingvae_amd/model.py
+++ b/coarsegrainingvae_amd/model.py
@@ -101,7 +101,7 @@
         if self.fused_loop and geom is not None and S.requires_grad:
             from . import decoder_fused
             if decoder_fused.usable(self, S, plan, geom):
-                return decoder_fused.pseudo_decoder(self, S, Sbar, V, plan, geom, layer_hooks)
+                return decoder_fused.pseudo_decoder(self, S, Sbar, V, plan, geom, layer_hooks, product_state=True)
         for layer, (message_block, update_block) in enumerate(zip(self.message_blocks, self.update_blocks)):
             if layer_hooks and layer in layer_hooks and S.requires_grad:
                 S = S.view_as(S)
diff --git a/include/cgvae_hip.h b/include/cgvae_hip.h
--- a/include/cgvae_hip.h
+++ b/include/cgvae_hip.h
@@ -8,7 +8,7 @@
 extern "C" {
 #endif
 
-#define CGV_VERSION 101
+#define CGV_VERSION 102
 
 #define CGV_E_BADARG (-1)
 #define CGV_E_UNSUPPORTED (-2)
@@ -36,7 +36,8 @@
   CGV_OPT_BWD_INPUT_SPLIT = 15,
   CGV_OPT_MSG_BWD_MFMA = 16,
   CGV_OPT_STREAMK = 17,
-  CGV_OPT_COUNT = 18
+  CGV_OPT_DECODER_ALL_LIVE = 18,
+  CGV_OPT_COUNT = 19
 };
 int cgv_timestamp(uint64_t* slot , void* stream);
 int cgv_timestamp_hz(void);
@@ -176,10 +177,11 @@
 int cgv_decoder_max_edges(void);
 int cgv_decoder_block_channels(int width);
 int cgv_decoder_debug_clock(uint64_t* buf );
+enum { CGV_DECODER_FIRST = 1, CGV_DECODER_LAST = 2 };
 int cgv_decoder_msg_fwd(const float* a1, const float* W2, const float* b2, const float* s, const float* sbar, const float* v,
                         const float* vbar, const float* geom_d, const int32_t* rowptr_d, const int32_t* src_d, const float* Wd,
                         const float* bd, float* phi, float* stack, float* sbar_out, float* v_out, float* vbar_out,
-                        float* rows_out, int n_nodes, int n_feat, int n_rbf, int n_edges, void* stream);
+                        float* rows_out, int n_nodes, int n_feat, int n_rbf, int n_edges, void* stream, int variant);
 int cgv_prior_msg_fwd(const float* a1, const float* W2, const float* b2, const float* s, const float* v, const float* geom_d,
                       const int32_t* rowptr_d, const int32_t* src_d, const float* Wd, const float* bd, float* phi, float* s_out,
                       float* v_out, int n_nodes, int n_feat, int n_rbf, int n_edges, int with_dv, void* stream);
@@ -208,7 +210,7 @@
                         const float* ghb , const float* gvrows_slices, int n_slices, int64_t slice_stride,
                         const float* gv_res , const float* gvb , const float* W2, float* g_phi, float* g_s,
                         float* g_sbar, float* g_v, float* g_vbar, float* gWd, float* gbd, float* slices_out,
-                        int64_t out_slice_stride, int n_nodes, int n_feat, int n_rbf, int n_edges, void* stream);
+                        int64_t out_slice_stride, int n_nodes, int n_feat, int n_rbf, int n_edges, void* stream, int variant);
 int cgv_decoder_slices_to_dense(const float* base , const float* slices, int n_slices, int64_t slice_stride,
                                 float* out, int n_nodes, int n_feat, void* stream);
 
```

Result: faster. 1303, median of 4 (+1.5%).
